# jwliao1209/DiffMusic

Hardware: AMD Instinct MI355X
Metric: denoising steps/sec (10 s clip, 200-step DPS) (higher is better)
Workload: dtype f16; 1 GPU; MusicLDM + DPS music_inpainting, 10 s @16 kHz, 200-step schedule, batch 8 per GPU (BASELINE.json configs[1]); global_batch=8, clips_per_gpu=8, lanes=1, parallelism=clip-sharded x1 (RCCL world size 1, no per-step collective), finite=True, nan_steps=0, settle_steps=10, cached_reference_transform=True, launched_by=single process

## Files before the change

diffmusic_amd/_lib.py:

```python
import ctypes as C
import os

_HERE = os.path.dirname(os.path.abspath(__file__))
LIB_PATH = os.environ.get("DMX_LIB_PATH") or os.path.join(_HERE, "lib", "libdiffmusic_hip.so")
MAX_STAGES = 8


class HifiGanConfig(C.Structure):
    _fields_ = [("model_in_dim", C.c_int), ("upsample_initial_channel", C.c_int), ("num_upsamples", C.c_int),
                ("upsample_rates", C.c_int * MAX_STAGES), ("upsample_kernel_sizes", C.c_int * MAX_STAGES),
                ("num_kernels", C.c_int), ("resblock_kernel_sizes", C.c_int * MAX_STAGES),
                ("num_dilations", C.c_int), ("resblock_dilation_sizes", C.c_int * (MAX_STAGES * MAX_STAGES)),
                ("leaky_relu_slope", C.c_float)]


class VaeConfig(C.Structure):
    _fields_ = [("latent_channels", C.c_int), ("out_channels", C.c_int), ("num_blocks", C.c_int),
                ("block_out_channels", C.c_int * MAX_STAGES), ("layers_per_block", C.c_int),
                ("norm_num_groups", C.c_int), ("eps", C.c_float)]


class UNetConfig(C.Structure):
    _fields_ = [("in_channels", C.c_int), ("out_channels", C.c_int), ("num_blocks", C.c_int),
                ("block_out_channels", C.c_int * MAX_STAGES), ("layers_per_block", C.c_int),
                ("attention_heads", C.c_int), ("norm_num_groups", C.c_int),
                ("down_attn", C.c_int * MAX_STAGES), ("up_attn", C.c_int * MAX_STAGES),
                ("class_embed_dim", C.c_int), ("num_attn_per_layer", C.c_int), ("attn_cross_dims", C.c_int * 4)]


class HtsatConfig(C.Structure):
    _fields_ = [("spec_size", C.c_int), ("num_mel_bins", C.c_int), ("patch_size", C.c_int), ("embed_dim", C.c_int), ("window_size", C.c_int),
                ("num_stages", C.c_int), ("depths", C.c_int * 4), ("num_heads", C.c_int * 4), ("ln_eps", C.c_float), ("bn_eps", C.c_float)]


class GemmDesc(C.Structure):
    _fields_ = [("A", C.c_void_p), ("W", C.c_void_p), ("C", C.c_void_p), ("C2", C.c_void_p),
                ("bias", C.c_void_p), ("rowbias", C.c_void_p), ("R", C.c_void_p), ("X", C.c_void_p),
                ("M", C.c_int), ("N", C.c_int), ("K", C.c_int), ("ldw", C.c_int),
                ("Hi", C.c_int), ("Wi", C.c_int), ("Ci", C.c_int), ("lda", C.c_int),
                ("Hq", C.c_int), ("Wq", C.c_int), ("sy", C.c_int), ("sx", C.c_int),
                ("ntaps", C.c_int),
                ("Ho", C.c_int), ("Wo", C.c_int), ("ldc", C.c_int), ("osy", C.c_int), ("ooy", C.c_int),
                ("osx", C.c_int), ("oox", C.c_int),
                ("ldr", C.c_int), ("ldx", C.c_int), ("ldc2", C.c_int),
                ("Z", C.c_int), ("Zi", C.c_int),
                ("sAo", C.c_longlong), ("sAi", C.c_longlong), ("sWo", C.c_longlong), ("sWi", C.c_longlong),
                ("sCo", C.c_longlong), ("sCi", C.c_longlong),
                ("alpha", C.c_float), ("act_slope", C.c_float), ("mask_slope", C.c_float),
                ("flags", C.c_int),
                ("tdy", C.c_byte * 16), ("tdx", C.c_byte * 16), ("resid_inv_slope", C.c_float), ("tile_cfg", C.c_int), ("ldrb", C.c_int), ("ksplit", C.c_int),
                ("XB", C.c_void_p), ("B2", C.c_void_p), ("ldxb", C.c_int), ("ldb2", C.c_int),
                ("colsum", C.c_void_p), ("ln_eps", C.c_float), ("rowstats_in", C.c_void_p), ("rowstats_out", C.c_void_p), ("nslots", C.c_int),
                ("gn_part", C.c_void_p), ("gnb_x", C.c_void_p), ("gnb_scale", C.c_void_p), ("gnb_shift", C.c_void_p),
                ("gnb_ldx", C.c_int), ("gnb_silu", C.c_int), ("gnb_stats", C.c_void_p), ("gnb_cpg", C.c_int)]


EPI_BIAS, EPI_ROWBIAS, EPI_RESID, EPI_ACCUM, EPI_MASK, EPI_LRELU2, EPI_TANH, EPI_F32OUT, EPI_NO_C, EPI_RESID_INV, EPI_MASKBITS, EPI_BITS2, EPI_SOFTBWD = \
    1, 2, 4, 8, 16, 32, 64, 128, 256, 512, 1024, 2048, 4096
EPI_GEGLU, EPI_LNFOLD, EPI_ROWSTATS, EPI_GNSTATS, EPI_GNBWD = 8192, 16384, 32768, 65536, 131072

_SIGS = {
    "dmx_abi_version": (C.c_int, []),
    "dmx_act_dtype": (C.c_int, []),
    "dmx_last_error": (C.c_char_p, []),
    "dmx_hifigan_create": (C.c_void_p, [C.POINTER(HifiGanConfig)]),
    "dmx_vae_decoder_create": (C.c_void_p, [C.POINTER(VaeConfig)]),
    "dmx_unet_create": (C.c_void_p, [C.POINTER(UNetConfig)]),
    "dmx_model_destroy": (None, [C.c_void_p]),
    "dmx_model_num_params": (C.c_int, [C.c_void_p]),
    "dmx_model_param_name": (C.c_char_p, [C.c_void_p, C.c_int]),
    "dmx_model_param_numel": (C.c_size_t, [C.c_void_p, C.c_int]),
    "dmx_model_param_ndim": (C.c_int, [C.c_void_p, C.c_int]),
    "dmx_model_param_dim": (C.c_int, [C.c_void_p, C.c_int, C.c_int]),
    "dmx_model_load_param": (C.c_int, [C.c_void_p, C.c_char_p, C.c_void_p, C.c_size_t]),
    "dmx_model_finalize": (C.c_int, [C.c_void_p, C.c_void_p]),
    "dmx_hifigan_out_len": (C.c_int, [C.c_void_p, C.c_int]),
    "dmx_hifigan_workspace_bytes": (C.c_size_t, [C.c_void_p, C.c_int, C.c_int]),
    "dmx_hifigan_fwd": (C.c_int, [C.c_void_p, C.c_void_p, C.c_void_p, C.c_int, C.c_int, C.c_void_p, C.c_size_t, C.c_void_p]),
    "dmx_hifigan_bwd": (C.c_int, [C.c_void_p, C.c_void_p, C.c_void_p, C.c_void_p]),
    "dmx_hifigan_fwd_dead": (C.c_int, [C.c_void_p, C.c_void_p, C.c_void_p, C.c_int, C.c_int, C.c_int, C.c_int, C.c_void_p, C.c_size_t,
                                       C.c_void_p]),
    "dmx_hifigan_dead_plan": (C.c_int, [C.c_void_p, C.POINTER(C.c_int), C.POINTER(C.c_int), C.POINTER(C.c_int), C.POINTER(C.c_int), C.c_int]),
    "dmx_conv_dead_rows": (C.c_int, [C.c_int] * 9 + [C.POINTER(C.c_int), C.POINTER(C.c_int)]),
    "dmx_vae_workspace_bytes": (C.c_size_t, [C.c_void_p, C.c_int, C.c_int, C.c_int]),
    "dmx_vae_decode_fwd": (C.c_int, [C.c_void_p, C.c_void_p, C.c_float, C.c_void_p, C.c_void_p, C.c_int, C.c_int, C.c_int,
                                     C.c_int, C.c_void_p, C.c_size_t, C.c_void_p]),
    "dmx_vae_decode_bwd": (C.c_int, [C.c_void_p, C.c_void_p, C.c_float, C.c_void_p, C.c_void_p]),
    "dmx_vae_encoder_create": (C.c_void_p, [C.POINTER(VaeConfig)]),
    "dmx_vae_encoder_workspace_bytes": (C.c_size_t, [C.c_void_p, C.c_int, C.c_int, C.c_int]),
    "dmx_vae_encode_fwd": (C.c_int, [C.c_void_p, C.c_void_p, C.c_float, C.c_void_p, C.c_int, C.c_int, C.c_int, C.c_void_p, C.c_size_t,
                                     C.c_void_p]),
    "dmx_latent_init": (C.c_int, [C.c_void_p] * 6 + [C.c_int] * 3 + [C.c_float] * 3 + [C.c_void_p]),
    "dmx_conv2d_raw": (C.c_int, [C.c_void_p] * 4 + [C.c_int] * 9 + [C.c_void_p]),
    "dmx_unet_workspace_bytes": (C.c_size_t, [C.c_void_p, C.c_int, C.c_int, C.c_int]),
    "dmx_unet_fwd": (C.c_int, [C.c_void_p, C.c_void_p, C.c_void_p, C.c_void_p, C.c_void_p, C.c_int, C.c_int, C.c_int,
                               C.c_void_p, C.c_size_t, C.c_void_p]),
    "dmx_unet_fwd_ctx": (C.c_int, [C.c_void_p] * 5 + [C.c_int, C.c_void_p, C.c_int, C.c_void_p, C.c_void_p, C.c_int, C.c_int, C.c_int,
                                   C.c_void_p, C.c_size_t, C.c_void_p]),
    "dmx_unet_workspace_bytes_ctx": (C.c_size_t, [C.c_void_p, C.c_int, C.c_int, C.c_int, C.c_int, C.c_int]),
    "dmx_htsat_create": (C.c_void_p, [C.POINTER(HtsatConfig)]),
    "dmx_htsat_feature_dims": (C.c_int, [C.c_void_p, C.POINTER(C.c_int), C.POINTER(C.c_int)]),
    "dmx_htsat_workspace_bytes": (C.c_size_t, [C.c_void_p, C.c_int, C.c_int]),
    "dmx_htsat_fwd": (C.c_int, [C.c_void_p, C.c_void_p, C.c_int, C.c_int, C.c_void_p, C.c_int, C.c_void_p, C.c_size_t, C.c_void_p]),
    "dmx_htsat_bwd": (C.c_int, [C.c_void_p, C.c_void_p, C.c_void_p, C.c_void_p, C.c_void_p]),
    "dmx_htsat_tape_raw": (C.c_size_t, [C.c_void_p, C.c_int, C.c_int, C.c_int, C.c_void_p, C.c_size_t, C.c_void_p]),
    "dmx_gram_fwd": (C.c_int, [C.c_void_p, C.c_void_p, C.c_int, C.c_int, C.c_int, C.c_void_p]),
    "dmx_gram_bwd": (C.c_int, [C.c_void_p, C.c_void_p, C.c_void_p, C.c_int, C.c_int, C.c_int, C.c_void_p]),
    "dmx_gemm_raw": (C.c_int, [C.c_void_p, C.c_size_t, C.c_void_p]),
    "dmx_prof_begin": (None, []),
    "dmx_prof_end": (C.c_int, [C.POINTER(C.c_double), C.POINTER(C.c_double)]),
    "dmx_flash_attn_raw": (C.c_int, [C.c_void_p, C.c_void_p, C.c_void_p, C.c_void_p, C.c_void_p] + [C.c_int] * 6 + [C.c_float, C.c_void_p]),
    "dmx_flash_attn_ld_raw": (C.c_int, [C.c_void_p] * 5 + [C.c_int] * 8 + [C.c_float, C.POINTER(C.c_int), C.c_void_p]),
    "dmx_softmax_raw": (C.c_int, [C.c_void_p] * 3 + [C.c_longlong, C.c_int, C.c_longlong, C.c_longlong, C.c_int, C.c_void_p]),
    "dmx_softmax_act_raw": (C.c_int, [C.c_void_p] * 3 + [C.c_longlong, C.c_int, C.c_longlong, C.c_int, C.c_void_p]),
    "dmx_transpose_raw": (C.c_int, [C.c_void_p, C.c_void_p, C.c_int, C.c_int, C.c_longlong, C.c_longlong, C.c_int, C.c_int] + [C.c_longlong] * 4
                          + [C.c_void_p]),
    "dmx_rowdot_raw": (C.c_int, [C.c_void_p] * 3 + [C.c_longlong, C.c_int, C.c_longlong, C.c_longlong, C.c_void_p]),
    "dmx_layernorm_raw": (C.c_int, [C.c_void_p] * 4 + [C.c_int, C.c_int, C.c_float, C.c_void_p]),
    "dmx_geglu_raw": (C.c_int, [C.c_void_p, C.c_void_p, C.c_longlong, C.c_int, C.c_void_p]),
    "dmx_gemm_splitk_workspace": (C.c_int, [C.c_void_p, C.c_size_t]),
    "dmx_conv_pair_raw": (C.c_int, [C.c_void_p, C.c_void_p, C.c_size_t, C.c_void_p]),
    "dmx_conv_pair_group_raw": (C.c_int, [C.c_int, C.c_void_p, C.c_void_p, C.c_size_t, C.c_void_p]),
    "dmx_conv_pair_dead_raw": (C.c_int, [C.c_void_p, C.c_void_p, C.c_size_t, C.POINTER(C.c_int), C.POINTER(C.c_int), C.POINTER(C.c_int), C.c_void_p]),
    "dmx_conv_pair_group_dead_raw": (C.c_int, [C.c_int, C.c_void_p, C.c_void_p, C.c_size_t, C.POINTER(C.c_int), C.c_void_p]),
    "dmx_groupnorm_scratch_floats": (C.c_size_t, [C.c_int, C.c_int, C.c_int]),
    "dmx_groupnorm_raw": (C.c_int, [C.c_void_p] * 8 + [C.c_int] * 4 + [C.c_float, C.c_int, C.c_void_p]),
    "dmx_groupnorm_part_floats": (C.c_size_t, [C.c_int, C.c_int, C.c_int]),
    "dmx_groupnorm_parts_raw": (C.c_int, [C.c_void_p] * 7 + [C.c_int] * 4 + [C.c_float, C.c_int, C.c_int, C.c_void_p, C.c_void_p, C.c_void_p]),
    "dmx_gemm_last_tile_rows_raw": (C.c_int, []),
    "dmx_groupnorm_bwd_raw": (C.c_int, [C.c_void_p] * 10 + [C.c_int] * 6 + [C.c_void_p, C.c_void_p, C.c_void_p]),
    "dmx_prof_dominant": (C.c_int, [C.POINTER(C.c_double)] * 3),
    "dmx_audio_create": (C.c_void_p, [C.c_int, C.c_int, C.c_int, C.c_int, C.c_void_p]),
    "dmx_audio_destroy": (None, [C.c_void_p]),
    "dmx_audio_num_frames": (C.c_int, [C.c_void_p, C.c_int]),
    "dmx_audio_num_bins": (C.c_int, [C.c_void_p]),
    "dmx_audio_state_bytes": (C.c_size_t, [C.c_void_p, C.c_int, C.c_int]),
    "dmx_audio_transform_fwd": (C.c_int, [C.c_void_p, C.c_void_p, C.c_longlong, C.c_void_p, C.c_void_p, C.c_int, C.c_int, C.c_int,
                                          C.c_int, C.c_float, C.c_float, C.c_void_p]),
    "dmx_audio_transform_bwd": (C.c_int, [C.c_void_p, C.c_void_p, C.c_void_p, C.c_longlong, C.c_void_p, C.c_int, C.c_int, C.c_int,
                                          C.c_int, C.c_float, C.c_float, C.c_int, C.c_void_p]),
    "dmx_audio_is_fused": (C.c_int, [C.c_void_p, C.c_int]),
    "dmx_audio_guidance_fwd": (C.c_int, [C.c_void_p, C.c_void_p, C.c_longlong, C.c_void_p, C.c_void_p, C.c_longlong, C.c_void_p, C.c_void_p,
                                         C.c_int, C.c_int, C.c_int, C.c_int, C.c_float, C.c_float, C.c_void_p]),
    "dmx_audio_guidance_bwd": (C.c_int, [C.c_void_p, C.c_void_p, C.c_longlong, C.c_void_p, C.c_void_p, C.c_longlong, C.c_float, C.c_void_p,
                                         C.c_void_p, C.c_longlong, C.c_int, C.c_void_p, C.c_int, C.c_int, C.c_int, C.c_int, C.c_float, C.c_float,
                                         C.c_void_p]),
    "dmx_audio_guidance_fwd_ex": (C.c_int, [C.c_void_p, C.c_void_p, C.c_longlong, C.c_void_p, C.c_void_p, C.c_longlong, C.c_void_p, C.c_void_p,
                                            C.c_int, C.c_int, C.c_int, C.c_int, C.c_float, C.c_float, C.c_void_p, C.c_longlong, C.c_void_p,
                                            C.c_float, C.c_void_p]),
    "dmx_audio_guidance_bwd_ex": (C.c_int, [C.c_void_p, C.c_void_p, C.c_longlong, C.c_void_p, C.c_void_p, C.c_longlong, C.c_float, C.c_void_p,
                                            C.c_void_p, C.c_longlong, C.c_int, C.c_void_p, C.c_int, C.c_int, C.c_int, C.c_int, C.c_float, C.c_float,
                                            C.c_void_p, C.c_longlong, C.c_void_p, C.c_float, C.c_void_p]),
    "dmx_audio_guidance_fwd_shaped": (C.c_int, [C.c_void_p, C.c_void_p, C.c_longlong, C.c_void_p, C.c_void_p, C.c_longlong, C.c_void_p, C.c_void_p,
                                                C.c_int, C.c_int, C.c_int, C.c_int, C.c_float, C.c_float, C.c_void_p, C.c_longlong, C.c_void_p,
                                                C.c_float, C.c_void_p, C.c_void_p]),
    "dmx_audio_guidance_bwd_shaped": (C.c_int, [C.c_void_p, C.c_void_p, C.c_longlong, C.c_void_p, C.c_void_p, C.c_longlong, C.c_float, C.c_void_p,
                                                C.c_void_p, C.c_longlong, C.c_int, C.c_void_p, C.c_int, C.c_int, C.c_int, C.c_int, C.c_float, C.c_float,
                                                C.c_void_p, C.c_longlong, C.c_void_p, C.c_float, C.c_void_p, C.c_void_p]),
    "dmx_clip_fwd": (C.c_int, [C.c_void_p, C.c_longlong, C.c_void_p, C.c_void_p, C.c_longlong, C.c_int, C.c_int, C.c_void_p]),
    "dmx_clip_bwd": (C.c_int, [C.c_void_p, C.c_longlong, C.c_void_p, C.c_longlong, C.c_void_p, C.c_void_p, C.c_longlong, C.c_int, C.c_int, C.c_int,
                               C.c_void_p]),
    "dmx_declip_project": (C.c_int, [C.c_void_p, C.c_longlong, C.c_void_p, C.c_longlong, C.c_void_p, C.c_void_p, C.c_longlong, C.c_int, C.c_int,
                                     C.c_void_p]),
    "dmx_drc_fwd": (C.c_int, [C.c_void_p, C.c_longlong, C.c_void_p, C.c_longlong, C.c_void_p, C.c_void_p, C.c_int, C.c_int] + [C.c_float] * 6 +
                    [C.c_void_p]),
    "dmx_drc_bwd": (C.c_int, [C.c_void_p, C.c_longlong, C.c_void_p, C.c_longlong, C.c_void_p, C.c_void_p, C.c_void_p, C.c_void_p, C.c_longlong,
                              C.c_int, C.c_int, C.c_int] + [C.c_float] * 6 + [C.c_void_p]),
    "dmx_drc_fwd_p": (C.c_int, [C.c_void_p, C.c_longlong, C.c_void_p, C.c_longlong, C.c_void_p, C.c_void_p, C.c_void_p, C.c_int, C.c_int, C.c_float,
                                C.c_void_p]),
    "dmx_drc_bwd_p": (C.c_int, [C.c_void_p, C.c_longlong, C.c_void_p, C.c_longlong] + [C.c_void_p] * 6 + [C.c_longlong, C.c_int, C.c_int, C.c_int,
                                                                                                        C.c_float, C.c_void_p]),
    "dmx_drc_pgrad": (C.c_int, [C.c_void_p] * 6 + [C.c_int, C.c_int, C.c_float, C.c_void_p]),
    "dmx_drc_update": (C.c_int, [C.c_void_p] * 5 + [C.c_int] * 3 + [C.c_void_p] + [C.c_double] * 3 + [C.c_float, C.c_void_p, C.c_void_p, C.c_void_p]),
    "dmx_warp_fwd": (C.c_int, [C.c_void_p, C.c_longlong, C.c_void_p, C.c_longlong, C.c_void_p, C.c_int, C.c_int, C.c_void_p]),
    "dmx_warp_bwd": (C.c_int, [C.c_void_p, C.c_void_p, C.c_longlong, C.c_void_p, C.c_int, C.c_int, C.c_int, C.c_void_p]),
    "dmx_warp_wgrad": (C.c_int, [C.c_void_p, C.c_void_p, C.c_longlong, C.c_void_p, C.c_longlong, C.c_void_p, C.c_int, C.c_int, C.c_void_p]),
    "dmx_warp_update": (C.c_int, [C.c_void_p] * 5 + [C.c_int] * 4 + [C.c_double] * 5 + [C.c_int, C.c_void_p]),
    "dmx_click_detect": (C.c_int, [C.c_void_p, C.c_longlong] + [C.c_void_p] * 5 + [C.c_int, C.c_int, C.c_float, C.c_float, C.c_void_p]),
    "dmx_click_mask": (C.c_int, [C.c_void_p, C.c_void_p, C.c_void_p, C.c_int, C.c_int, C.c_int, C.c_void_p]),
    "dmx_mask_rows": (C.c_int, [C.c_void_p, C.c_longlong, C.c_void_p, C.c_longlong, C.c_void_p, C.c_int, C.c_int, C.c_int, C.c_void_p]),
    "dmx_declick_blend": (C.c_int, [C.c_void_p, C.c_longlong, C.c_void_p, C.c_longlong, C.c_void_p, C.c_longlong, C.c_void_p, C.c_int, C.c_int,
                                    C.c_int, C.c_void_p]),
    "dmx_noise_add": (C.c_int, [C.c_void_p, C.c_void_p, C.c_void_p, C.c_longlong, C.c_float, C.c_void_p]),
    "dmx_audio_stft_mag": (C.c_int, [C.c_void_p, C.c_void_p, C.c_longlong, C.c_void_p, C.c_void_p, C.c_int, C.c_int, C.c_void_p]),
    "dmx_audio_stft_mag_bwd": (C.c_int, [C.c_void_p, C.c_void_p, C.c_void_p, C.c_longlong, C.c_void_p, C.c_int, C.c_int, C.c_int, C.c_void_p]),
    "dmx_audio_tf_frames": (C.c_int, [C.c_int]),
    "dmx_audio_tf_gain": (C.c_int, [C.c_void_p, C.c_void_p, C.c_longlong, C.c_void_p, C.c_longlong, C.c_void_p, C.c_longlong, C.c_int, C.c_int, C.c_int,
                                    C.c_void_p]),
    "dmx_audio_tf_curve": (C.c_int, [C.c_void_p, C.c_void_p, C.c_longlong, C.c_void_p, C.c_longlong, C.c_void_p, C.c_longlong, C.c_int, C.c_int, C.c_int,
                                     C.c_void_p]),
    "dmx_audio_tf_wgrad_segments": (C.c_int, [C.c_int]),
    "dmx_audio_tf_wgrad": (C.c_int, [C.c_void_p, C.c_void_p, C.c_longlong, C.c_void_p, C.c_longlong, C.c_void_p, C.c_int, C.c_int, C.c_void_p]),
    "dmx_audio_eq_update": (C.c_int, [C.c_void_p, C.c_int] + [C.c_void_p] * 3 + [C.c_int, C.c_int] + [C.c_double] * 4 + [C.c_int, C.c_void_p]),
    "dmx_audio_melscale": (C.c_int, [C.c_void_p, C.c_void_p, C.c_void_p, C.c_int, C.c_int, C.c_float, C.c_float, C.c_void_p]),
    "dmx_mask_apply": (C.c_int, [C.c_void_p, C.c_longlong, C.c_void_p, C.c_void_p, C.c_longlong, C.c_int, C.c_int, C.c_int, C.c_void_p]),
    "dmx_l2_loss": (C.c_int, [C.c_void_p, C.c_longlong, C.c_void_p, C.c_void_p, C.c_void_p, C.c_int, C.c_longlong, C.c_float, C.c_void_p]),
    "dmx_track_stitch_fwd": (C.c_int, [C.c_void_p, C.c_longlong, C.c_void_p, C.POINTER(C.c_int)] + [C.c_int] * 4 + [C.c_void_p]),
    "dmx_track_stitch_bwd": (C.c_int, [C.c_void_p, C.c_void_p, C.c_longlong, C.POINTER(C.c_int)] + [C.c_int] * 5 + [C.c_void_p]),
    "dmx_stem_mix_fwd": (C.c_int, [C.c_void_p, C.c_longlong, C.c_void_p, C.POINTER(C.c_float)] + [C.c_int] * 3 + [C.c_void_p]),
    "dmx_stem_mix_bwd": (C.c_int, [C.c_void_p, C.c_void_p, C.c_longlong, C.POINTER(C.c_float)] + [C.c_int] * 4 + [C.c_void_p]),
    "dmx_stem_project": (C.c_int, [C.c_void_p, C.c_longlong, C.c_void_p, C.c_void_p, C.POINTER(C.c_float), C.c_int, C.c_int, C.c_void_p]),
    "dmx_grad_normalize": (C.c_int, [C.c_void_p, C.c_void_p, C.c_int, C.c_longlong, C.c_float, C.c_void_p]),
    "dmx_fir_fwd": (C.c_int, [C.c_void_p, C.c_longlong, C.c_void_p, C.c_void_p, C.c_longlong] + [C.c_int] * 7 + [C.c_void_p]),
    "dmx_fir_bwd": (C.c_int, [C.c_void_p, C.c_longlong, C.c_void_p, C.c_void_p, C.c_void_p, C.c_longlong] + [C.c_int] * 7 + [C.c_void_p]),
    "dmx_fir_clip_fwd": (C.c_int, [C.c_void_p, C.c_longlong, C.c_void_p, C.c_void_p, C.c_longlong] + [C.c_int] * 4 + [C.c_void_p]),
    "dmx_fir_clip_bwd": (C.c_int, [C.c_void_p, C.c_longlong, C.c_void_p, C.c_void_p, C.c_void_p, C.c_longlong] + [C.c_int] * 4 + [C.c_void_p]),
    "dmx_fir_wgrad_workspace_floats": (C.c_size_t, [C.c_int, C.c_int, C.c_int]),
    "dmx_fir_wgrad": (C.c_int, [C.c_void_p, C.c_longlong, C.c_void_p, C.c_longlong, C.c_void_p, C.c_size_t] + [C.c_int] * 4 + [C.c_void_p]),
    "dmx_ir_update": (C.c_int, [C.c_void_p, C.c_int] + [C.c_void_p] * 4 + [C.c_int, C.c_int] + [C.c_double] * 4 + [C.c_int, C.c_void_p]),
    "dmx_sched_pred_x0": (C.c_int, [C.c_void_p, C.c_void_p, C.c_void_p, C.c_longlong, C.c_float, C.c_void_p]),
    "dmx_sched_pred_x0_ex": (C.c_int, [C.c_void_p, C.c_void_p, C.c_void_p, C.c_longlong, C.c_float, C.c_int, C.c_float, C.c_void_p]),
    "dmx_sched_step_ex": (C.c_int, [C.c_int] + [C.c_void_p] * 9 + [C.c_int, C.c_int] + [C.c_float] * 5 + [C.c_int, C.c_int, C.c_float, C.c_void_p]),
    "dmx_sched_cfg_combine": (C.c_int, [C.c_void_p, C.c_void_p, C.c_longlong, C.c_float, C.c_void_p]),
    "dmx_randn_philox": (C.c_int, [C.c_void_p, C.c_int, C.c_longlong, C.POINTER(C.c_ulonglong), C.c_ulonglong, C.c_void_p]),
    "dmx_sched_step": (C.c_int, [C.c_int] + [C.c_void_p] * 9 + [C.c_int, C.c_int] + [C.c_float] * 5 + [C.c_int, C.c_void_p]),
}

ADDED_IN_V4 = ("dmx_vae_encoder_create", "dmx_vae_encoder_workspace_bytes", "dmx_vae_encode_fwd", "dmx_latent_init",
               "dmx_track_stitch_fwd", "dmx_track_stitch_bwd", "dmx_audio_guidance_fwd_shaped", "dmx_audio_guidance_bwd_shaped",
               "dmx_clip_fwd", "dmx_clip_bwd", "dmx_declip_project", "dmx_hifigan_fwd_dead", "dmx_hifigan_dead_plan", "dmx_conv_dead_rows",
               "dmx_fir_clip_fwd", "dmx_fir_clip_bwd", "dmx_fir_wgrad", "dmx_fir_wgrad_workspace_floats", "dmx_ir_update",
               "dmx_stem_mix_fwd", "dmx_stem_mix_bwd", "dmx_stem_project", "dmx_audio_tf_gain", "dmx_audio_tf_frames",
               "dmx_audio_tf_curve", "dmx_audio_tf_wgrad_segments", "dmx_audio_tf_wgrad", "dmx_audio_eq_update", "dmx_drc_fwd", "dmx_drc_bwd",
               "dmx_warp_fwd", "dmx_warp_bwd", "dmx_warp_wgrad", "dmx_warp_update", "dmx_drc_fwd_p", "dmx_drc_bwd_p", "dmx_drc_pgrad",
               "dmx_drc_update", "dmx_click_detect", "dmx_click_mask", "dmx_mask_rows", "dmx_declick_blend")

_lib = None


def check_symbols(h, path=LIB_PATH):
    for name in ADDED_IN_V4:
        if not hasattr(h, name):
            raise RuntimeError(f"{path} reports ABI version {ABI_VERSION} but does not export `{name}` (a build from before the VAE "
                               "encoder / track-mode / declipping / blind-dereverberation / source-separation / time-frequency-masking / blind-equalisation / de-compression / wow-and-flutter / blind-wow-and-flutter / blind-de-compression / declicking entry points): rebuild it (python -m diffmusic_amd.build --force)")


def lib():
    global _lib
    if _lib is None:
        if not os.path.exists(LIB_PATH):
            raise RuntimeError(f"{LIB_PATH} is missing: build it with `python -m diffmusic_amd.build` "
                               "(the diffmusic_amd hot path has no CPU fallback)")
        h = C.CDLL(LIB_PATH)
        for name, (res, args) in _SIGS.items():
            if not hasattr(h, name):
                continue
            fn = getattr(h, name)
            fn.restype, fn.argtypes = res, args
        if h.dmx_abi_version() != ABI_VERSION:
            raise RuntimeError(f"libdiffmusic_hip.so ABI version {h.dmx_abi_version()} != {ABI_VERSION} expected by this package: rebuild it "
                               "(python -m diffmusic_amd.build --force)")
        check_symbols(h)
        _lib = h
    return _lib


ABI_VERSION = 4


def act_dtype():
    import torch
    return torch.float16 if lib().dmx_act_dtype() == 1 else torch.bfloat16


class DmxError(RuntimeError):
    pass


def check(rc, what=""):
    if rc != 0:
        msg = lib().dmx_last_error()
        raise DmxError(f"{what} failed with code {rc}: {msg.decode() if msg else ''}")
```

diffmusic_amd/csrc/capi.hip:

```cpp
#include "conv_pair.h"
#include "models.h"

#define M_IMPL(m) ((m) ? (m)->impl : nullptr)
#define ST(s) ((hipStream_t)(s))

extern "C" {

int dmx_abi_version(void) { return DMX_ABI_VERSION; }
int dmx_act_dtype(void) { return DMX_ACT_DTYPE; }

dmx_model* dmx_hifigan_create(const dmx_hifigan_config* cfg) {
  if (!cfg || cfg->num_upsamples > DMX_MAX_STAGES || cfg->num_kernels > DMX_MAX_STAGES || cfg->num_dilations > DMX_MAX_STAGES) {
    dmx_set_error("bad hifigan config");
    return nullptr;
  }
  return new dmx_model{dmx_make_hifigan(cfg)};
}
dmx_model* dmx_vae_decoder_create(const dmx_vae_config* cfg) {
  if (!cfg || cfg->num_blocks > DMX_MAX_STAGES) { dmx_set_error("bad vae config"); return nullptr; }
  Model* m = dmx_make_vae(cfg);
  return m ? new dmx_model{m} : nullptr;
}
dmx_model* dmx_unet_create(const dmx_unet_config* cfg) {
  if (!cfg || cfg->num_blocks > DMX_MAX_STAGES) { dmx_set_error("bad unet config"); return nullptr; }
  Model* m = dmx_make_unet(cfg);
  return m ? new dmx_model{m} : nullptr;
}
void dmx_model_destroy(dmx_model* m) {
  if (!m) return;
  delete m->impl;
  delete m;
}
int dmx_model_num_params(const dmx_model* m) { return (int)m->impl->ps.params.size(); }
const char* dmx_model_param_name(const dmx_model* m, int i) { return m->impl->ps.params[i].name.c_str(); }
size_t dmx_model_param_numel(const dmx_model* m, int i) { return m->impl->ps.params[i].numel; }
int dmx_model_param_ndim(const dmx_model* m, int i) { return (int)m->impl->ps.params[i].shape.size(); }
int dmx_model_param_dim(const dmx_model* m, int i, int d) { return m->impl->ps.params[i].shape[d]; }
int dmx_model_load_param(dmx_model* m, const char* name, const float* data_host, size_t numel) {
  if (m->impl->finalized) { dmx_set_error("model already finalized"); return DMX_ERR_STATE; }
  return m->impl->ps.load(name, data_host, numel);
}
int dmx_model_finalize(dmx_model* m, void* stream) {
  std::string missing;
  if (!m->impl->ps.all_loaded(&missing)) { dmx_set_error("parameter '%s' was never loaded", missing.c_str()); return DMX_ERR_PARAM; }
  const int rc = m->impl->finalize(ST(stream));
  if (rc == DMX_OK) m->impl->finalized = true;
  return rc;
}

static int check(dmx_model* m, int kind) {
  if (!m || !m->impl || m->impl->kind != kind) { dmx_set_error("wrong model handle"); return DMX_ERR_STATE; }
  if (!m->impl->finalized) { dmx_set_error("model not finalized"); return DMX_ERR_STATE; }
  return DMX_OK;
}

int dmx_hifigan_out_len(const dmx_model* m, int frames) { return dmx_hifigan_out_len_impl(m->impl, frames); }
size_t dmx_hifigan_workspace_bytes(dmx_model* m, int batch, int frames) { return dmx_hifigan_ws_impl(m->impl, batch, frames); }
int dmx_hifigan_fwd(dmx_model* m, const uint16_t* mel, float* wav, int batch, int frames, void* ws, size_t ws_bytes, void* stream) {
  int rc = check(m, DMX_MODEL_HIFIGAN);
  if (rc) return rc;
  if (!ws) { dmx_set_error("null workspace"); return DMX_ERR_WORKSPACE; }
  return dmx_hifigan_fwd_impl(m->impl, mel, wav, batch, frames, ws, ws_bytes, ST(stream));
}
int dmx_hifigan_fwd_dead(dmx_model* m, const uint16_t* mel, float* wav, int batch, int frames, int s0, int s1, void* ws, size_t ws_bytes,
                         void* stream) {
  int rc = check(m, DMX_MODEL_HIFIGAN);
  if (rc) return rc;
  if (!ws || !mel || !wav) { dmx_set_error("hifigan_fwd_dead: null buffer"); return DMX_ERR_STATE; }
  return dmx_hifigan_fwd_dead_impl(m->impl, mel, wav, batch, frames, s0, s1, ws, ws_bytes, ST(stream));
}
int dmx_hifigan_dead_plan(dmx_model* m, int* skipped, int* total, int* lo, int* hi, int n) {
  if (!m || !m->impl || m->impl->kind != DMX_MODEL_HIFIGAN) { dmx_set_error("wrong model handle"); return -1; }
  return dmx_hifigan_dead_plan_impl(m->impl, skipped, total, lo, hi, n);
}
int dmx_conv_dead_rows(int k, int dil, int pad, int stride, int transposed, int t_in, int t_out, int a, int b, int* lo, int* hi) {
  if (!lo || !hi) return DMX_ERR_STATE;
  return dmx_conv_dead_rows_impl(k, dil, pad, stride, transposed, t_in, t_out, a, b, lo, hi);
}
int dmx_hifigan_bwd(dmx_model* m, const float* dwav, uint16_t* dmel, void* stream) {
  int rc = check(m, DMX_MODEL_HIFIGAN);
  if (rc) return rc;
  return dmx_hifigan_bwd_impl(m->impl, dwav, dmel, ST(stream));
}

size_t dmx_vae_workspace_bytes(dmx_model* m, int batch, int h, int w) { return dmx_vae_ws_impl(m->impl, batch, h, w); }
int dmx_vae_decode_fwd(dmx_model* m, const float* z, float z_scale, uint16_t* mel, float* mel_f32, int batch, int h, int w,
                       int keep_state, void* ws, size_t ws_bytes, void* stream) {
  int rc = check(m, DMX_MODEL_VAE);
  if (rc) return rc;
  if (!ws) { dmx_set_error("null workspace"); return DMX_ERR_WORKSPACE; }
  return dmx_vae_fwd_impl(m->impl, z, z_scale, mel, mel_f32, batch, h, w, keep_state, ws, ws_bytes, ST(stream));
}
int dmx_vae_decode_bwd(dmx_model* m, const uint16_t* dmel, float z_scale, float* dz, void* stream) {
  int rc = check(m, DMX_MODEL_VAE);
  if (rc) return rc;
  return dmx_vae_bwd_impl(m->impl, dmel, z_scale, dz, ST(stream));
}

dmx_model* dmx_vae_encoder_create(const dmx_vae_config* cfg) {
  if (!cfg || cfg->num_blocks > DMX_MAX_STAGES) { dmx_set_error("bad vae config"); return nullptr; }
  Model* m = dmx_make_vae_encoder(cfg);
  return m ? new dmx_model{m} : nullptr;
}
size_t dmx_vae_encoder_workspace_bytes(dmx_model* m, int batch, int frames, int bins) {
  if (!m || !m->impl || m->impl->kind != DMX_MODEL_VAE_ENC) return 0;
  return dmx_vae_enc_ws_impl(m->impl, batch, frames, bins);
}
int dmx_vae_encode_fwd(dmx_model* m, const float* mel, float log_floor, float* moments, int batch, int frames, int bins, void* ws,
                       size_t ws_bytes, void* stream) {
  int rc = check(m, DMX_MODEL_VAE_ENC);
  if (rc) return rc;
  if (!ws) { dmx_set_error("null workspace"); return DMX_ERR_WORKSPACE; }
  return dmx_vae_enc_fwd_impl(m->impl, mel, log_floor, moments, batch, frames, bins, ws, ws_bytes, ST(stream));
}
int dmx_latent_init(const float* moments, float* mean, float* logvar, float* x, const float* eps, const float* noise, int batch,
                    int latent_channels, int hw, float sqrt_abar, float scaling_factor, float sqrt_1m_abar, void* stream) {
  return dmx_latent_init_impl(moments, mean, logvar, x, eps, noise, batch, latent_channels, hw, sqrt_abar, scaling_factor, sqrt_1m_abar, ST(stream));
}
int dmx_conv2d_raw(const float* w_host, const float* b_host, const void* x, void* y, int B, int Hi, int Wi, int Ci, int Co, int k, int stride,
                   int pad_lo, int pad_hi, void* stream) {
  return dmx_conv2d_raw_impl(w_host, b_host, (const act_t*)x, (act_t*)y, B, Hi, Wi, Ci, Co, k, stride, pad_lo, pad_hi, ST(stream));
}

dmx_model* dmx_htsat_create(const dmx_htsat_config* cfg) {
  Model* impl = dmx_make_htsat(cfg);
  if (!impl) return nullptr;
  return new dmx_model{impl};
}
int dmx_htsat_feature_dims(dmx_model* m, int* tokens, int* channels) {
  if (!m || !m->impl || m->impl->kind != DMX_MODEL_HTSAT) { dmx_set_error("wrong model handle"); return DMX_ERR_STATE; }
  dmx_htsat_dims_impl(m->impl, tokens, channels);
  return DMX_OK;
}
size_t dmx_htsat_workspace_bytes(dmx_model* m, int batch, int frames) {
  if (!m || !m->impl || m->impl->kind != DMX_MODEL_HTSAT) return 0;
  return dmx_htsat_ws_impl(m->impl, batch, frames);
}
int dmx_htsat_fwd(dmx_model* m, const float* mel, int batch, int frames, float* feat, int keep_state, void* ws, size_t ws_bytes, void* stream) {
  int rc = check(m, DMX_MODEL_HTSAT);
  if (rc) return rc;
  if (!ws) { dmx_set_error("null workspace"); return DMX_ERR_WORKSPACE; }
  return dmx_htsat_fwd_impl(m->impl, mel, batch, frames, feat, keep_state, ws, ws_bytes, ST(stream));
}
int dmx_htsat_bwd(dmx_model* m, const float* dfeat, const float* scale, float* dmel, void* stream) {
  int rc = check(m, DMX_MODEL_HTSAT);
  if (rc) return rc;
  return dmx_htsat_bwd_impl(m->impl, dfeat, scale, dmel, ST(stream));
}
size_t dmx_htsat_tape_raw(dmx_model* m, int stage, int block, int which, void* dst, size_t dst_elems, void* stream) {
  if (!m || !m->impl || m->impl->kind != DMX_MODEL_HTSAT) return 0;
  const act_t* p = nullptr;
  const size_t n = dmx_htsat_tape_impl(m->impl, stage, block, which, &p);
  if (n && dst && dst_elems >= n) (void)hipMemcpyAsync(dst, p, n * sizeof(act_t), hipMemcpyDeviceToDevice, ST(stream));
  return n;
}
int dmx_gram_fwd(const float* F, float* G, int batch, int tokens, int channels, void* stream) {
  const int rc = dmx_gram_fwd_impl(F, G, batch, tokens, channels, ST(stream));
  if (rc == DMX_ERR_SHAPE) dmx_set_error("gram: 1 <= tokens <= 96");
  return rc;
}
int dmx_gram_bwd(const float* F, const float* dG, float* dF, int batch, int tokens, int channels, void* stream) {
  return dmx_gram_bwd_impl(F, dG, dF, batch, tokens, channels, ST(stream));
}

size_t dmx_unet_workspace_bytes(dmx_model* m, int batch, int h, int w) { return dmx_unet_ws_impl(m->impl, batch, h, w, 0, 0); }
size_t dmx_unet_workspace_bytes_ctx(dmx_model* m, int batch, int h, int w, int n0, int n1) { return dmx_unet_ws_impl(m->impl, batch, h, w, n0, n1); }
int dmx_unet_fwd(dmx_model* m, const float* x, const float* t, const float* class_labels, float* eps, int batch, int h, int w,
                 void* ws, size_t ws_bytes, void* stream) {
  int rc = check(m, DMX_MODEL_UNET);
  if (rc) return rc;
  if (!ws) { dmx_set_error("null workspace"); return DMX_ERR_WORKSPACE; }
  return dmx_unet_fwd_impl(m->impl, x, t, class_labels, eps, batch, h, w, ws, ws_bytes, ST(stream), nullptr, 0, nullptr, 0, nullptr);
}
int dmx_unet_fwd_ctx(dmx_model* m, const float* x, const float* t, const float* class_labels, const float* ctx0, int n0,
                     const float* ctx1, int n1, const float* bias1, float* eps, int batch, int h, int w, void* ws, size_t ws_bytes,
                     void* stream) {
  int rc = check(m, DMX_MODEL_UNET);
  if (rc) return rc;
  if (!ws) { dmx_set_error("null workspace"); return DMX_ERR_WORKSPACE; }
  return dmx_unet_fwd_impl(m->impl, x, t, class_labels, eps, batch, h, w, ws, ws_bytes, ST(stream), ctx0, n0, ctx1, n1, bias1);
}

static thread_local int g_raw_gn_rows = 0;
int dmx_gemm_raw(const void* desc, size_t desc_bytes, void* stream) {
  if (desc_bytes != sizeof(GemmDesc)) { dmx_set_error("GemmDesc size mismatch: %zu vs %zu", desc_bytes, sizeof(GemmDesc)); return DMX_ERR_SHAPE; }
  return dmx_gemm_launch(*reinterpret_cast<const GemmDesc*>(desc), ST(stream), &g_raw_gn_rows);
}
int dmx_gemm_last_tile_rows_raw(void) { return g_raw_gn_rows; }

int dmx_conv_pair_raw(const void* desc_a, const void* desc_b, size_t desc_bytes, void* stream) {
  if (desc_bytes != sizeof(GemmDesc)) { dmx_set_error("GemmDesc size mismatch: %zu vs %zu", desc_bytes, sizeof(GemmDesc)); return DMX_ERR_SHAPE; }
  const GemmDesc* a = reinterpret_cast<const GemmDesc*>(desc_a);
  const GemmDesc& b = *reinterpret_cast<const GemmDesc*>(desc_b);
  if (!dmx_conv_pair_eligible(a, b)) { dmx_set_error("shape not handled by the fused convolution-pair kernel"); return DMX_ERR_SHAPE; }
  return dmx_conv_pair_launch(a, b, ST(stream));
}

int dmx_conv_pair_group_raw(int n, const void* descs_a, const void* descs_b, size_t desc_bytes, void* stream) {
  if (desc_bytes != sizeof(GemmDesc)) { dmx_set_error("GemmDesc size mismatch: %zu vs %zu", desc_bytes, sizeof(GemmDesc)); return DMX_ERR_SHAPE; }
  if (n < 1 || n > 3) { dmx_set_error("conv pair group: 1..3 problems"); return DMX_ERR_SHAPE; }
  const GemmDesc* a = reinterpret_cast<const GemmDesc*>(descs_a);
  const GemmDesc* b = reinterpret_cast<const GemmDesc*>(descs_b);
  const GemmDesc* pa[3]; const GemmDesc* pb[3];
  for (int j = 0; j < n; ++j) { pa[j] = a + j; pb[j] = b + j; }
  const int rc = dmx_conv_pair_group_launch(n, pa, pb, ST(stream));
  if (rc == DMX_ERR_SHAPE) dmx_set_error("shape not handled by the fused convolution-pair kernel");
  return rc;
}

static PairDead pair_dead_of(const int* d) { PairDead pd; pd.skip0 = d[0]; pd.skip1 = d[1]; pd.zero0 = d[2]; pd.zero1 = d[3]; return pd; }

int dmx_conv_pair_dead_raw(const void* desc_a, const void* desc_b, size_t desc_bytes, const int* dead, int* skipped, int* total, void* stream) {
  if (skipped) *skipped = 0;
  if (total) *total = 0;
  if (desc_bytes != sizeof(GemmDesc)) { dmx_set_error("GemmDesc size mismatch: %zu vs %zu", desc_bytes, sizeof(GemmDesc)); return DMX_ERR_SHAPE; }
  const GemmDesc* a = reinterpret_cast<const GemmDesc*>(desc_a);
  const GemmDesc& b = *reinterpret_cast<const GemmDesc*>(desc_b);
  if (!dmx_conv_pair_eligible(a, b)) { dmx_set_error("shape not handled by the fused convolution-pair kernel"); return DMX_ERR_SHAPE; }
  PairDead pd;
  if (dead) pd = pair_dead_of(dead);
  int sk = 0, tot = 0;
  dmx_conv_pair_slabs(a, b, dead ? &pd : nullptr, &sk, &tot);
  if (skipped) *skipped = sk;
  if (total) *total = tot;
  const int rc = dmx_conv_pair_launch(a, b, ST(stream), dead ? &pd : nullptr);
  if (rc == DMX_ERR_SHAPE) dmx_set_error("dead rows not handled by the fused convolution-pair kernel (zero rows need the residual to be stage a's input)");
  return rc;
}

int dmx_conv_pair_group_dead_raw(int n, const void* descs_a, const void* descs_b, size_t desc_bytes, const int* dead, void* stream) {
  if (desc_bytes != sizeof(GemmDesc)) { dmx_set_error("GemmDesc size mismatch: %zu vs %zu", desc_bytes, sizeof(GemmDesc)); return DMX_ERR_SHAPE; }
  if (n < 1 || n > 3) { dmx_set_error("conv pair group: 1..3 problems"); return DMX_ERR_SHAPE; }
  const GemmDesc* a = reinterpret_cast<const GemmDesc*>(descs_a);
  const GemmDesc* b = reinterpret_cast<const GemmDesc*>(descs_b);
  const GemmDesc* pa[3]; const GemmDesc* pb[3];
  PairDead pd[3];
  for (int j = 0; j < n; ++j) { pa[j] = a + j; pb[j] = b + j; if (dead) pd[j] = pair_dead_of(dead + 4 * j); }
  const int rc = dmx_conv_pair_group_launch(n, pa, pb, ST(stream), dead ? pd : nullptr);
  if (rc == DMX_ERR_SHAPE) dmx_set_error("shape not handled by the fused convolution-pair kernel");
  return rc;
}

int dmx_flash_attn_raw(const void* q, const void* k, const void* v, void* o, const float* colbias, int B, int Nq, int Nk, int ldv, int C,
                       int heads, float scale, void* stream) {
  const int rc = dmx_flash_attn_fwd((const act_t*)q, (const act_t*)k, (const act_t*)v, (act_t*)o, colbias, B, Nq, Nk, C, heads, scale,
                                    ST(stream), 0, 0, ldv);
  if (rc == DMX_ERR_SHAPE) dmx_set_error("flash attention: unsupported head_dim / strides");
  return rc;
}

int dmx_flash_attn_ld_raw(const void* q, const void* k, const void* v, void* o, const float* colbias, int B, int Nq, int Nk, int ldq, int ldk,
                          int ldv, int C, int heads, float scale, int* qt_out, void* stream) {
  if (qt_out) *qt_out = 0;
  if (B < 1 || heads < 1 || C < heads || C % heads) { dmx_set_error("flash attention: C %d is not heads %d x head_dim", C, heads); return DMX_ERR_SHAPE; }
  const int rc = dmx_flash_attn_fwd((const act_t*)q, (const act_t*)k, (const act_t*)v, (act_t*)o, colbias, B, Nq, Nk, C, heads, scale,
                                    ST(stream), ldq, ldk, ldv, qt_out);
  if (rc == DMX_ERR_SHAPE)
    dmx_set_error("flash attention: head_dim %d (multiples of 8 up to 96), Nq %d, Nk %d (>= 1) or row strides %d / %d / %d (multiples of 8) unsupported",
                  C / heads, Nq, Nk, ldq, ldk, ldv);
  return rc;
}

int dmx_softmax_raw(const float* S, void* P, const float* colbias, long long rows, int N, long long lds, long long ldp, int rows_per_bias,
                    void* stream) {
  const int rc = dmx_softmax_fwd(S, (act_t*)P, colbias, rows, N, lds, ldp, rows_per_bias, ST(stream));
  if (rc == DMX_ERR_SHAPE) dmx_set_error("softmax: N %d (a multiple of 4, <= 4096), lds %lld, ldp %lld (multiples of 4) unsupported", N, lds, ldp);
  return rc;
}
int dmx_softmax_act_raw(const void* S, void* P, const float* colbias, long long rows, int N, long long ldp, int rows_per_bias, void* stream) {
  const int rc = dmx_softmax_act((const act_t*)S, (act_t*)P, colbias, rows, N, ldp, rows_per_bias, ST(stream));
  if (rc == DMX_ERR_SHAPE) dmx_set_error("softmax: N %d (a multiple of 4, <= 4096), ldp %lld (a multiple of 4) unsupported", N, ldp);
  return rc;
}
int dmx_transpose_raw(const void* in, void* out, int R, int C, long long ldi, long long ldo, int Z, int Zi, long long sIo, long long sIi,
                      long long sOo, long long sOi, void* stream) {
  return dmx_transpose((const act_t*)in, (act_t*)out, R, C, ldi, ldo, Z, Zi, sIo, sIi, sOo, sOi, ST(stream));
}
int dmx_rowdot_raw(const void* a, const void* b, float* out, long long rows, int C, long long lda, long long ldb, void* stream) {
  const int rc = dmx_rowdot((const act_t*)a, (const act_t*)b, out, rows, C, lda, ldb, ST(stream));
  if (rc == DMX_ERR_SHAPE) dmx_set_error("rowdot: C %d, lda %lld, ldb %lld must be multiples of 8", C, lda, ldb);
  return rc;
}
int dmx_layernorm_raw(const void* x, void* y, const float* gamma, const float* beta, int rows, int C, float eps, void* stream) {
  const int rc = dmx_layernorm_fwd((const act_t*)x, (act_t*)y, gamma, beta, rows, C, eps, ST(stream));
  if (rc == DMX_ERR_SHAPE) dmx_set_error("layernorm: C %d must be a multiple of 8", C);
  return rc;
}
int dmx_geglu_raw(const void* x, void* y, long long rows, int I, void* stream) {
  const int rc = dmx_geglu((const act_t*)x, (act_t*)y, rows, I, ST(stream));
  if (rc == DMX_ERR_SHAPE) dmx_set_error("geglu: I %d must be a multiple of 8", I);
  return rc;
}

int dmx_gemm_splitk_workspace(void* ws, size_t bytes) {
  dmx_gemm_set_splitk_workspace(reinterpret_cast<float*>(ws), ws ? bytes : 0);
  return DMX_OK;
}

size_t dmx_groupnorm_scratch_floats(int B, int C, int G) { return dmx_gn_scratch_floats(B, C, G); }
int dmx_groupnorm_raw(const void* x, void* y, const float* gamma, const float* beta, float* stats, float* scale, float* shift,
                      float* partial, int B, int P, int C, int G, float eps, int silu, void* stream) {
  const int rc = dmx_groupnorm_fwd((const act_t*)x, (act_t*)y, gamma, beta, stats, scale, shift, partial, B, P, C, G, eps, silu, ST(stream));
  if (rc == DMX_ERR_SHAPE) dmx_set_error("groupnorm: unsupported channel / group counts");
  return rc;
}

size_t dmx_groupnorm_part_floats(int B, int P, int N) { return dmx_gn_part_floats(B, P, N); }
int dmx_groupnorm_parts_raw(const void* x, void* y, const float* gamma, const float* beta, float* stats, float* scale, float* shift,
                            int B, int P, int C, int G, float eps, int silu, int nreg, float* const* part, const int* geom, void* stream) {
  if (nreg < 1 || nreg > 8) { dmx_set_error("groupnorm_parts: 1..8 regions"); return DMX_ERR_SHAPE; }
  if (G <= 0 || C % G || ((C / G) & 3)) { dmx_set_error("groupnorm_parts: channels per group must be a multiple of 4 (C %d, G %d)", C, G); return DMX_ERR_SHAPE; }
  GnParts gp;
  for (int i = 0; i < nreg; ++i) {
    GnRegion r;
    r.part = part[i]; r.tm = geom[i * 6]; r.P = geom[i * 6 + 1]; r.nq = geom[i * 6 + 2]; r.qoff = geom[i * 6 + 3]; r.cq = geom[i * 6 + 4];
    if (!r.part || r.tm < 32 || r.P < r.tm || r.nq <= 0 || r.cq <= 0 || r.cq > r.nq || r.qoff < 0 || r.qoff + r.cq > C / 4) {
      dmx_set_error("groupnorm_parts: region %d: tm %d, P %d, nq %d, qoff %d, cq %d do not describe a producer launch of this tensor", i, r.tm, r.P, r.nq, r.qoff, r.cq);
      return DMX_ERR_SHAPE;
    }
    gp.r[gp.n++] = r;
  }
  const int rc = dmx_groupnorm_fwd((const act_t*)x, (act_t*)y, gamma, beta, stats, scale, shift, nullptr, B, P, C, G, eps, silu, ST(stream), &gp);
  if (rc == DMX_ERR_SHAPE) dmx_set_error("groupnorm: unsupported channel / group counts");
  return rc;
}
int dmx_groupnorm_bwd_raw(const void* x, const void* dy, const void* add, void* dx, const float* stats, const float* scale, const float* shift,
                          float* k0, float* k1, float* partial, int B, int P, int C, int G, int silu, int nreg, float* const* part,
                          const int* geom, void* stream) {
  if (nreg < 0 || nreg > 8) { dmx_set_error("groupnorm_bwd: 0..8 regions"); return DMX_ERR_SHAPE; }
  if (nreg > 0 && !partial && (G <= 0 || C % G || ((C / G) & 3))) { dmx_set_error("groupnorm_bwd: regions need channels per group % 4 == 0, or scratch for the classic pass"); return DMX_ERR_SHAPE; }
  GnParts gp;
  for (int i = 0; i < nreg; ++i) {
    GnRegion r;
    r.part = part[i]; r.tm = geom[i * 6]; r.P = geom[i * 6 + 1]; r.nq = geom[i * 6 + 2]; r.qoff = geom[i * 6 + 3]; r.cq = geom[i * 6 + 4];
    if (!r.part || r.tm < 32 || r.P < r.tm || r.nq <= 0 || r.cq <= 0 || r.cq > r.nq || r.qoff < 0 || r.qoff + r.cq > C / 4) {
      dmx_set_error("groupnorm_bwd: region %d does not describe a producer launch of this tensor", i);
      return DMX_ERR_SHAPE;
    }
    gp.r[gp.n++] = r;
  }
  return dmx_groupnorm_bwd((const act_t*)x, (const act_t*)dy, (const act_t*)add, (act_t*)dx, stats, scale, shift, k0, k1, partial, B, P, C, G,
                           silu, ST(stream), nreg ? &gp : nullptr);
}

}
```

diffmusic_amd/csrc/conv_pair.h:

```cpp
#pragma once
#include <cstdlib>
#include <cstring>
#include "dmx_common.h"

struct PairDead { int skip0 = 0, skip1 = 0, zero0 = 0, zero1 = 0; };

bool dmx_conv_pair_eligible(const GemmDesc* a, const GemmDesc& b);
int dmx_conv_pair_launch(const GemmDesc* a, const GemmDesc& b, hipStream_t st, const PairDead* dead = nullptr);
int dmx_conv_pair_group_launch(int n, const GemmDesc* const* a, const GemmDesc* const* b, hipStream_t st, const PairDead* dead = nullptr);
void dmx_conv_pair_slabs(const GemmDesc* a, const GemmDesc& b, const PairDead* dead, int* skipped, int* total);

int dmx_prof_open(hipStream_t st);
void dmx_prof_close(int rec, hipStream_t st, double flops, double bytes, int M, int N, int K, int taps, int flags, int cfg);
```

diffmusic_amd/csrc/conv_pair.hip:

```cpp
#include "gemm_epilogue.h"
#include "conv_pair.h"

namespace {

constexpr int PAIR_HALO = 50;
constexpr int PAIR_ROWS = 256;
constexpr unsigned PAIR_OOB = 0x80000000u;

struct PairParams {
  GemmDesc a, b;
  int T, nb, BMo;
  int loA, hiA, loB, hiB;
  int off0A, dA, off0B, dB;
  int single;
  int r_from_slab;
  int a_tape_bits_only;
  int skip_q0, skip_n;
  int z0, z1;
};

#ifdef DMX_PAIR_STAMPS
__device__ unsigned long long g_pair_stamps[4096 * 8];
#define DMX_STAMP(i) do { stamp_v[i] = wall_clock64(); } while (0)
#else
#define DMX_STAMP(i) do { } while (0)
#endif

template <int C>
struct PairCfg {
  static constexpr int PITCH = 2 * C + 32;
  static constexpr int CPR = C / 8;
  static constexpr int WN = C > 64 ? C / 64 : 1;
  static constexpr int NW = 4 * WN;
  static constexpr int NT = NW * 64;
  static constexpr int FN = C / 16 / WN;
  static constexpr int SLAB_ROWS = PAIR_ROWS + PAIR_HALO;
  static constexpr int SLAB_BYTES = SLAB_ROWS * PITCH;
  static constexpr int TILE = C * 128;
  static constexpr int NS = C == 128 ? 4 : 3;
  static constexpr int PER = TILE / 1024 / NW;
  static constexpr int SLAB_IT = (SLAB_ROWS * CPR + NT - 1) / NT;
  static constexpr int BITS_IT = PAIR_ROWS * CPR / NT;
  static constexpr int BITS_BYTES = PAIR_ROWS * CPR;
  static constexpr int BIAS_BYTES = 2 * C * 4;
  static constexpr int LDS_BYTES = SLAB_BYTES + NS * TILE + BITS_BYTES + BIAS_BYTES;
  static constexpr int MIN_WAVES = C == 32 ? 3 : 2;
  static_assert(PER >= 1 && PAIR_ROWS * CPR % NT == 0, "tile / thread-count mismatch");
};

template <int FN>
struct PairFrags { frag8_t x[2][4]; frag8_t w[2][FN]; };

#define DMX_PAIR_DSR(dst, addr, off) asm volatile("ds_read_b128 %0, %1 offset:%2" : "=v"(dst) : "v"(addr), "n"(off))

#define DMX_LDS_ADDR(p) ((unsigned)(size_t)(__attribute__((address_space(3))) const char*)(p))
typedef unsigned u32x2_t __attribute__((ext_vector_type(2)));
typedef unsigned u32x4_t __attribute__((ext_vector_type(4)));
__device__ __forceinline__ void pair_lds_w64(const void* p, uint2 v) {
  const u32x2_t w = {v.x, v.y};
  asm volatile("ds_write_b64 %0, %1" ::"v"(DMX_LDS_ADDR(p)), "v"(w) : "memory");
}
#define DMX_PAIR_DSR64(dst, p) asm volatile("ds_read_b64 %0, %1" : "=v"(dst) : "v"(DMX_LDS_ADDR(p)))
#define DMX_PAIR_DSRU8(dst, p) asm volatile("ds_read_u8 %0, %1" : "=v"(dst) : "v"(DMX_LDS_ADDR(p)))
__device__ __forceinline__ void pair_lds_wait() { asm volatile("s_waitcnt lgkmcnt(0)" ::: "memory"); }
template <typename T>
__device__ __forceinline__ void pair_tie8(T (&r)[8]) {
  asm volatile("s_waitcnt lgkmcnt(0)" : "+v"(r[0]), "+v"(r[1]), "+v"(r[2]), "+v"(r[3]), "+v"(r[4]), "+v"(r[5]), "+v"(r[6]), "+v"(r[7]) : : "memory");
}
template <typename T>
__device__ __forceinline__ void pair_tie16(T (&r)[16]) {
  asm volatile("s_waitcnt lgkmcnt(0)"
               : "+v"(r[0]), "+v"(r[1]), "+v"(r[2]), "+v"(r[3]), "+v"(r[4]), "+v"(r[5]), "+v"(r[6]), "+v"(r[7]), "+v"(r[8]), "+v"(r[9]), "+v"(r[10]),
                 "+v"(r[11]), "+v"(r[12]), "+v"(r[13]), "+v"(r[14]), "+v"(r[15])
               :
               : "memory");
}
template <typename T, int N>
__device__ __forceinline__ void pair_tie(T (&r)[N]) {
  static_assert(N == 8 || N == 16, "4 row fragments x 2 or 4 column fragments");
  if constexpr (N == 8) pair_tie8(r); else pair_tie16(r);
}

__device__ __forceinline__ void pair_settle(PairFrags<4>& f) {
  asm volatile("s_waitcnt lgkmcnt(0)"
               : "+v"(f.x[0][0]), "+v"(f.x[0][1]), "+v"(f.x[0][2]), "+v"(f.x[0][3]), "+v"(f.x[1][0]), "+v"(f.x[1][1]), "+v"(f.x[1][2]),
                 "+v"(f.x[1][3]), "+v"(f.w[0][0]), "+v"(f.w[0][1]), "+v"(f.w[0][2]), "+v"(f.w[0][3]), "+v"(f.w[1][0]), "+v"(f.w[1][1]),
                 "+v"(f.w[1][2]), "+v"(f.w[1][3])
               :
               : "memory");
}
__device__ __forceinline__ void pair_settle(PairFrags<2>& f) {
  asm volatile("s_waitcnt lgkmcnt(0)"
               : "+v"(f.x[0][0]), "+v"(f.x[0][1]), "+v"(f.x[0][2]), "+v"(f.x[0][3]), "+v"(f.x[1][0]), "+v"(f.x[1][1]), "+v"(f.x[1][2]),
                 "+v"(f.x[1][3]), "+v"(f.w[0][0]), "+v"(f.w[0][1]), "+v"(f.w[1][0]), "+v"(f.w[1][1])
               :
               : "memory");
}

template <int C>
__device__ __forceinline__ void pair_body(const PairParams& P, char* smem, int bid, const int nwg) {
  using K = PairCfg<C>;
  constexpr int PITCH = K::PITCH, CPR = K::CPR, FN = K::FN, NS = K::NS, PER = K::PER, TILE = K::TILE, NT = K::NT, NW = K::NW, WN = K::WN;
  char* ring = smem;
  char* slab = smem + NS * TILE;
  unsigned char* s_bits = reinterpret_cast<unsigned char*>(slab + K::SLAB_BYTES);
  float* s_bias = reinterpret_cast<float*>(slab + K::SLAB_BYTES + K::BITS_BYTES);

  const int tid = threadIdx.x, lane = tid & 63, lr = lane & 15, lq = lane >> 4;
  const int wave = __builtin_amdgcn_readfirstlane(tid >> 6);
  const int rg = wave / WN, cg = wave - rg * WN;
#ifdef DMX_PAIR_STAMPS
  const int stamp_id = bid;
  unsigned long long stamp_v[8] = {0, 0, 0, 0, 0, 0, 0, 0};
#endif
  DMX_STAMP(0);
  {
    const int q = nwg >> 3, r = nwg & 7, xcd = bid & 7, loc = bid >> 3;
    bid = (xcd < r ? xcd * (q + 1) : r * (q + 1) + (xcd - r) * q) + loc;
  }
  const int T = P.T;
  const int b = bid / P.nb;
  int tq = bid - b * P.nb;
  if (tq >= P.skip_q0) tq += P.skip_n;
  const int t0 = tq * P.BMo;
  const bool single = P.single != 0;
  const int kA = single ? 0 : P.a.ntaps, kB = P.b.ntaps;
  const int stepsA = (kA * C + 63) / 64, stepsB = (kB * C + 63) / 64, total = stepsA + stepsB;

  const __amdgpu_buffer_rsrc_t rsA = __builtin_amdgcn_make_buffer_rsrc(const_cast<act_t*>(single ? P.b.W : P.a.W), 0, PAIR_OOB, 0x00020000);
  const __amdgpu_buffer_rsrc_t rsB = __builtin_amdgcn_make_buffer_rsrc(const_cast<act_t*>(P.b.W), 0, PAIR_OOB, 0x00020000);
  const int lrow = lane >> 3, cc = (lane & 7) ^ lrow;
  auto issue_dma = [&](int g) {
    const bool inA = g < stepsA;
    const int sidx = inA ? g : g - stepsA;
    const int Kel = inA ? P.a.K : P.b.K;
    const unsigned ldw2 = (unsigned)(inA ? P.a.ldw : P.b.ldw) * 2u;
    const int kel = sidx * 64 + cc * 8;
    const bool ok = g < total && kel < Kel;
    char* dst = ring + (g % NS) * TILE;
#pragma unroll
    for (int i = 0; i < PER; ++i) {
      const int j = i * NW + wave;
      const unsigned voff = ok ? (unsigned)(j * 8 + lrow) * ldw2 + (unsigned)kel * 2u : PAIR_OOB;
      if (inA) __builtin_amdgcn_raw_ptr_buffer_load_lds(rsA, (__attribute__((address_space(3))) void*)(dst + j * 1024), 16, voff, 0, 0, 0);
      else __builtin_amdgcn_raw_ptr_buffer_load_lds(rsB, (__attribute__((address_space(3))) void*)(dst + j * 1024), 16, voff, 0, 0, 0);
    }
  };
  issue_dma(0);
  issue_dma(1);
  issue_dma(2);

  {
    const act_t* src = single ? P.b.A : P.a.A;
    const int nrows = PAIR_ROWS + (single ? P.loB + P.hiB : P.loA + P.hiA);
    const int tfirst = t0 - P.loB - (single ? 0 : P.loA);
    uint4 sv[K::SLAB_IT];
#pragma unroll
    for (int it = 0; it < K::SLAB_IT; ++it) {
      const int c = tid + it * NT, row = c / CPR, piece = c % CPR, t = tfirst + row;
      sv[it] = make_uint4(0, 0, 0, 0);
      if (row < nrows && t >= 0 && t < T && !(t >= P.z0 && t < P.z1)) sv[it] = *reinterpret_cast<const uint4*>(src + ((long long)b * T + t) * C + piece * 8);
    }
    const bool masked = !single && (P.a.flags & EPI_MASK);
    const bool maskbits = !single && (P.a.flags & EPI_MASKBITS);
    constexpr int BPT = K::BITS_BYTES / NT;
    static_assert(BPT == 4 || BPT == 8, "bit-mask copy granularity");
    static_assert(CPR % BPT == 0, "a thread's mask bytes must stay inside one row");
    uint32_t mb[2] = {0u, 0u};
    if (maskbits) {
      const int c = tid * BPT, row = c / CPR, piece = c % CPR, t = t0 - P.loB + row;
      if (t >= 0 && t < T) {
        const unsigned char* src = P.a.XB + ((long long)b * T + t) * P.a.ldxb + piece;
        mb[0] = *reinterpret_cast<const uint32_t*>(src);
        if (BPT == 8) mb[1] = *reinterpret_cast<const uint32_t*>(src + 4);
      }
    }
#pragma unroll
    for (int it = 0; it < K::SLAB_IT; ++it) {
      const int c = tid + it * NT, row = c / CPR, piece = c % CPR;
      if (row < K::SLAB_ROWS) *reinterpret_cast<uint4*>(slab + row * PITCH + piece * 16) = sv[it];
    }
    if (masked) {
#pragma unroll 1
      for (int it = 0; it < K::BITS_IT; ++it) {
        const int c = tid + it * NT, row = c / CPR, piece = c % CPR, t = t0 - P.loB + row;
        uint4 m = make_uint4(0, 0, 0, 0);
        if (t >= 0 && t < T) m = *reinterpret_cast<const uint4*>(P.a.X + ((long long)b * T + t) * C + piece * 8);
        s_bits[c] = (unsigned char)dmx_pos8(m);
      }
    }
    if (maskbits) {
      uint32_t* d = reinterpret_cast<uint32_t*>(s_bits + tid * BPT);
      d[0] = mb[0];
      if (BPT == 8) d[1] = mb[1];
    }
  }
  if (tid < 2 * C) {
    const GemmDesc& d = tid < C ? P.a : P.b;
    const int ch = tid < C ? tid : tid - C;
    s_bias[tid] = (!(single && tid < C) && d.bias && (d.flags & (EPI_BIAS | EPI_BIASINIT))) ? d.bias[ch] : 0.f;
  }
  asm volatile("s_waitcnt vmcnt(0)" ::: "memory");
  __syncthreads();
  DMX_STAMP(1);

  f32x4 acc[4][FN];
  auto zero_acc = [&]() {
#pragma unroll
    for (int i = 0; i < 4; ++i)
#pragma unroll
      for (int n = 0; n < FN; ++n) acc[i][n] = f32x4{0.f, 0.f, 0.f, 0.f};
  };
  auto init_acc = [&](const GemmDesc& d) {
    if (C < 128 && (d.flags & EPI_BIASINIT)) {
      f32x4 bb[FN];
#pragma unroll
      for (int n = 0; n < FN; ++n)
        asm volatile("ds_read_b128 %0, %1" : "=v"(bb[n]) : "v"(DMX_LDS_ADDR(s_bias + (&d == &P.b ? C : 0) + cg * 64 + n * 16 + lq * 4)));
      if constexpr (FN == 2) asm volatile("s_waitcnt lgkmcnt(0)" : "+v"(bb[0]), "+v"(bb[1]) : : "memory");
      else asm volatile("s_waitcnt lgkmcnt(0)" : "+v"(bb[0]), "+v"(bb[1]), "+v"(bb[2]), "+v"(bb[3]) : : "memory");
#pragma unroll
      for (int n = 0; n < FN; ++n)
#pragma unroll
        for (int i = 0; i < 4; ++i) acc[i][n] = bb[n];
    } else {
      zero_acc();
    }
  };
  using Frags = PairFrags<FN>;
  const unsigned xlane = (unsigned)(size_t)(__attribute__((address_space(3))) const char*)(slab + (rg * 64 + lr) * PITCH + lq * 16);
  const unsigned wlane0 = (unsigned)(size_t)(__attribute__((address_space(3))) const char*)(ring + (cg * 64 + lr) * 128 + (((0 * 4 + lq) ^ (lr & 7)) << 4));
  const unsigned wlane1 = (unsigned)(size_t)(__attribute__((address_space(3))) const char*)(ring + (cg * 64 + lr) * 128 + (((1 * 4 + lq) ^ (lr & 7)) << 4));
  auto load_frags = [&](Frags& f, bool isB, int sidx, int g) {
    const int off0 = isB ? P.off0B : P.off0A, dd = isB ? P.dB : P.dA, kk = isB ? kB : kA;
    unsigned xa0, xa1;
    if constexpr (C >= 64) {
      constexpr int SPT = C / 64;
      const int tp = sidx / SPT, kh = sidx - tp * SPT;
      xa0 = xlane + (unsigned)((off0 + tp * dd) * PITCH + kh * 128);
      xa1 = xa0 + 64u;
    } else {
      const int tp0 = 2 * sidx, tp1 = (2 * sidx + 1 < kk) ? 2 * sidx + 1 : kk - 1;
      xa0 = xlane + (unsigned)((off0 + tp0 * dd) * PITCH);
      xa1 = xlane + (unsigned)((off0 + tp1 * dd) * PITCH);
    }
    const unsigned wo = (unsigned)((g % NS) * TILE);
    const unsigned wa0 = wlane0 + wo, wa1 = wlane1 + wo;
    static_for<0, 4>([&f, xa0, xa1](auto I) {
      constexpr int i = decltype(I)::value;
      DMX_PAIR_DSR(f.x[0][i], xa0, i * 16 * PITCH);
      DMX_PAIR_DSR(f.x[1][i], xa1, i * 16 * PITCH);
    });
    static_for<0, FN>([&f, wa0, wa1](auto N) {
      constexpr int n = decltype(N)::value;
      DMX_PAIR_DSR(f.w[0][n], wa0, n * 2048);
      DMX_PAIR_DSR(f.w[1][n], wa1, n * 2048);
    });
  };
  auto mfma_half = [&](const Frags& f, int ks) {
#pragma unroll
    for (int i = 0; i < 4; ++i)
#pragma unroll
      for (int n = 0; n < FN; ++n) acc[i][n] = DMX_MFMA16(f.w[ks][n], f.x[ks][i], acc[i][n]);
  };
  auto step = [&](Frags& cur, Frags& nxt, bool isB, int sidx, int n, int g) {
    const bool more = sidx + 1 < n;
    if (more) load_frags(nxt, isB, sidx + 1, g + 1);
    mfma_half(cur, 0);
    __builtin_amdgcn_sched_barrier(0);
    issue_dma(g + 3);
    __builtin_amdgcn_sched_barrier(0);
    mfma_half(cur, 1);
    if (more) pair_settle(nxt);
    asm volatile("s_waitcnt vmcnt(%0)" ::"n"(PER) : "memory");
    __builtin_amdgcn_s_barrier();
  };
  auto run_stage = [&](bool isB, int n, int g0) {
    Frags fa, fb;
    load_frags(fa, isB, 0, g0);
    pair_settle(fa);
    __builtin_amdgcn_s_barrier();
    if constexpr (C == 128) {
      int sidx = 0;
      for (; sidx + 1 < n; sidx += 2) {
        const int g = g0 + sidx;
        load_frags(fb, isB, sidx + 1, g + 1);
        mfma_half(fa, 0);
        __builtin_amdgcn_sched_barrier(0);
        issue_dma(g + 3);
        __builtin_amdgcn_sched_barrier(0);
        mfma_half(fa, 1);
        __builtin_amdgcn_sched_barrier(0);
        issue_dma(g + 4);
        __builtin_amdgcn_sched_barrier(0);
        pair_settle(fb);
        const bool more = sidx + 2 < n;
        if (more) load_frags(fa, isB, sidx + 2, g + 2);
        mfma_half(fb, 0);
        mfma_half(fb, 1);
        if (more) pair_settle(fa);
        asm volatile("s_waitcnt vmcnt(0)" ::: "memory");
        __builtin_amdgcn_s_barrier();
      }
      if (sidx < n) {
        mfma_half(fa, 0);
        __builtin_amdgcn_sched_barrier(0);
        issue_dma(g0 + sidx + 3);
        __builtin_amdgcn_sched_barrier(0);
        mfma_half(fa, 1);
        asm volatile("s_waitcnt vmcnt(0)" ::: "memory");
        __builtin_amdgcn_s_barrier();
      }
    } else {
      for (int sidx = 0; sidx < n; sidx += 2) {
        step(fa, fb, isB, sidx, n, g0 + sidx);
        if (sidx + 1 < n) step(fb, fa, isB, sidx + 1, n, g0 + sidx + 1);
      }
    }
  };

  uint2 rpre[4 * FN];
  unsigned tape_bits[2] = {0u, 0u};
  bool tape_bits_valid = false;
#pragma unroll
  for (int i = 0; i < 4 * FN; ++i) rpre[i] = make_uint2(0, 0);
  if (!single) {
    init_acc(P.a);
    run_stage(false, stepsA, 0);
    DMX_STAMP(2);
    const int fa = P.a.flags;
    float4 abias[FN];
    {
      f32x4 ab[FN];
#pragma unroll
      for (int n = 0; n < FN; ++n) asm volatile("ds_read_b128 %0, %1" : "=v"(ab[n]) : "v"(DMX_LDS_ADDR(s_bias + cg * 64 + n * 16 + lq * 4)));
      if constexpr (FN == 2) asm volatile("s_waitcnt lgkmcnt(0)" : "+v"(ab[0]), "+v"(ab[1]) : : "memory");
      else asm volatile("s_waitcnt lgkmcnt(0)" : "+v"(ab[0]), "+v"(ab[1]), "+v"(ab[2]), "+v"(ab[3]) : : "memory");
#pragma unroll
      for (int n = 0; n < FN; ++n) abias[n] = (fa & EPI_BIAS) ? make_float4(ab[n][0], ab[n][1], ab[n][2], ab[n][3]) : make_float4(0.f, 0.f, 0.f, 0.f);
    }
    if (P.r_from_slab) {
      u32x2_t rp[4 * FN];
#pragma unroll
      for (int i = 0; i < 4; ++i)
#pragma unroll
        for (int n = 0; n < FN; ++n)
          DMX_PAIR_DSR64(rp[i * FN + n], slab + (rg * 64 + i * 16 + lr + P.loA + P.loB) * PITCH + (cg * 64 + n * 16 + lq * 4) * 2);
      pair_tie(rp);
#pragma unroll
      for (int k = 0; k < 4 * FN; ++k) rpre[k] = make_uint2(rp[k][0], rp[k][1]);
      __builtin_amdgcn_s_barrier();
    }
    DMX_STAMP(6);
    const float aslope = P.a.act_slope, mslope = P.a.mask_slope;
#pragma unroll
    for (int i = 0; i < 4; ++i) {
      const int row = rg * 64 + i * 16 + lr;
      const int t = t0 - P.loB + row;
      const bool inside = t >= 0 && t < T;
      unsigned mbits[FN];
#pragma unroll
      for (int n = 0; n < FN; ++n) mbits[n] = 0u;
      if (fa & (EPI_MASK | EPI_MASKBITS)) {
#pragma unroll
        for (int n = 0; n < FN; ++n) DMX_PAIR_DSRU8(mbits[n], s_bits + row * CPR + ((cg * 64 + n * 16 + lq * 4) >> 3));
        if constexpr (FN == 2) asm volatile("s_waitcnt lgkmcnt(0)" : "+v"(mbits[0]), "+v"(mbits[1]) : : "memory");
        else asm volatile("s_waitcnt lgkmcnt(0)" : "+v"(mbits[0]), "+v"(mbits[1]), "+v"(mbits[2]), "+v"(mbits[3]) : : "memory");
      }
#pragma unroll
      for (int n = 0; n < FN; ++n) {
        const int ch = cg * 64 + n * 16 + lq * 4;
        float v[4] = {acc[i][n][0], acc[i][n][1], acc[i][n][2], acc[i][n][3]};
        if (fa & (EPI_MASK | EPI_MASKBITS)) {
          const unsigned bits = mbits[n] >> (ch & 4);
#pragma unroll
          for (int e = 0; e < 4; ++e) v[e] *= ((bits >> e) & 1u) ? 1.f : mslope;
        }
        {
          const float4 bb = abias[n];
          v[0] += bb.x; v[1] += bb.y; v[2] += bb.z; v[3] += bb.w;
        }
        if (fa & EPI_LRELU2) {
#pragma unroll
          for (int e = 0; e < 4; ++e) v[e] = v[e] > 0.f ? v[e] : v[e] * aslope;
        }
        if (!inside) { v[0] = v[1] = v[2] = v[3] = 0.f; }
        pair_lds_w64(slab + row * PITCH + ch * 2, make_uint2(pack2a(v[0], v[1]), pack2a(v[2], v[3])));
      }
    }
    pair_lds_wait();
    __builtin_amdgcn_s_barrier();
    DMX_STAMP(7);
    if (fa & EPI_LRELU2) {
      const bool bits = (fa & EPI_BITS2) != 0, full = !P.a_tape_bits_only;
      u32x4_t tq[K::BITS_IT];
#pragma unroll
      for (int it = 0; it < K::BITS_IT; ++it) {
        const int c = tid + it * NT, row = c / CPR, piece = c % CPR;
        asm volatile("ds_read_b128 %0, %1" : "=v"(tq[it]) : "v"(DMX_LDS_ADDR(slab + row * PITCH + piece * 16)));
      }
      static_assert(K::BITS_IT == 4 || K::BITS_IT == 8, "tape read-back granularity");
      if constexpr (K::BITS_IT == 4)
        asm volatile("s_waitcnt lgkmcnt(0)" : "+v"(tq[0]), "+v"(tq[1]), "+v"(tq[2]), "+v"(tq[3]) : : "memory");
      else
        asm volatile("s_waitcnt lgkmcnt(0)" : "+v"(tq[0]), "+v"(tq[1]), "+v"(tq[2]), "+v"(tq[3]), "+v"(tq[4]), "+v"(tq[5]), "+v"(tq[6]), "+v"(tq[7]) : : "memory");
      uint4 tv[K::BITS_IT];
#pragma unroll
      for (int it = 0; it < K::BITS_IT; ++it) tv[it] = make_uint4(tq[it][0], tq[it][1], tq[it][2], tq[it][3]);
#pragma unroll
      for (int it = 0; it < K::BITS_IT; ++it) {
        const int c = tid + it * NT, row = c / CPR, piece = c % CPR, t = t0 - P.loB + row;
        if (row >= P.loB && row < P.loB + P.BMo && t < T) {
          if (full) *reinterpret_cast<uint4*>(P.a.C2 + ((long long)b * T + t) * C + piece * 8) = tv[it];
        }
        if constexpr (C < 128) {
          if (bits) tape_bits[it >> 2] |= (dmx_pos8(tv[it]) & 0xffu) << (8 * (it & 3));
        } else {
          if (bits && row >= P.loB && row < P.loB + P.BMo && t < T) P.a.B2[((long long)b * T + t) * P.a.ldb2 + piece] = (unsigned char)dmx_pos8(tv[it]);
        }
      }
      tape_bits_valid = bits && C < 128;
    }
  }

  DMX_STAMP(3);
  init_acc(P.b);
  run_stage(true, stepsB, stepsA);
  __syncthreads();
  DMX_STAMP(4);
  {
    constexpr int EPI_WAVE_BYTES = 64 * (FN * 32 + 16) + 64 * 12;
    static_assert(EPI_WAVE_BYTES * NW <= K::SLAB_BYTES, "epilogue staging does not fit the slab");
    const int mbase = b * T + t0;
    const int tend = t0 + P.BMo < T ? t0 + P.BMo : T;
    gemm_epilogue_lds_impl<4, FN, 1>(P.b, acc, mbase + rg * 64, cg * 64, lane, 0, T, slab + wave * EPI_WAVE_BYTES, b * T + tend, rpre,
                                        !single && P.r_from_slab != 0);
  }
  if (tape_bits_valid) {
#pragma unroll
    for (int it = 0; it < K::BITS_IT; ++it) {
      const int c = tid + it * NT, row = c / CPR, piece = c % CPR, t = t0 - P.loB + row;
      if (row >= P.loB && row < P.loB + P.BMo && t < T)
        P.a.B2[((long long)b * T + t) * P.a.ldb2 + piece] = (unsigned char)((tape_bits[it >> 2] >> (8 * (it & 3))) & 0xffu);
    }
  }
  DMX_STAMP(5);
#ifdef DMX_PAIR_STAMPS
  if (threadIdx.x == 0 && stamp_id < 4096)
    for (int i = 0; i < 8; ++i) g_pair_stamps[stamp_id * 8 + i] = stamp_v[i];
#endif
}

template <int C>
__global__ __launch_bounds__(PairCfg<C>::NT, PairCfg<C>::MIN_WAVES) void conv_pair_kernel(const PairParams P) {
  extern __shared__ __attribute__((aligned(1024))) char smem[];
  pair_body<C>(P, smem, blockIdx.x, gridDim.x);
}

constexpr int DMX_PAIR_GROUP = 3;
struct PairGroup { PairParams p[DMX_PAIR_GROUP]; int n[DMX_PAIR_GROUP]; };
template <int C>
__global__ __launch_bounds__(PairCfg<C>::NT, PairCfg<C>::MIN_WAVES) void conv_pair_group_kernel(const PairGroup G) {
  extern __shared__ __attribute__((aligned(1024))) char smem[];
  const int j = blockIdx.y, n = G.n[j];
  if ((int)blockIdx.x >= n) return;
  pair_body<C>(G.p[j], smem, blockIdx.x, n);
}

struct Halo { int lo, hi; bool ok; int d; };
Halo halo_of(const GemmDesc& d) {
  Halo h{0, 0, true, d.ntaps > 1 ? d.tdx[1] - d.tdx[0] : 0};
  for (int j = 0; j < d.ntaps; ++j) {
    if (d.tdx[j] != d.tdx[0] + j * h.d) h.ok = false;
    if (d.tdy[j] != 0) h.ok = false;
    if (-d.tdx[j] > h.lo) h.lo = -d.tdx[j];
    if (d.tdx[j] > h.hi) h.hi = d.tdx[j];
  }
  if (h.lo + h.hi > PAIR_HALO) h.ok = false;
  return h;
}

bool stage_ok(const GemmDesc& d, int C, int T, int allowed_flags) {
  if (d.N != C || d.Ci != C || d.lda != C || d.K != d.ntaps * C || d.ldw < d.K) return false;
  if (d.ntaps < 1 || d.ntaps > 16 || d.Z != 1 || d.Hq != 1 || d.Hi != 1 || d.Ho != 1) return false;
  if (d.Wq != T || d.Wi != T || d.Wo != T || d.sx != 1 || d.osx != 1 || d.oox != 0 || d.ooy != 0) return false;
  if (d.flags & ~allowed_flags) return false;
  if (d.M % T != 0) return false;
  return true;
}

bool g_pair_enabled = getenv("DMX_NO_PAIR") == nullptr;

}

bool dmx_conv_pair_eligible(const GemmDesc* a, const GemmDesc& b) {
  if (!g_pair_enabled) return false;
  const int C = b.N, T = b.Wq;
  static const bool c128 = getenv("DMX_NO_PAIR128") == nullptr;
  if (C != 32 && C != 64 && !(C == 128 && c128)) return false;
  if (T < 1) return false;
  const int bflags = EPI_BIAS | EPI_RESID | EPI_RESID_INV | EPI_ACCUM | EPI_MASK | EPI_LRELU2 | EPI_NO_C | EPI_MASKBITS | EPI_BITS2;
  if (!stage_ok(b, C, T, bflags) || !halo_of(b).ok) return false;
  if ((b.flags & EPI_LRELU2) && !(b.act_slope >= 0.f && b.act_slope <= 1.f)) return false;
  if ((b.flags & EPI_RESID_INV) && !(b.resid_inv_slope >= 1.f)) return false;
  if (b.ldc != C || ((b.flags & EPI_RESID) && b.ldr != C) || ((b.flags & EPI_MASK) && b.ldx != C) || ((b.flags & EPI_LRELU2) && b.ldc2 != C))
    return false;
  if ((b.flags & EPI_MASKBITS) && (!b.XB || b.ldxb * 8 < C || (b.ldxb & 3))) return false;
  if ((b.flags & EPI_BITS2) && (!b.B2 || b.ldb2 * 8 < C)) return false;
  if (a) {
    if (!stage_ok(*a, C, T, EPI_BIAS | EPI_LRELU2 | EPI_NO_C | EPI_MASK | EPI_MASKBITS | EPI_BITS2) || !halo_of(*a).ok) return false;
    if (a->M != b.M || a->alpha != 1.f) return false;
    if ((a->flags & EPI_LRELU2) && !(a->flags & EPI_BITS2) && (a->ldc2 != C || !a->C2)) return false;
    if ((a->flags & EPI_LRELU2) && a->C2 && a->ldc2 != C) return false;
    if ((a->flags & EPI_BITS2) && (!(a->flags & EPI_LRELU2) || !a->B2 || a->ldb2 * 8 < C)) return false;
    if ((a->flags & EPI_MASK) && (a->ldx != C || !a->X)) return false;
    if ((a->flags & EPI_MASKBITS) && (!a->XB || a->ldxb * 8 < C || (a->ldxb & 3) || (a->flags & EPI_MASK))) return false;
    const Halo hb = halo_of(b);
    if (PAIR_ROWS - hb.lo - hb.hi < 128) return false;
  }
  return true;
}

namespace {
void pair_skip_slabs(const PairDead* dead, int T, int BMo, int& q0, int& q1) {
  q0 = q1 = 0;
  if (!dead || dead->skip1 <= dead->skip0) return;
  const int nb = cdiv(T, BMo);
  const int lo = cdiv(dead->skip0 > 0 ? dead->skip0 : 0, BMo), hi = dead->skip1 >= T ? nb : dead->skip1 / BMo;
  if (hi > lo && hi - lo < nb) { q0 = lo; q1 = hi; }
}

long long pair_params(const GemmDesc* a, const GemmDesc& b, PairParams& P, double& fl, double& by, const PairDead* dead = nullptr) {
  memset(&P, 0, sizeof(P));
  P.b = b;
  P.single = a ? 0 : 1;
  if (a) P.a = *a;
  const Halo hb = halo_of(b);
  P.loB = hb.lo; P.hiB = hb.hi;
  P.off0B = b.tdx[0] + hb.lo; P.dB = hb.d;
  if (a) { const Halo ha = halo_of(*a); P.loA = ha.lo; P.hiA = ha.hi; P.off0A = a->tdx[0] + ha.lo; P.dA = ha.d; }
  P.T = b.Wq;
  P.BMo = a ? PAIR_ROWS - hb.lo - hb.hi : PAIR_ROWS;
  P.nb = cdiv(P.T, P.BMo);
  const int nb_all = P.nb;
  {
    int q0, q1;
    pair_skip_slabs(dead, P.T, P.BMo, q0, q1);
    P.skip_q0 = q0; P.skip_n = q1 - q0;
    P.nb -= P.skip_n;
    if (dead && dead->zero1 > dead->zero0) { P.z0 = dead->zero0; P.z1 = dead->zero1; }
  }
  static const bool bias_init = getenv("DMX_NO_BIAS_INIT") == nullptr;
  if (bias_init && b.N < 128) {
    if ((P.b.flags & EPI_BIAS) && P.b.bias && !(P.b.flags & (EPI_MASK | EPI_MASKBITS))) P.b.flags = (P.b.flags & ~EPI_BIAS) | EPI_BIASINIT;
    if (a && (P.a.flags & EPI_BIAS) && P.a.bias && !(P.a.flags & (EPI_MASK | EPI_MASKBITS))) P.a.flags = (P.a.flags & ~EPI_BIAS) | EPI_BIASINIT;
  }
  P.r_from_slab = (a && (b.flags & EPI_RESID) && b.R == a->A && b.ldr == b.N) ? 1 : 0;
  P.a_tape_bits_only = (a && (a->flags & EPI_BITS2) && !a->C2) ? 1 : 0;
  const int nclips = b.M / P.T;
  const int C = b.N;
  fl = 2.0 * b.M * (double)b.N * b.K;
  by = 2.0 * b.M * (double)C * 2.0;
  const double bits_by = b.M * (double)C / 8.0;
  if (a) {
    fl += 2.0 * a->M * (double)a->N * a->K;
    if ((a->flags & EPI_LRELU2) && !P.a_tape_bits_only) by += 2.0 * b.M * (double)C;
    if (a->flags & EPI_BITS2) by += bits_by;
    if (a->flags & EPI_MASK) by += 2.0 * b.M * (double)C;
    if (a->flags & EPI_MASKBITS) by += bits_by;
  }
  if ((b.flags & EPI_RESID) && !P.r_from_slab) by += 2.0 * b.M * (double)C;
  if (b.flags & EPI_MASK) by += 2.0 * b.M * (double)C;
  if (b.flags & EPI_MASKBITS) by += bits_by;
  if (b.flags & EPI_BITS2) by += bits_by;
  if (b.flags & EPI_ACCUM) by += 2.0 * b.M * (double)C;
  if ((b.flags & EPI_LRELU2) && !(b.flags & EPI_NO_C)) by += 2.0 * b.M * (double)C;
  fl *= (double)P.nb / nb_all; by *= (double)P.nb / nb_all;
  return (long long)nclips * P.nb;
}
bool pair_zero_ok(const PairParams& P) { return P.z1 <= P.z0 || !(P.b.flags & EPI_RESID) || P.r_from_slab; }
}

void dmx_conv_pair_slabs(const GemmDesc* a, const GemmDesc& b, const PairDead* dead, int* skipped, int* total) {
  const Halo hb = halo_of(b);
  const int T = b.Wq, BMo = a ? PAIR_ROWS - hb.lo - hb.hi : PAIR_ROWS;
  int q0, q1;
  pair_skip_slabs(dead, T, BMo, q0, q1);
  *skipped = q1 - q0;
  *total = cdiv(T, BMo);
}

static int pair_extra_lds() { static const int v = [] { const char* e = getenv("DMX_PAIR_EXTRA_LDS"); return e ? atoi(e) : 0; }(); return v; }
int dmx_conv_pair_launch(const GemmDesc* a, const GemmDesc& b, hipStream_t st, const PairDead* dead) {
  if (!dmx_conv_pair_eligible(a, b)) return DMX_ERR_SHAPE;
  PairParams P;
  double fl, by;
  const long long grid = pair_params(a, b, P, fl, by, dead);
  if (grid > 0x7fffffffLL) return DMX_ERR_SHAPE;
  if (!pair_zero_ok(P)) return DMX_ERR_SHAPE;
  const int C = b.N;
  const int rec = dmx_prof_open(st);
  auto launch = [&](auto tag) {
    constexpr int CC = decltype(tag)::value;
    static bool attr = false;
    if (!attr) { (void)hipFuncSetAttribute((const void*)conv_pair_kernel<CC>, hipFuncAttributeMaxDynamicSharedMemorySize, PairCfg<CC>::LDS_BYTES + (CC < 128 ? pair_extra_lds() : 0)); attr = true; }
    hipLaunchKernelGGL(conv_pair_kernel<CC>, dim3((unsigned)grid), dim3(PairCfg<CC>::NT), PairCfg<CC>::LDS_BYTES + (CC < 128 ? pair_extra_lds() : 0), st, P);
  };
  if (C == 32) launch(std::integral_constant<int, 32>{});
  else if (C == 64) launch(std::integral_constant<int, 64>{});
  else launch(std::integral_constant<int, 128>{});
  dmx_prof_close(rec, st, fl, by, b.M, b.N, (a ? a->K : 0) + b.K, b.ntaps, b.flags, a ? 21 : 20);
  return hipGetLastError() == hipSuccess ? DMX_OK : DMX_ERR_LAUNCH;
}

int dmx_conv_pair_group_launch(int n, const GemmDesc* const* a, const GemmDesc* const* b, hipStream_t st, const PairDead* dead) {
  if (n < 1 || n > DMX_PAIR_GROUP) return DMX_ERR_SHAPE;
  static const bool off = getenv("DMX_NO_PAIR_GROUP") != nullptr;
  bool same = !off && n > 1;
  for (int j = 0; j < n; ++j) {
    if (!a[j] || !b[j] || !dmx_conv_pair_eligible(a[j], *b[j])) return DMX_ERR_SHAPE;
    if (b[j]->N != b[0]->N) same = false;
    for (int i = 0; i < j; ++i)
      if (b[j]->C == b[i]->C || (b[j]->C2 && b[j]->C2 == b[i]->C2)) same = false;
  }
  if (!same) {
    for (int j = 0; j < n; ++j) { const int rc = dmx_conv_pair_launch(a[j], *b[j], st, dead ? dead + j : nullptr); if (rc != DMX_OK) return rc; }
    return DMX_OK;
  }
  int order[DMX_PAIR_GROUP] = {0, 1, 2};
  auto work = [&](int j) { return a[j]->K + b[j]->K; };
  for (int i = 0; i < n; ++i)
    for (int k = i + 1; k < n; ++k)
      if (work(order[k]) > work(order[i])) { const int t = order[i]; order[i] = order[k]; order[k] = t; }
  PairGroup G;
  memset(&G, 0, sizeof(G));
  double fl = 0.0, by = 0.0;
  long long gmax = 0;
  int Ksum = 0;
  for (int i = 0; i < n; ++i) {
    const int j = order[i];
    double f1, b1;
    const long long g = pair_params(a[j], *b[j], G.p[i], f1, b1, dead ? dead + j : nullptr);
    if (g > 0x7ffffff0LL || !pair_zero_ok(G.p[i])) return DMX_ERR_SHAPE;
    G.n[i] = (int)g;
    if (g > gmax) gmax = g;
    fl += f1; by += b1; Ksum += a[j]->K + b[j]->K;
  }
  const unsigned gx = (unsigned)((gmax + 7) & ~7ll);
  const int C = b[0]->N;
  const int rec = dmx_prof_open(st);
  auto launch = [&](auto tag) {
    constexpr int CC = decltype(tag)::value;
    static bool attr = false;
    if (!attr) { (void)hipFuncSetAttribute((const void*)conv_pair_group_kernel<CC>, hipFuncAttributeMaxDynamicSharedMemorySize, PairCfg<CC>::LDS_BYTES); attr = true; }
    hipLaunchKernelGGL(conv_pair_group_kernel<CC>, dim3(gx, (unsigned)n), dim3(PairCfg<CC>::NT), PairCfg<CC>::LDS_BYTES, st, G);
  };
  if (C == 32) launch(std::integral_constant<int, 32>{});
  else if (C == 64) launch(std::integral_constant<int, 64>{});
  else launch(std::integral_constant<int, 128>{});
  dmx_prof_close(rec, st, fl, by, b[0]->M, C, Ksum, b[0]->ntaps, b[0]->flags, 22);
  return hipGetLastError() == hipSuccess ? DMX_OK : DMX_ERR_LAUNCH;
}

#ifdef DMX_PAIR_STAMPS
extern "C" int dmx_pair_stamps_read(unsigned long long* host) {
  return hipMemcpyFromSymbol(host, HIP_SYMBOL(g_pair_stamps), sizeof(unsigned long long) * 4096 * 8) == hipSuccess ? 0 : -1;
}
#endif
```

diffmusic_amd/csrc/gemm_epilogue.h:

```cpp
#pragma once
#include "dmx_common.h"
#include <type_traits>

namespace {

template <int I, int N, typename F>
__device__ __forceinline__ void static_for(F&& f) {
  if constexpr (I < N) {
    f(std::integral_constant<int, I>{});
    static_for<I + 1, N>(f);
  }
}


template <int FM, int FN>
__device__ __forceinline__ void gemm_epilogue(const GemmDesc& p, f32x4 (&acc)[FM][FN], int m0, int n0, int lr, int lq,
                                              long long coff, int HqWq) {
  const int flags = p.flags;
#pragma unroll
  for (int i = 0; i < FM; ++i) {
    const int m = m0 + i * 16 + lr;
    if (m >= p.M) continue;
    const int b = m / HqWq, rem = m - b * HqWq;
    const int qy = rem / p.Wq, qx = rem - qy * p.Wq;
    const long long orow = ((long long)b * p.Ho + (qy * p.osy + p.ooy)) * p.Wo + (qx * p.osx + p.oox);
#pragma unroll
    for (int j = 0; j < FN; ++j) {
      const int n = n0 + j * 16 + lq * 4;
      if (n >= p.N) continue;
      float v[4] = {acc[i][j][0], acc[i][j][1], acc[i][j][2], acc[i][j][3]};
      if (flags & EPI_MASK) {
        const uint2 xr = *reinterpret_cast<const uint2*>(p.X + coff + orow * p.ldx + n);
        const float s = p.mask_slope;
        v[0] *= (alo(xr.x) > 0.f) ? 1.f : s;
        v[1] *= (ahi(xr.x) > 0.f) ? 1.f : s;
        v[2] *= (alo(xr.y) > 0.f) ? 1.f : s;
        v[3] *= (ahi(xr.y) > 0.f) ? 1.f : s;
      }
      if (flags & EPI_BIAS) {
        const float4 bb = *reinterpret_cast<const float4*>(p.bias + n);
        v[0] += bb.x; v[1] += bb.y; v[2] += bb.z; v[3] += bb.w;
      }
      if (flags & EPI_ROWBIAS) {
        const float4 bb = *reinterpret_cast<const float4*>(p.rowbias + (long long)b * (p.ldrb ? p.ldrb : p.N) + n);
        v[0] += bb.x; v[1] += bb.y; v[2] += bb.z; v[3] += bb.w;
      }
      if (flags & EPI_RESID) {
        const uint2 rr = *reinterpret_cast<const uint2*>(p.R + coff + orow * p.ldr + n);
        float r0 = alo(rr.x), r1 = ahi(rr.x), r2 = alo(rr.y), r3 = ahi(rr.y);
        if (flags & EPI_RESID_INV) {
          const float is = p.resid_inv_slope;
          r0 = r0 > 0.f ? r0 : r0 * is; r1 = r1 > 0.f ? r1 : r1 * is; r2 = r2 > 0.f ? r2 : r2 * is; r3 = r3 > 0.f ? r3 : r3 * is;
        }
        v[0] += r0; v[1] += r1; v[2] += r2; v[3] += r3;
      }
      const float al = p.alpha;
      v[0] *= al; v[1] *= al; v[2] *= al; v[3] *= al;
      if (flags & EPI_F32OUT) {
        float* cp = reinterpret_cast<float*>(p.C) + coff + orow * p.ldc + n;
        if (flags & EPI_ACCUM) {
          const float4 o = *reinterpret_cast<const float4*>(cp);
          v[0] += o.x; v[1] += o.y; v[2] += o.z; v[3] += o.w;
        }
        if (flags & EPI_TANH) { v[0] = tanhf(v[0]); v[1] = tanhf(v[1]); v[2] = tanhf(v[2]); v[3] = tanhf(v[3]); }
        *reinterpret_cast<float4*>(cp) = make_float4(v[0], v[1], v[2], v[3]);
      } else {
        act_t* cp = reinterpret_cast<act_t*>(p.C) + coff + orow * p.ldc + n;
        if (flags & EPI_ACCUM) {
          const uint2 o = *reinterpret_cast<const uint2*>(cp);
          v[0] += alo(o.x); v[1] += ahi(o.x); v[2] += alo(o.y); v[3] += ahi(o.y);
        }
        if (flags & EPI_TANH) { v[0] = tanhf(v[0]); v[1] = tanhf(v[1]); v[2] = tanhf(v[2]); v[3] = tanhf(v[3]); }
        if (!(flags & EPI_NO_C)) *reinterpret_cast<uint2*>(cp) = make_uint2(pack2a(v[0], v[1]), pack2a(v[2], v[3]));
      }
      if (flags & EPI_LRELU2) {
        const float s = p.act_slope;
        const float a0 = v[0] > 0.f ? v[0] : v[0] * s, a1 = v[1] > 0.f ? v[1] : v[1] * s;
        const float a2 = v[2] > 0.f ? v[2] : v[2] * s, a3 = v[3] > 0.f ? v[3] : v[3] * s;
        *reinterpret_cast<uint2*>(p.C2 + coff + orow * p.ldc2 + n) = make_uint2(pack2a(a0, a1), pack2a(a2, a3));
      }
    }
  }
}

__device__ __forceinline__ unsigned dmx_pos8(const uint4& v) {
  auto pos = [](uint32_t u) -> uint32_t { return (((u & 0x7fff7fffu) + 0x7fff7fffu) & ~u) & 0x80008000u; };
  const uint32_t w = (pos(v.x) >> 15) | (pos(v.y) >> 13) | (pos(v.z) >> 11) | (pos(v.w) >> 9);
  return (w & 0x55u) | ((w >> 15) & 0xaau);
}

#ifndef DMX_GNB_HB
#define DMX_GNB_HB 4
#endif
#ifndef DMX_EPI_IB
#define DMX_EPI_IB 4
#endif
template <int FM>
struct EpiChunk { static constexpr int IB = (FM % DMX_EPI_IB == 0) ? DMX_EPI_IB : (FM % 4 == 0) ? 4 : (FM % 3 == 0) ? 3 : (FM % 2 == 0) ? 2 : 1; static constexpr int CH = IB * 16; };

template <int FM, int FN, int EM>
__device__ __forceinline__ void gemm_epilogue_lds_impl(const GemmDesc& p, f32x4 (&acc)[FM][FN], int m0, int n0, int lane,
                                                       long long coff, int HqWq, char* wl, int mlimit,
                                                       const uint2 (&rpre)[FM * FN], const bool use_rpre) {
  constexpr bool BITS = EM == 1;
  constexpr bool SOFT = EM == 2;
  constexpr bool GEGLU = EM == 3;
  constexpr bool ROWS = EM == 4;
  static_assert(!ROWS || FN == 2 || FN == 4, "row statistics come in slots of 32 columns");
  constexpr bool GNS = EM == 5;
  constexpr bool GNB = EM == 6;
  static_assert(!GEGLU || FN % 2 == 0, "GEGLU pairs accumulator fragments");
  constexpr int CH = EpiChunk<FM>::CH;
  constexpr int IB = EpiChunk<FM>::IB;
  constexpr int TNB = FN * 32;
  constexpr int PITCH = TNB + 16;
  constexpr int CPR = TNB / 16;
  constexpr int RPI = 64 / CPR;
  constexpr int NIT = CH / RPI;
  static_assert(CH % RPI == 0, "chunk rows must be a multiple of the rows per wave-instruction");
  const int lr = lane & 15, lq = lane >> 4;
  const int rr = lane / CPR, cch = lane - rr * CPR;
  int* tab = reinterpret_cast<int*>(wl + CH * PITCH);
  const int flags = p.flags;
  const int ncol = n0 + cch * 8;
  const bool col_ok = ncol < p.N;
  const int mend = p.M < mlimit ? p.M : mlimit;
  const bool ident = p.osy == 1 && p.osx == 1 && p.ooy == 0 && p.oox == 0 && p.Ho == p.Hq && p.Wo == p.Wq;
#define DMX_LDS_SYNC() asm volatile("s_waitcnt lgkmcnt(0)" ::: "memory")
  float4 bcol[FN];
#pragma unroll
  for (int j = 0; j < FN; ++j) {
    const int n = n0 + j * 16 + lq * 4;
    bcol[j] = ((flags & EPI_BIAS) && n < p.N) ? *reinterpret_cast<const float4*>(p.bias + n) : make_float4(0.f, 0.f, 0.f, 0.f);
  }
  float gs[4] = {0.f, 0.f, 0.f, 0.f};
  constexpr int GN_SLOT = 64;
  static_assert(!(GNS || GNB) || (CH == GN_SLOT && FN == 4), "GroupNorm statistics: 64-row chunks of 64-column wave tiles only (one summation order)");
  const int gn_b0 = (GNS || GNB) ? m0 / HqWq : 0;
  static_for<0, FM / IB>([&](auto H) {
    constexpr int h = decltype(H)::value;
    int orows[NIT];
    if (ident) {
#pragma unroll
      for (int it = 0; it < NIT; ++it) {
        const int m = m0 + h * CH + it * RPI + rr;
        orows[it] = m < mend ? m : -1;
      }
    } else {
      if (lane < CH) {
        const int m = m0 + h * CH + lane;
        int orow = -1;
        if (m < mend) {
          const int b = m / HqWq, rem = m - b * HqWq;
          const int qy = rem / p.Wq, qx = rem - qy * p.Wq;
          orow = (b * p.Ho + (qy * p.osy + p.ooy)) * p.Wo + (qx * p.osx + p.oox);
        }
        tab[lane] = orow;
      }
      DMX_LDS_SYNC();
#pragma unroll
      for (int it = 0; it < NIT; ++it) orows[it] = tab[it * RPI + rr];
      DMX_LDS_SYNC();
    }
    auto stage_in = [&](const act_t* G, int ld, auto&& f) {
      {
        uint4 v[NIT];
#pragma unroll
        for (int it = 0; it < NIT; ++it) {
          const bool ok = orows[it] >= 0 && col_ok;
          const long long off = ok ? (long long)orows[it] * ld + ncol : 0ll;
          v[it] = *reinterpret_cast<const uint4*>(G + coff + off);
          if (!ok) v[it] = make_uint4(0, 0, 0, 0);
        }
#pragma unroll
        for (int it = 0; it < NIT; ++it) *reinterpret_cast<uint4*>(wl + (it * RPI + rr) * PITCH + cch * 16) = v[it];
      }
      DMX_LDS_SYNC();
#pragma unroll
      for (int ii = 0; ii < IB; ++ii)
#pragma unroll
        for (int j = 0; j < FN; ++j) {
          const uint2 q = *reinterpret_cast<const uint2*>(wl + (ii * 16 + lr) * PITCH + (j * 16 + lq * 4) * 2);
          f(acc[h * IB + ii][j], alo(q.x), ahi(q.x), alo(q.y), ahi(q.y));
        }
      DMX_LDS_SYNC();
    };
    auto stage_out = [&](act_t* G, int ld, auto&& f) {
      constexpr int JS = GEGLU ? 2 : 1;
      static_for<0, IB>([&](auto II) {
        static_for<0, FN / JS>([&](auto JJ) {
          constexpr int ii = decltype(II)::value, j = decltype(JJ)::value * JS;
          float o[4];
          f(acc[h * IB + ii][j], o);
          *reinterpret_cast<uint2*>(wl + (ii * 16 + lr) * PITCH + ((j / JS) * 16 + lq * 4) * 2) = make_uint2(pack2a(o[0], o[1]), pack2a(o[2], o[3]));
        });
      });
      DMX_LDS_SYNC();
      constexpr int HN = NIT > 4 ? NIT / 2 : NIT;
#pragma unroll
      for (int g0 = 0; g0 < NIT; g0 += HN) {
      uint4 v[HN];
#pragma unroll
      for (int it = 0; it < HN; ++it) v[it] = *reinterpret_cast<const uint4*>(wl + ((g0 + it) * RPI + rr) * PITCH + cch * 16);
      const int ocol = GEGLU ? (n0 >> 1) + cch * 8 : ncol;
      const bool ocol_ok = GEGLU ? (cch < CPR / 2 && ocol < (p.N >> 1)) : col_ok;
#pragma unroll
      for (int it = 0; it < HN; ++it) {
        if (orows[g0 + it] >= 0 && ocol_ok) *reinterpret_cast<uint4*>(G + coff + (long long)orows[g0 + it] * ld + ocol) = v[it];
      }
      }
    };
    auto emit_gn = [&]() {
#ifndef DMX_BF16
      typedef _Float16 dmx_h2 __attribute__((ext_vector_type(2)));
      const dmx_h2 one = {(_Float16)1.0f, (_Float16)1.0f};
#endif
#pragma unroll
      for (int it = 0; it < NIT; ++it) {
        const uint4 v = *reinterpret_cast<const uint4*>(wl + (it * RPI + rr) * PITCH + cch * 16);
        if (orows[it] >= 0 && col_ok) {
#ifndef DMX_BF16
          const dmx_h2 a0 = __builtin_bit_cast(dmx_h2, v.x), a1 = __builtin_bit_cast(dmx_h2, v.y);
          const dmx_h2 a2 = __builtin_bit_cast(dmx_h2, v.z), a3 = __builtin_bit_cast(dmx_h2, v.w);
          const float s0 = __builtin_amdgcn_fdot2(a0, one, __builtin_amdgcn_fdot2(a1, one, 0.f, false), false);
          const float q0 = __builtin_amdgcn_fdot2(a0, a0, __builtin_amdgcn_fdot2(a1, a1, 0.f, false), false);
          const float s1 = __builtin_amdgcn_fdot2(a2, one, __builtin_amdgcn_fdot2(a3, one, 0.f, false), false);
          const float q1 = __builtin_amdgcn_fdot2(a2, a2, __builtin_amdgcn_fdot2(a3, a3, 0.f, false), false);
#else
          const float f0 = alo(v.x), f1 = ahi(v.x), f2 = alo(v.y), f3 = ahi(v.y), f4 = alo(v.z), f5 = ahi(v.z), f6 = alo(v.w), f7 = ahi(v.w);
          const float s0 = (f0 + f1) + (f2 + f3), s1 = (f4 + f5) + (f6 + f7);
          const float q0 = __builtin_fmaf(f0, f0, __builtin_fmaf(f1, f1, __builtin_fmaf(f2, f2, f3 * f3)));
          const float q1 = __builtin_fmaf(f4, f4, __builtin_fmaf(f5, f5, __builtin_fmaf(f6, f6, f7 * f7)));
#endif
          gs[0] += s0; gs[1] += q0; gs[2] += s1; gs[3] += q1;
        }
      }
    };
    auto emit_gnb = [&]() {
      {
        const int bb = gn_b0;
        float sc[8], sf[8];
        {
          const float* scp = p.gnb_scale + (long long)bb * p.N + ncol;
          const float* sfp = p.gnb_shift + (long long)bb * p.N + ncol;
          const float4 a0 = col_ok ? *reinterpret_cast<const float4*>(scp) : make_float4(0.f, 0.f, 0.f, 0.f);
          const float4 a1 = col_ok ? *reinterpret_cast<const float4*>(scp + 4) : make_float4(0.f, 0.f, 0.f, 0.f);
          const float4 c0 = col_ok ? *reinterpret_cast<const float4*>(sfp) : make_float4(0.f, 0.f, 0.f, 0.f);
          const float4 c1 = col_ok ? *reinterpret_cast<const float4*>(sfp + 4) : make_float4(0.f, 0.f, 0.f, 0.f);
          sc[0] = a0.x; sc[1] = a0.y; sc[2] = a0.z; sc[3] = a0.w; sc[4] = a1.x; sc[5] = a1.y; sc[6] = a1.z; sc[7] = a1.w;
          sf[0] = c0.x; sf[1] = c0.y; sf[2] = c0.z; sf[3] = c0.w; sf[4] = c1.x; sf[5] = c1.y; sf[6] = c1.z; sf[7] = c1.w;
        }
        const int ngrp = p.N / p.gnb_cpg;
        const float mu[2] = {col_ok ? p.gnb_stats[((long long)bb * ngrp + ncol / p.gnb_cpg) * 2] : 0.f,
                             col_ok ? p.gnb_stats[((long long)bb * ngrp + (ncol + 4) / p.gnb_cpg) * 2] : 0.f};
        constexpr int HB = DMX_GNB_HB > 4 && NIT % DMX_GNB_HB == 0 ? DMX_GNB_HB : (NIT % 4 == 0 ? 4 : (NIT % 3 == 0 ? 3 : (NIT % 2 == 0 ? 2 : 1)));
#pragma unroll
        for (int g0 = 0; g0 < NIT; g0 += HB) {
          uint4 xv[HB];
          bool ok[HB];
#pragma unroll
          for (int it = 0; it < HB; ++it) {
            ok[it] = orows[g0 + it] >= 0 && col_ok;
            xv[it] = *reinterpret_cast<const uint4*>(p.gnb_x + (ok[it] ? (long long)orows[g0 + it] * p.gnb_ldx + ncol : 0ll));
          }
#pragma unroll
          for (int it = 0; it < HB; ++it) {
            const uint4 dv = *reinterpret_cast<const uint4*>(wl + ((g0 + it) * RPI + rr) * PITCH + cch * 16);
            if (ok[it]) {
              const float xf[8] = {alo(xv[it].x), ahi(xv[it].x), alo(xv[it].y), ahi(xv[it].y), alo(xv[it].z), ahi(xv[it].z), alo(xv[it].w), ahi(xv[it].w)};
              const float df[8] = {alo(dv.x), ahi(dv.x), alo(dv.y), ahi(dv.y), alo(dv.z), ahi(dv.z), alo(dv.w), ahi(dv.w)};
              float a1[2] = {0.f, 0.f}, a2[2] = {0.f, 0.f};
#pragma unroll
              for (int e = 0; e < 8; ++e) {
                float dz = df[e];
                if (p.gnb_silu) {
                  const float z = __builtin_fmaf(xf[e], sc[e], sf[e]);
                  const float sg = __builtin_amdgcn_rcpf(1.f + __expf(-z));
                  dz *= sg * (1.f + z * (1.f - sg));
                }
                const float dxh = dz * sc[e];
                a1[e >> 2] += dxh;
                a2[e >> 2] = __builtin_fmaf(dxh, xf[e] - mu[e >> 2], a2[e >> 2]);
              }
              gs[0] += a1[0]; gs[1] += a2[0]; gs[2] += a1[1]; gs[3] += a2[1];
            }
          }
        }
      }
    };
    auto emit_bits = [&]() {
#pragma unroll
      for (int it = 0; it < NIT; ++it) {
        const uint4 v = *reinterpret_cast<const uint4*>(wl + (it * RPI + rr) * PITCH + cch * 16);
        if (orows[it] >= 0 && col_ok) p.B2[(long long)orows[it] * p.ldb2 + (ncol >> 3)] = (unsigned char)dmx_pos8(v);
      }
    };
    if (BITS && (flags & EPI_MASKBITS)) {
      static_assert(FN == 2 || FN == 4, "sign-bit masks: wave tiles of 32 or 64 columns");
      const float sl = p.mask_slope;
      const bool span_ok = n0 + FN * 16 <= p.N;
      const int sh0 = 8 * (lq >> 1) + 4 * (lq & 1);
      uint32_t q0s[IB], q1s[IB];
      int orow_s[IB];
#pragma unroll
      for (int ii = 0; ii < IB; ++ii) {
        const int r = ii * 16 + lr;
        if (ident) { const int m = m0 + h * CH + r; orow_s[ii] = m < mend ? m : -1; }
        else orow_s[ii] = tab[r];
      }
      if (span_ok) {
#pragma unroll
        for (int ii = 0; ii < IB; ++ii) {
          const unsigned char* src = p.XB + (long long)(orow_s[ii] >= 0 ? orow_s[ii] : 0) * p.ldxb + (n0 >> 3);
          if constexpr (FN == 4) { const uint2 q = *reinterpret_cast<const uint2*>(src); q0s[ii] = q.x; q1s[ii] = q.y; }
          else { q0s[ii] = *reinterpret_cast<const uint32_t*>(src); q1s[ii] = 0xffffffffu; }
        }
#pragma unroll
        for (int ii = 0; ii < IB; ++ii) if (orow_s[ii] < 0) { q0s[ii] = 0xffffffffu; q1s[ii] = 0xffffffffu; }
      } else {
#pragma unroll
        for (int ii = 0; ii < IB; ++ii) {
          uint32_t q0 = 0xffffffffu, q1 = 0xffffffffu;
          if (orow_s[ii] >= 0) {
            const unsigned char* src = p.XB + (long long)orow_s[ii] * p.ldxb + (n0 >> 3);
            q0 = q1 = 0u;
#pragma unroll 1
            for (int k = 0; k < FN * 2; ++k) {
              const uint32_t by = n0 + k * 8 < p.N ? (uint32_t)src[k] : 0xffu;
              if (k < 4) q0 |= by << (8 * k); else q1 |= by << (8 * (k - 4));
            }
          }
          q0s[ii] = q0; q1s[ii] = q1;
        }
      }
#pragma unroll
      for (int ii = 0; ii < IB; ++ii) {
        const uint32_t q0 = q0s[ii], q1 = q1s[ii];
#pragma unroll
        for (int j = 0; j < FN; ++j) {
          const unsigned nib = ((j < 2 ? q0 : q1) >> (sh0 + 16 * (j & 1)));
          f32x4& a = acc[h * IB + ii][j];
          a[0] *= (nib & 1u) ? 1.f : sl; a[1] *= (nib & 2u) ? 1.f : sl; a[2] *= (nib & 4u) ? 1.f : sl; a[3] *= (nib & 8u) ? 1.f : sl;
        }
      }
    } else if (SOFT && (flags & EPI_SOFTBWD)) {
      const float* rv = p.rowbias + (p.sCo ? coff / p.sCo : 0ll) * (long long)p.M;
#pragma unroll
      for (int ii = 0; ii < IB; ++ii) {
        const int m = m0 + h * CH + ii * 16 + lr;
        const float dl = m < mend ? rv[m] : 0.f;
#pragma unroll
        for (int j = 0; j < FN; ++j) { f32x4& a = acc[h * IB + ii][j]; a[0] -= dl; a[1] -= dl; a[2] -= dl; a[3] -= dl; }
      }
      stage_in(p.X, p.ldx, [&](f32x4& a, float x0, float x1, float x2, float x3) { a[0] *= x0; a[1] *= x1; a[2] *= x2; a[3] *= x3; });
    } else if (flags & EPI_MASK) {
      const float sl = p.mask_slope;
      stage_in(p.X, p.ldx, [&](f32x4& a, float x0, float x1, float x2, float x3) {
        a[0] *= x0 > 0.f ? 1.f : sl; a[1] *= x1 > 0.f ? 1.f : sl; a[2] *= x2 > 0.f ? 1.f : sl; a[3] *= x3 > 0.f ? 1.f : sl;
      });
    }
    if (flags & (EPI_BIAS | EPI_ROWBIAS)) {
#pragma unroll
      for (int ii = 0; ii < IB; ++ii) {
        int bimg = 0;
        if (flags & EPI_ROWBIAS) {
          const int m = m0 + h * CH + ii * 16 + lr;
          bimg = (m < p.M ? m : 0) / HqWq;
        }
#pragma unroll
        for (int j = 0; j < FN; ++j) {
          const int n = n0 + j * 16 + lq * 4;
          if (n >= p.N) continue;
          f32x4& a = acc[h * IB + ii][j];
          if (flags & EPI_BIAS) {
            const float4 bb = bcol[j];
            a[0] += bb.x; a[1] += bb.y; a[2] += bb.z; a[3] += bb.w;
          }
          if (flags & EPI_ROWBIAS) {
            const float4 bb = *reinterpret_cast<const float4*>(p.rowbias + (long long)bimg * (p.ldrb ? p.ldrb : p.N) + n);
            a[0] += bb.x; a[1] += bb.y; a[2] += bb.z; a[3] += bb.w;
          }
        }
      }
    }
    if constexpr (GEGLU) {
#pragma unroll
      for (int ii = 0; ii < IB; ++ii)
#pragma unroll
        for (int j = 0; j < FN; j += 2) {
          f32x4& a = acc[h * IB + ii][j];
          const f32x4& g = acc[h * IB + ii][j + 1];
#pragma unroll
          for (int e = 0; e < 4; ++e) a[e] *= 0.5f * g[e] * erfcf(g[e] * -0.70710678118654752f);
        }
    }
    if ((flags & EPI_RESID) && use_rpre) {
      const float is = (flags & EPI_RESID_INV) ? p.resid_inv_slope : 1.f;
#pragma unroll
      for (int ii = 0; ii < IB; ++ii)
#pragma unroll
        for (int j = 0; j < FN; ++j) {
          const uint2 q = rpre[(h * IB + ii) * FN + j];
          const float x0 = alo(q.x), x1 = ahi(q.x), x2 = alo(q.y), x3 = ahi(q.y);
          f32x4& a = acc[h * IB + ii][j];
          a[0] += fminf(x0, x0 * is); a[1] += fminf(x1, x1 * is); a[2] += fminf(x2, x2 * is); a[3] += fminf(x3, x3 * is);
        }
    } else if (flags & EPI_RESID) {
      const float is = (flags & EPI_RESID_INV) ? p.resid_inv_slope : 1.f;
      stage_in(p.R, p.ldr, [&](f32x4& a, float x0, float x1, float x2, float x3) {
        a[0] += fminf(x0, x0 * is); a[1] += fminf(x1, x1 * is); a[2] += fminf(x2, x2 * is); a[3] += fminf(x3, x3 * is);
      });
    }
    if (p.alpha != 1.f) {
      const float al = p.alpha;
#pragma unroll
      for (int ii = 0; ii < IB; ++ii)
#pragma unroll
        for (int j = 0; j < FN; ++j) { f32x4& a = acc[h * IB + ii][j]; a[0] *= al; a[1] *= al; a[2] *= al; a[3] *= al; }
    }
    if (flags & EPI_ACCUM)
      stage_in(reinterpret_cast<const act_t*>(p.C), p.ldc, [&](f32x4& a, float x0, float x1, float x2, float x3) { a[0] += x0; a[1] += x1; a[2] += x2; a[3] += x3; });
    if (flags & EPI_TANH) {
#pragma unroll
      for (int ii = 0; ii < IB; ++ii)
#pragma unroll
        for (int j = 0; j < FN; ++j) { f32x4& a = acc[h * IB + ii][j]; a[0] = tanhf(a[0]); a[1] = tanhf(a[1]); a[2] = tanhf(a[2]); a[3] = tanhf(a[3]); }
    }
    if constexpr (ROWS) {
      if (flags & EPI_ROWSTATS) {
        float2* rso = reinterpret_cast<float2*>(p.rowstats_out);
        const int ns = p.nslots;
#pragma unroll
        for (int ii = 0; ii < IB; ++ii) {
          const int m = m0 + h * CH + ii * 16 + lr;
#pragma unroll
          for (int sl = 0; sl < FN / 2; ++sl) {
            float sv = 0.f, qv = 0.f;
#pragma unroll
            for (int jj = 0; jj < 2; ++jj) {
              const int j = sl * 2 + jj;
              const f32x4& a = acc[h * IB + ii][j];
              if (n0 + j * 16 + lq * 4 < p.N) {
                sv += (a[0] + a[1]) + (a[2] + a[3]);
                qv += (a[0] * a[0] + a[1] * a[1]) + (a[2] * a[2] + a[3] * a[3]);
              }
            }
            sv += __shfl_xor(sv, 16, 64); sv += __shfl_xor(sv, 32, 64);
            qv += __shfl_xor(qv, 16, 64); qv += __shfl_xor(qv, 32, 64);
            const int slot = (n0 >> 5) + sl;
            if (lq == 0 && m < mend && slot < ns) rso[(long long)m * ns + slot] = make_float2(sv, qv);
          }
        }
      }
    }
    const bool bits2 = (flags & EPI_BITS2) != 0;
    if (!(flags & EPI_NO_C)) {
      stage_out(reinterpret_cast<act_t*>(p.C), p.ldc, [&](const f32x4& a, float (&o)[4]) { o[0] = a[0]; o[1] = a[1]; o[2] = a[2]; o[3] = a[3]; });
      if constexpr (BITS) { if (bits2 && !(flags & EPI_LRELU2)) emit_bits(); }
      if constexpr (GNS) { if (flags & EPI_GNSTATS) emit_gn(); }
      if constexpr (GNB) { if ((flags & EPI_GNBWD) && m0 + h * CH < mend) emit_gnb(); }
      if constexpr (GNS || GNB) {
        if ((flags & (EPI_GNSTATS | EPI_GNBWD)) && m0 + h * CH < mend) {
#pragma unroll
          for (int o = CPR; o < 64; o <<= 1) {
#pragma unroll
            for (int k = 0; k < 4; ++k) gs[k] += __shfl_xor(gs[k], o, 64);
          }
          if (rr == 0 && col_ok) {
            const int nq = p.N >> 2, slots = (HqWq + GN_SLOT - 1) / GN_SLOT + 1;
            float* dst = p.gn_part + (((long long)gn_b0 * slots + (m0 + h * CH - gn_b0 * HqWq) / GN_SLOT) * nq + (ncol >> 2)) * 2;
            *reinterpret_cast<float4*>(dst) = make_float4(gs[0], gs[1], gs[2], gs[3]);
          }
        }
        gs[0] = gs[1] = gs[2] = gs[3] = 0.f;
      }
      DMX_LDS_SYNC();
    }
    if (flags & EPI_LRELU2) {
      const float sl = p.act_slope;
      stage_out(p.C2, p.ldc2, [&](const f32x4& a, float (&o)[4]) {
        o[0] = fmaxf(a[0], a[0] * sl); o[1] = fmaxf(a[1], a[1] * sl); o[2] = fmaxf(a[2], a[2] * sl); o[3] = fmaxf(a[3], a[3] * sl);
      });
      if constexpr (BITS) { if (bits2) emit_bits(); }
      DMX_LDS_SYNC();
    }
  });
#undef DMX_LDS_SYNC
}

template <int FM, int FN, int EM>
__device__ __forceinline__ void gemm_epilogue_lds(const GemmDesc& p, f32x4 (&acc)[FM][FN], int m0, int n0, int lane,
                                                  long long coff, int HqWq, char* wl, int mlimit = 0x7fffffff) {
  const uint2 none[FM * FN] = {};
  gemm_epilogue_lds_impl<FM, FN, EM>(p, acc, m0, n0, lane, coff, HqWq, wl, mlimit, none, false);
}

}
```

diffmusic_amd/csrc/hifigan.hip:

```cpp
#include "models.h"
#include "conv_pair.h"
#include <cstdlib>

struct SplitKScope {
  explicit SplitKScope(float* ws, size_t bytes, bool on) : on_(on && ws) { if (on_) dmx_gemm_set_splitk_workspace(ws, bytes); }
  ~SplitKScope() { if (on_) dmx_gemm_set_splitk_workspace(nullptr, 0); }
  bool on_;
};

struct Span { int a = 0, b = 0; bool empty() const { return b <= a; } };
static inline Span span_meet(Span x, Span y) { Span r{x.a > y.a ? x.a : y.a, x.b < y.b ? x.b : y.b}; if (r.empty()) r = Span{}; return r; }
static inline long long floor_div(long long a, long long b) { return a >= 0 ? a / b : -((-a + b - 1) / b); }
static inline long long ceil_div(long long a, long long b) { return -floor_div(-a, b); }

int dmx_conv_dead_rows_impl(int k, int dil, int pad, int stride, int transposed, int t_in, int t_out, int a, int b, int* lo, int* hi) {
  *lo = *hi = 0;
  if (k < 1 || dil < 1 || stride < 1 || pad < 0 || t_in < 1 || t_out < 1) return DMX_ERR_SHAPE;
  if (!transposed && stride != 1) return DMX_ERR_SHAPE;
  if (a < 0) a = 0;
  if (b > t_out) b = t_out;
  if (b <= a) return DMX_OK;
  const long long INF = 1ll << 40;
  const long long ea = a == 0 ? -INF : a, eb = b == t_out ? INF : b;
  long long l, h;
  if (!transposed) {
    l = ea - pad + (long long)(k - 1) * dil;
    h = eb - pad;
  } else {
    l = ceil_div(ea + pad, stride);
    h = ceil_div(eb - (k - 1) + pad, stride);
  }
  if (l < 0) l = 0;
  if (h > t_in) h = t_in;
  if (h > l) { *lo = (int)l; *hi = (int)h; }
  return DMX_OK;
}
static Span dead_in(const ConvLayer& L, Span d, int t_in, int t_out) {
  Span r;
  (void)dmx_conv_dead_rows_impl(L.kw, L.dil, L.pad_w, L.stride, L.transposed ? 1 : 0, t_in, t_out, d.a, d.b, &r.a, &r.b);
  return r;
}

struct DeadPlan {
  int B = 0, T = 0, s0 = 0, s1 = 0;
  bool on = false;
  Span wav;
  std::vector<Span> out, xs;
  std::vector<Span> xo, h, x;
  std::vector<int> skipped, total;
};

struct HifiGan : Model {
  dmx_hifigan_config cfg;
  DeadPlan plan;
  bool use_dead = false;
  static constexpr size_t kSplitKBytes = 32u << 20;
  float* splitk_ws = nullptr;
  ConvLayer conv_pre, conv_post;
  std::vector<ConvLayer> ups;
  std::vector<ConvLayer> c1, c2;
  int nk = 0, nd = 0, ns = 0;
  int B = 0, T = 0;
  std::vector<int> Ts;
  act_t* act_pre = nullptr;
  std::vector<act_t*> xs_a;
  std::vector<act_t*> ha, xa;
  std::vector<act_t*> act_out;
  std::vector<unsigned char*> hb, xb;
  std::vector<char> fused;
  float* wav8 = nullptr;
  bool have_tape = false;
  hipStream_t bstream[DMX_MAX_STAGES] = {};
  std::vector<hipEvent_t> events;
  size_t ev_next = 0;
  bool want_multi = true;
  hipEvent_t next_event() { hipEvent_t e = events[ev_next]; ev_next = (ev_next + 1) % events.size(); return e; }
  bool multi() const { return want_multi && !dry && !dmx_prof_is_active() && nk > 1; }
  bool multi_wanted() const { return want_multi && nk > 1; }

  int idx(int s, int k, int d) const { return (s * nk + k) * nd + d; }

  explicit HifiGan(const dmx_hifigan_config& c) : cfg(c) {
    kind = DMX_MODEL_HIFIGAN;
    ns = c.num_upsamples; nk = c.num_kernels; nd = c.num_dilations;
    const int C0 = c.upsample_initial_channel;
    conv_pre = make_conv1d(ps, "conv_pre", c.model_in_dim, C0, 7, 1, 3, true);
    for (int i = 0; i < ns; ++i) {
      const int s = c.upsample_rates[i], k = c.upsample_kernel_sizes[i];
      ups.push_back(make_convT1d(ps, "upsampler." + std::to_string(i), C0 >> i, C0 >> (i + 1), k, s, (k - s) / 2, true));
    }
    int ch = C0;
    for (int i = 0; i < ns; ++i) {
      ch = C0 >> (i + 1);
      for (int j = 0; j < nk; ++j) {
        const int k = c.resblock_kernel_sizes[j];
        const std::string pre = "resblocks." + std::to_string(i * nk + j);
        for (int d = 0; d < nd; ++d) {
          const int dil = c.resblock_dilation_sizes[j * nd + d];
          c1.push_back(make_conv1d(ps, pre + ".convs1." + std::to_string(d), ch, ch, k, dil, (k * dil - dil) / 2, true));
          c2.push_back(make_conv1d(ps, pre + ".convs2." + std::to_string(d), ch, ch, k, 1, (k - 1) / 2, true));
        }
      }
    }
    conv_post = make_conv1d(ps, "conv_post", ch, 1, 7, 1, 3, true);
    want_multi = getenv("DMX_MULTI_STREAM") != nullptr && getenv("DMX_SINGLE_STREAM") == nullptr;
    for (int k = 1; k < nk; ++k) (void)hipStreamCreateWithFlags(&bstream[k], hipStreamNonBlocking);
    events.resize(256);
    for (auto& e : events) (void)hipEventCreateWithFlags(&e, hipEventDisableTiming);
    splitk_ws = (float*)ps.dalloc(kSplitKBytes);
  }
  ~HifiGan() override {
    dmx_gemm_release_splitk_workspace(splitk_ws);
    for (int k = 1; k < nk; ++k) if (bstream[k]) (void)hipStreamDestroy(bstream[k]);
    for (auto& e : events) (void)hipEventDestroy(e);
  }

  int finalize(hipStream_t st) override {
    int rc = pack_layer(ps, conv_pre, st);
    for (auto& l : ups) if (rc == DMX_OK) rc = pack_layer(ps, l, st);
    for (auto& l : c1) if (rc == DMX_OK) rc = pack_layer(ps, l, st);
    for (auto& l : c2) if (rc == DMX_OK) rc = pack_layer(ps, l, st);
    if (rc == DMX_OK) rc = pack_layer(ps, conv_post, st);
    return rc;
  }

  bool step_is_fused(int id, int To) const {
    GemmDesc da, db;
    act_t* dummy = reinterpret_cast<act_t*>(size_t(256));
    unsigned char* dummyb = reinterpret_cast<unsigned char*>(size_t(256));
    Epi ea; ea.flags = EPI_LRELU2 | EPI_NO_C | EPI_BITS2; ea.act_slope = cfg.leaky_relu_slope; ea.B2 = dummyb;
    if (conv_fwd_1d_desc(c1[id], dummy, nullptr, B, To, ea, da) != DMX_OK) return false;
    Epi eb; eb.flags = EPI_RESID | EPI_RESID_INV | EPI_LRELU2 | EPI_NO_C | EPI_ACCUM; eb.R = dummy; eb.C2 = dummy;
    eb.resid_inv_slope = 1.f / cfg.leaky_relu_slope; eb.act_slope = cfg.leaky_relu_slope;
    if (conv_fwd_1d_desc(c2[id], nullptr, dummy, B, To, eb, db) != DMX_OK) return false;
    return dmx_conv_pair_eligible(&da, db);
  }

  void step_slabs(int id, int To, bool bwd, const PairDead& pd, int& skipped, int& total) const {
    GemmDesc da, db;
    act_t* dummy = reinterpret_cast<act_t*>(size_t(256));
    unsigned char* dummyb = reinterpret_cast<unsigned char*>(size_t(256));
    skipped = total = 0;
    if (!bwd) {
      Epi ea; ea.flags = EPI_LRELU2 | EPI_NO_C | EPI_BITS2; ea.act_slope = cfg.leaky_relu_slope; ea.B2 = dummyb;
      Epi eb; eb.flags = EPI_RESID | EPI_RESID_INV; eb.R = dummy; eb.resid_inv_slope = 1.f / cfg.leaky_relu_slope;
      if (conv_fwd_1d_desc(c1[id], dummy, nullptr, B, To, ea, da) != DMX_OK || conv_fwd_1d_desc(c2[id], nullptr, dummy, B, To, eb, db) != DMX_OK) return;
    } else {
      Epi ea; ea.flags = EPI_MASKBITS; ea.mask_slope = cfg.leaky_relu_slope; ea.XB = dummyb;
      Epi eb; eb.flags = EPI_RESID | EPI_MASKBITS; eb.mask_slope = cfg.leaky_relu_slope; eb.R = dummy; eb.XB = dummyb;
      if (conv_bwd_1d_desc(c2[id], dummy, dummy, B, To, ea, da) != DMX_OK || conv_bwd_1d_desc(c1[id], dummy, dummy, B, To, eb, db) != DMX_OK) return;
    }
    dmx_conv_pair_slabs(&da, db, &pd, &skipped, &total);
  }
  bool stage_all_fused(int s, int To) const {
    bool all = nk <= 3;
    for (int k = 0; k < nk; ++k) for (int d = 0; d < nd; ++d) all = all && step_is_fused(idx(s, k, d), To);
    return all;
  }
  PairDead dead_fwd(int id) const {
    const Span w = span_meet(plan.xo[id], plan.h[id]);
    PairDead pd; pd.skip0 = w.a; pd.skip1 = w.b;
    return pd;
  }
  PairDead dead_bwd(int s, int id, int d) const {
    const Span w = d == 0 ? plan.xs[s] : plan.x[id];
    PairDead pd; pd.skip0 = w.a; pd.skip1 = w.b; pd.zero0 = plan.xo[id].a; pd.zero1 = plan.xo[id].b;
    return pd;
  }

  void make_plan(int T_, int s0, int s1) {
    if (plan.B == B && plan.T == T_ && plan.s0 == s0 && plan.s1 == s1 && (int)plan.out.size() == ns) return;
    plan = DeadPlan();
    plan.B = B; plan.T = T_; plan.s0 = s0; plan.s1 = s1;
    plan.out.assign(ns, Span{}); plan.xs.assign(ns, Span{});
    plan.xo.assign(ns * nk * nd, Span{}); plan.h.assign(ns * nk * nd, Span{}); plan.x.assign(ns * nk * nd, Span{});
    plan.skipped.assign(ns, 0); plan.total.assign(ns, 0);
    std::vector<int> len(ns);
    int t = T_;
    for (int i = 0; i < ns; ++i) { t = conv_out_len(ups[i], t); len[i] = t; }
    const int Tout = ns ? len[ns - 1] : T_;
    plan.wav = span_meet(Span{s0, s1}, Span{0, Tout});
    if (plan.wav.empty() || ns == 0) return;
    Span cur = dead_in(conv_post, plan.wav, Tout, Tout);
    for (int s = ns - 1; s >= 0; --s) {
      const int To = len[s], Tin = s ? len[s - 1] : T_;
      plan.out[s] = cur;
      Span xs{0, To};
      for (int k = 0; k < nk; ++k) {
        Span o = cur;
        for (int d = nd - 1; d >= 0; --d) {
          const int id = idx(s, k, d);
          plan.xo[id] = o;
          plan.h[id] = dead_in(c2[id], o, To, To);
          plan.x[id] = span_meet(dead_in(c1[id], plan.h[id], To, To), o);
          o = plan.x[id];
        }
        xs = span_meet(xs, o);
      }
      plan.xs[s] = xs;
      cur = dead_in(ups[s], xs, Tin, To);
    }
    if (multi_wanted()) return;
    int any = 0;
    for (int s = 0; s < ns; ++s) {
      if (!stage_all_fused(s, len[s])) continue;
      for (int k = 0; k < nk; ++k)
        for (int d = 0; d < nd; ++d) {
          const int id = idx(s, k, d);
          int sk, tot;
          step_slabs(id, len[s], false, dead_fwd(id), sk, tot);
          plan.skipped[s] += sk; plan.total[s] += tot;
          step_slabs(id, len[s], true, dead_bwd(s, id, d), sk, tot);
          plan.skipped[s] += sk; plan.total[s] += tot;
        }
      any += plan.skipped[s];
    }
    plan.on = any > 0;
    if (!plan.on) plan.skipped.assign(ns, 0);
  }

  int out_len(int T_) const {
    int t = T_;
    for (int i = 0; i < ns; ++i) t = conv_out_len(ups[i], t);
    return t;
  }

  int forward(const act_t* mel, float* wav, int B_, int T_, void* ws, size_t ws_bytes, hipStream_t st, int s0 = 0, int s1 = 0) {
    if (cfg.model_in_dim & 7) return DMX_ERR_SHAPE;
    dry = (ws == nullptr);
    B = B_;
    if (!dry) {
      use_dead = false;
      if (s1 > s0) { make_plan(T_, s0, s1); use_dead = plan.on; }
    }
    const bool dead = use_dead && !dry;
    SplitKScope sk_scope(splitk_ws, kSplitKBytes, !dry && !multi_wanted());
    arena.reset(ws, dry ? (size_t)-1 : ws_bytes);
    T = T_;
    Ts.assign(ns, 0);
    xs_a.assign(ns, nullptr); act_out.assign(ns, nullptr);
    ha.assign(ns * nk * nd, nullptr); xa.assign(ns * nk * nd, nullptr);
    hb.assign(ns * nk * nd, nullptr); xb.assign(ns * nk * nd, nullptr);
    fused.assign(ns * nk * nd, 0);
    const float slope = cfg.leaky_relu_slope;
    auto bits = [&](size_t rows, int C) { return (unsigned char*)arena.raw(rows * (size_t)(C >> 3)); };
    act_pre = arena.bf((size_t)B * T * conv_pre.Cop);
    {
      Epi e; e.flags = EPI_LRELU2 | EPI_NO_C; e.act_slope = slope; e.C2 = act_pre;
      RUN(conv_fwd_1d(conv_pre, mel, act_pre, B, T, e, st));
    }
    const act_t* cur_act = act_pre;
    int Tin = T;
    for (int s = 0; s < ns; ++s) {
      const ConvLayer& up = ups[s];
      const int To = conv_out_len(up, Tin), C = up.Cop;
      const size_t n = (size_t)B * To * C;
      Ts[s] = To;
      xs_a[s] = arena.bf(n);
      act_out[s] = arena.bf(n);
      unsigned char* xs_b = nullptr;
      for (int k = 0; k < nk; ++k)
        for (int d = 0; d < nd; ++d) {
          const int id = idx(s, k, d);
          fused[id] = step_is_fused(id, To) ? 1 : 0;
          xa[id] = d == 0 ? xs_a[s] : arena.bf(n);
          if (fused[id]) {
            hb[id] = bits((size_t)B * To, C);
            if (d == 0) { if (!xs_b) xs_b = bits((size_t)B * To, C); xb[id] = xs_b; }
            else xb[id] = bits((size_t)B * To, C);
          } else {
            ha[id] = arena.bf(n);
          }
        }
      const size_t mk = arena.mark();
      act_t* sum = arena.bf(n);
      {
        Epi e; e.flags = EPI_LRELU2 | EPI_NO_C; e.act_slope = slope; e.C2 = xs_a[s];
        if (xs_b) { e.flags |= EPI_BITS2; e.B2 = xs_b; }
        RUN(conv_fwd_1d(up, cur_act, xs_a[s], B, Tin, e, st));
      }
      const float next_slope = (s == ns - 1) ? 0.01f : slope;
      const bool mt = multi();
      bool all_fused = nk <= 3;
      for (int k = 0; k < nk; ++k) for (int d = 0; d < nd; ++d) all_fused = all_fused && fused[idx(s, k, d)] != 0;
      if (all_fused && !mt) {
        for (int d = 0; d < nd; ++d) {
          GemmDesc da[DMX_MAX_STAGES], db[DMX_MAX_STAGES];
          const GemmDesc* pa[DMX_MAX_STAGES]; const GemmDesc* pb[DMX_MAX_STAGES];
          PairDead pd[DMX_MAX_STAGES];
          for (int k = 0; k < nk; ++k) {
            const int id = idx(s, k, d);
            if (dead) pd[k] = dead_fwd(id);
            {
              Epi e; e.flags = EPI_LRELU2 | EPI_NO_C | EPI_BITS2; e.act_slope = slope; e.B2 = hb[id];
              RUN(conv_fwd_1d_desc(c1[id], xa[id], ha[id], B, To, e, da[k]));
            }
            if (d < nd - 1) {
              const int idn = idx(s, k, d + 1);
              act_t* xn = xa[idn];
              Epi e; e.flags = EPI_RESID | EPI_RESID_INV | EPI_LRELU2 | EPI_NO_C | EPI_BITS2; e.R = xa[id]; e.resid_inv_slope = 1.f / slope;
              e.act_slope = slope; e.C2 = xn; e.B2 = xb[idn];
              RUN(conv_fwd_1d_desc(c2[id], ha[id], xn, B, To, e, db[k]));
            } else {
              Epi e; e.flags = EPI_RESID | EPI_RESID_INV; e.R = xa[id]; e.resid_inv_slope = 1.f / slope; e.alpha = 1.f / nk;
              if (k > 0) e.flags |= EPI_ACCUM;
              if (k == nk - 1) { e.flags |= EPI_LRELU2 | EPI_NO_C; e.act_slope = next_slope; e.C2 = act_out[s]; }
              RUN(conv_fwd_1d_desc(c2[id], ha[id], sum, B, To, e, db[k]));
            }
            pa[k] = &da[k]; pb[k] = &db[k];
          }
          if (dry) continue;
          for (int k = 0; k < nk; ++k)
            if (!dmx_conv_pair_eligible(&da[k], db[k])) {
              dmx_set_error("hifigan: resblock step %d was planned as fused but the pair kernel refuses it", idx(s, k, d));
              return DMX_ERR_STATE;
            }
          if (d < nd - 1) RUN(dmx_conv_pair_group_launch(nk, pa, pb, st, dead ? pd : nullptr));
          else for (int k = 0; k < nk; ++k) RUN(conv_pair_run(da[k], db[k], st, dead ? &pd[k] : nullptr));
        }
        arena.release(mk);
        cur_act = act_out[s];
        Tin = To;
        continue;
      }
      hipEvent_t fin_prev = nullptr;
      if (mt) {
        hipEvent_t e0 = next_event();
        (void)hipEventRecord(e0, st);
        for (int k = 1; k < nk; ++k) (void)hipStreamWaitEvent(bstream[k], e0, 0);
      }
      for (int k = 0; k < nk; ++k) {
        hipStream_t sk = (mt && k > 0) ? bstream[k] : st;
        for (int d = 0; d < nd; ++d) {
          const int id = idx(s, k, d);
          const bool fz = fused[id] != 0;
          GemmDesc da, db;
          {
            Epi e; e.flags = EPI_LRELU2 | EPI_NO_C; e.act_slope = slope;
            if (fz) { e.flags |= EPI_BITS2; e.B2 = hb[id]; } else e.C2 = ha[id];
            RUN(conv_fwd_1d_desc(c1[id], xa[id], ha[id], B, To, e, da));
          }
          if (d < nd - 1) {
            const int idn = idx(s, k, d + 1);
            act_t* xn = xa[idn];
            Epi e; e.flags = EPI_RESID | EPI_RESID_INV | EPI_LRELU2 | EPI_NO_C; e.R = xa[id]; e.resid_inv_slope = 1.f / slope;
            e.act_slope = slope; e.C2 = xn;
            if (fused[idn]) { e.flags |= EPI_BITS2; e.B2 = xb[idn]; }
            RUN(conv_fwd_1d_desc(c2[id], ha[id], xn, B, To, e, db));
          } else {
            Epi e; e.flags = EPI_RESID | EPI_RESID_INV; e.R = xa[id]; e.resid_inv_slope = 1.f / slope; e.alpha = 1.f / nk;
            if (k > 0) e.flags |= EPI_ACCUM;
            if (k == nk - 1) { e.flags |= EPI_LRELU2 | EPI_NO_C; e.act_slope = next_slope; e.C2 = act_out[s]; }
            RUN(conv_fwd_1d_desc(c2[id], ha[id], sum, B, To, e, db));
          }
          if (!dry && fz && !dmx_conv_pair_eligible(&da, db)) {
            dmx_set_error("hifigan: resblock step %d was planned as fused but the pair kernel refuses it", id);
            return DMX_ERR_STATE;
          }
          if (d == nd - 1 && mt && fin_prev) (void)hipStreamWaitEvent(sk, fin_prev, 0);
          RUN(conv_pair_run(da, db, sk));
          if (d == nd - 1 && mt) { fin_prev = next_event(); (void)hipEventRecord(fin_prev, sk); }
        }
      }
      if (mt && fin_prev) (void)hipStreamWaitEvent(st, fin_prev, 0);
      arena.release(mk);
      cur_act = act_out[s];
      Tin = To;
    }
    const int Tout = Tin;
    wav8 = arena.f32((size_t)B * Tout * 8);
    CHECK_WS("hifigan");
    {
      Epi e; e.flags = EPI_F32OUT | EPI_TANH;
      RUN(conv_fwd_1d(conv_post, cur_act, wav8, B, Tout, e, st));
    }
    if (dead) RUN(dmx_gather_col_f32_dead(wav8, wav, (long long)B * Tout, 8, 0, Tout, plan.wav.a, plan.wav.b, st));
    else RUN(dmx_gather_col_f32(wav8, wav, (long long)B * Tout, 8, 0, st));
    have_tape = true;
    return DMX_OK;
  }

  int backward(const float* dwav, act_t* dmel, hipStream_t st) {
    if (!have_tape && !dry) { dmx_set_error("hifigan backward without forward"); return DMX_ERR_STATE; }
    SplitKScope sk_scope(splitk_ws, kSplitKBytes, !dry && !multi_wanted());
    const float slope = cfg.leaky_relu_slope;
    const int Tout = Ts[ns - 1];
    const size_t mk0 = arena.mark();
    act_t* gz = arena.bf((size_t)B * Tout * 8);
    const int Clast = ups[ns - 1].Cop;
    act_t* g = arena.bf((size_t)B * Tout * Clast);
    CHECK_WS("hifigan");
    const bool dead = use_dead && !dry;
    if (dead) RUN(dmx_tanh_bwd_pad8_dead(dwav, wav8, gz, (long long)B * Tout, Tout, plan.wav.a, plan.wav.b, st));
    else RUN(dmx_tanh_bwd_pad8(dwav, wav8, gz, (long long)B * Tout, st));
    {
      Epi e; e.flags = EPI_MASK; e.X = act_out[ns - 1]; e.mask_slope = 0.01f; e.alpha = 1.f / nk;
      RUN(conv_bwd_1d(conv_post, gz, g, B, Tout, e, st));
    }
    for (int s = ns - 1; s >= 0; --s) {
      const int To = Ts[s], Tin = s == 0 ? T : Ts[s - 1], C = ups[s].Cop;
      const size_t n = (size_t)B * To * C;
      act_t* gxs = arena.bf(n);
      act_t* ghk[DMX_MAX_STAGES];
      act_t* gAB[DMX_MAX_STAGES][2];
      for (int k = 0; k < nk; ++k) { ghk[k] = arena.bf(n); gAB[k][0] = arena.bf(n); gAB[k][1] = arena.bf(n); }
      const int Cin = ups[s].Cip;
      act_t* gprev = arena.bf((size_t)B * Tin * Cin);
      CHECK_WS("hifigan");
      const bool mt = multi();
      hipEvent_t fin_prev = nullptr;
      bool all_fused = nk <= 3;
      for (int k = 0; k < nk; ++k) for (int d = 0; d < nd; ++d) all_fused = all_fused && fused[idx(s, k, d)] != 0;
      if (all_fused && !mt) {
        const act_t* gcs[DMX_MAX_STAGES];
        for (int k = 0; k < nk; ++k) gcs[k] = g;
        if (dead && !plan.xs[s].empty() &&
            hipMemset2DAsync(gxs + (size_t)plan.xs[s].a * C, (size_t)To * C * sizeof(act_t), 0, (size_t)(plan.xs[s].b - plan.xs[s].a) * C * sizeof(act_t),
                             (size_t)B, st) != hipSuccess) {
          dmx_set_error("hifigan: clearing the dead rows of a stage gradient failed");
          return DMX_ERR_LAUNCH;
        }
        for (int d = nd - 1; d >= 0; --d) {
          GemmDesc da[DMX_MAX_STAGES], db[DMX_MAX_STAGES];
          const GemmDesc* pa[DMX_MAX_STAGES]; const GemmDesc* pb[DMX_MAX_STAGES];
          act_t* dsts[DMX_MAX_STAGES];
          PairDead pd[DMX_MAX_STAGES];
          for (int k = 0; k < nk; ++k) {
            const int id = idx(s, k, d);
            if (dead) pd[k] = dead_bwd(s, id, d);
            {
              Epi e; e.mask_slope = slope; e.flags = EPI_MASKBITS; e.XB = hb[id];
              RUN(conv_bwd_1d_desc(c2[id], gcs[k], ghk[k], B, To, e, da[k]));
            }
            Epi e; e.flags = EPI_RESID | EPI_MASKBITS; e.mask_slope = slope; e.R = gcs[k]; e.XB = xb[id];
            if (d == 0) { dsts[k] = gxs; if (k > 0) e.flags |= EPI_ACCUM; }
            else dsts[k] = (gcs[k] == gAB[k][0]) ? gAB[k][1] : gAB[k][0];
            RUN(conv_bwd_1d_desc(c1[id], ghk[k], dsts[k], B, To, e, db[k]));
            pa[k] = &da[k]; pb[k] = &db[k];
          }
          if (!dry) {
            if (d > 0) RUN(dmx_conv_pair_group_launch(nk, pa, pb, st, dead ? pd : nullptr));
            else for (int k = 0; k < nk; ++k) RUN(conv_pair_run(da[k], db[k], st, dead ? &pd[k] : nullptr));
          }
          for (int k = 0; k < nk; ++k) gcs[k] = dsts[k];
        }
      } else {
      if (mt) {
        hipEvent_t e0 = next_event();
        (void)hipEventRecord(e0, st);
        for (int k = 1; k < nk; ++k) (void)hipStreamWaitEvent(bstream[k], e0, 0);
      }
      for (int k = 0; k < nk; ++k) {
        hipStream_t sk = (mt && k > 0) ? bstream[k] : st;
        const act_t* gc = g;
        for (int d = nd - 1; d >= 0; --d) {
          const int id = idx(s, k, d);
          GemmDesc da, db;
          {
            Epi e; e.mask_slope = slope;
            if (fused[id]) { e.flags = EPI_MASKBITS; e.XB = hb[id]; } else { e.flags = EPI_MASK; e.X = ha[id]; }
            RUN(conv_bwd_1d_desc(c2[id], gc, ghk[k], B, To, e, da));
          }
          Epi e; e.flags = EPI_RESID; e.mask_slope = slope; e.R = gc;
          if (fused[id]) { e.flags |= EPI_MASKBITS; e.XB = xb[id]; } else { e.flags |= EPI_MASK; e.X = xa[id]; }
          act_t* dst;
          if (d == 0) {
            dst = gxs;
            if (k > 0) e.flags |= EPI_ACCUM;
            if (mt && fin_prev) (void)hipStreamWaitEvent(sk, fin_prev, 0);
          } else {
            dst = (gc == gAB[k][0]) ? gAB[k][1] : gAB[k][0];
          }
          RUN(conv_bwd_1d_desc(c1[id], ghk[k], dst, B, To, e, db));
          RUN(conv_pair_run(da, db, sk));
          if (d == 0 && mt) { fin_prev = next_event(); (void)hipEventRecord(fin_prev, sk); }
          gc = dst;
        }
      }
      }
      if (mt && fin_prev) (void)hipStreamWaitEvent(st, fin_prev, 0);
      {
        Epi e; e.flags = EPI_MASK; e.mask_slope = slope;
        if (s > 0) { e.X = act_out[s - 1]; e.alpha = 1.f / nk; } else { e.X = act_pre; }
        RUN(conv_bwd_1d(ups[s], gxs, gprev, B, Tin, e, st));
      }
      g = gprev;
    }
    {
      Epi e;
      RUN(conv_bwd_1d(conv_pre, g, dmel, B, T, e, st));
    }
    arena.release(mk0);
    return DMX_OK;
  }
};

Model* dmx_make_hifigan(const dmx_hifigan_config* c) { return new HifiGan(*c); }
int dmx_hifigan_out_len_impl(Model* m, int T) { return static_cast<HifiGan*>(m)->out_len(T); }
int dmx_hifigan_fwd_impl(Model* m, const act_t* mel, float* wav, int B, int T, void* ws, size_t wsb, hipStream_t st) {
  return static_cast<HifiGan*>(m)->forward(mel, wav, B, T, ws, wsb, st);
}
int dmx_hifigan_fwd_dead_impl(Model* m, const act_t* mel, float* wav, int B, int T, int s0, int s1, void* ws, size_t wsb, hipStream_t st) {
  return static_cast<HifiGan*>(m)->forward(mel, wav, B, T, ws, wsb, st, s0, s1);
}
int dmx_hifigan_dead_plan_impl(Model* m, int* skipped, int* total, int* lo, int* hi, int n) {
  HifiGan* h = static_cast<HifiGan*>(m);
  for (int s = 0; s < n && s < h->ns; ++s) {
    const bool have = h->use_dead && s < (int)h->plan.out.size();
    if (skipped) skipped[s] = have ? h->plan.skipped[s] : 0;
    if (total) total[s] = have ? h->plan.total[s] : 0;
    if (lo) lo[s] = have ? h->plan.out[s].a : 0;
    if (hi) hi[s] = have ? h->plan.out[s].b : 0;
  }
  return h->ns;
}
int dmx_hifigan_bwd_impl(Model* m, const float* dwav, act_t* dmel, hipStream_t st) {
  return static_cast<HifiGan*>(m)->backward(dwav, dmel, st);
}
size_t dmx_hifigan_ws_impl(Model* m, int B, int T) {
  HifiGan* h = static_cast<HifiGan*>(m);
  h->arena.peak = 0;
  h->forward(nullptr, nullptr, B, T, nullptr, 0, nullptr);
  h->backward(nullptr, nullptr, nullptr);
  h->have_tape = false;
  h->dry = false;
  return h->arena.peak + 256;
}
```

diffmusic_amd/csrc/models.h:

```cpp
#pragma once
#include "layers.h"
#include "../../include/diffmusic_hip.h"

enum { DMX_MODEL_HIFIGAN = 1, DMX_MODEL_VAE = 2, DMX_MODEL_UNET = 3, DMX_MODEL_HTSAT = 4, DMX_MODEL_VAE_ENC = 5 };

struct Model {
  int kind = 0;
  ParamStore ps;
  Arena arena;
  bool finalized = false;
  bool dry = false;
  virtual ~Model() { ps.free_all(); }
  virtual int finalize(hipStream_t st) = 0;
};
struct dmx_model { Model* impl; };

#define RUN(expr) do { if (!dry) { int rc_ = (expr); if (rc_ != DMX_OK) return rc_; } } while (0)
#define CHECK_WS(name) do { if (arena.overflow) { dmx_set_error(name " workspace too small: need %zu bytes", arena.peak); return DMX_ERR_WORKSPACE; } } while (0)

Model* dmx_make_hifigan(const dmx_hifigan_config* c);
int dmx_hifigan_out_len_impl(Model* m, int T);
int dmx_hifigan_fwd_impl(Model* m, const act_t* mel, float* wav, int B, int T, void* ws, size_t wsb, hipStream_t st);
int dmx_hifigan_bwd_impl(Model* m, const float* dwav, act_t* dmel, hipStream_t st);
int dmx_hifigan_fwd_dead_impl(Model* m, const act_t* mel, float* wav, int B, int T, int s0, int s1, void* ws, size_t wsb, hipStream_t st);
int dmx_hifigan_dead_plan_impl(Model* m, int* skipped, int* total, int* lo, int* hi, int n);
int dmx_conv_dead_rows_impl(int k, int dil, int pad, int stride, int transposed, int t_in, int t_out, int a, int b, int* lo, int* hi);
size_t dmx_hifigan_ws_impl(Model* m, int B, int T);

Model* dmx_make_vae(const dmx_vae_config* c);
size_t dmx_vae_ws_impl(Model* m, int B, int h, int w);
int dmx_vae_fwd_impl(Model* m, const float* z, float zs, act_t* mel, float* mel32, int B, int h, int w, int keep, void* ws, size_t wsb,
                     hipStream_t st);
int dmx_vae_bwd_impl(Model* m, const act_t* dmel, float zs, float* dz, hipStream_t st);
Model* dmx_make_vae_encoder(const dmx_vae_config* c);
size_t dmx_vae_enc_ws_impl(Model* m, int B, int T, int F);
int dmx_vae_enc_fwd_impl(Model* m, const float* mel, float log_floor, float* moments, int B, int T, int F, void* ws, size_t wsb, hipStream_t st);
int dmx_latent_init_impl(const float* moments, float* mean, float* logvar, float* x, const float* eps, const float* noise, int B, int L, int P,
                         float sqrt_abar, float scaling_factor, float sqrt_1m_abar, hipStream_t st);
int dmx_conv2d_raw_impl(const float* w_host, const float* b_host, const act_t* x, act_t* y, int B, int Hi, int Wi, int Ci, int Co, int k,
                        int stride, int pad_lo, int pad_hi, hipStream_t st);
Model* dmx_make_unet(const dmx_unet_config* c);
size_t dmx_unet_ws_impl(Model* m, int B, int h, int w, int n0, int n1);
int dmx_unet_fwd_impl(Model* m, const float* x, const float* t, const float* cls, float* eps, int B, int h, int w, void* ws, size_t wsb,
                      hipStream_t st, const float* c0, int n0, const float* c1, int n1, const float* bias1);

Model* dmx_make_htsat(const dmx_htsat_config* c);
size_t dmx_htsat_ws_impl(Model* m, int B, int frames);
int dmx_htsat_fwd_impl(Model* m, const float* mel, int B, int frames, float* feat, int keep, void* ws, size_t wsb, hipStream_t st);
int dmx_htsat_bwd_impl(Model* m, const float* dfeat, const float* scale, float* dmel, hipStream_t st);
void dmx_htsat_dims_impl(Model* m, int* tokens, int* channels);
size_t dmx_htsat_tape_impl(Model* m, int stage, int block, int which, const act_t** p);
int dmx_gram_fwd_impl(const float* F, float* G, int B, int T, int C, hipStream_t st);
int dmx_gram_bwd_impl(const float* F, const float* dG, float* dF, int B, int T, int C, hipStream_t st);
```

diffmusic_amd/engine.py:

```python
import ctypes as C
import os
import torch
from . import _lib as L
from . import ops
from ._ctypes_ops import _stream
from .weights import synth_state_dict

HIFIGAN_DEFAULT = dict(model_in_dim=64, upsample_initial_channel=1024, upsample_rates=[5, 4, 2, 2, 2],
                       upsample_kernel_sizes=[16, 16, 8, 4, 4], resblock_kernel_sizes=[3, 7, 11],
                       resblock_dilation_sizes=[[1, 3, 5]] * 3, leaky_relu_slope=0.1, sampling_rate=16000)
VAE_DEFAULT = dict(latent_channels=8, out_channels=1, block_out_channels=[128, 256, 512], layers_per_block=2,
                   norm_num_groups=32, scaling_factor=0.9227914214134216, eps=1e-6)
UNET_MUSICLDM_DEFAULT = dict(in_channels=8, out_channels=8, block_out_channels=[128, 256, 384, 640],
                             layers_per_block=2, attention_heads=8, norm_num_groups=32,
                             down_attn=[0, 1, 1, 1], up_attn=[1, 1, 1, 0], class_embed_dim=512, attn_cross_dims=[0])
UNET_AUDIOLDM2_DEFAULT = dict(UNET_MUSICLDM_DEFAULT, class_embed_dim=0, attn_cross_dims=[0, 768, 1024])


def _fill(arr, vals):
    for i, v in enumerate(vals):
        arr[i] = int(v)


class _Engine:
    kind = "generic"

    def __init__(self, handle, config, device):
        if not handle:
            L.check(-1, "model create")
        self._h = C.c_void_p(handle)
        self.cfg = dict(config)
        self.device = torch.device(device)
        self._ws = {}
        self._finalized = False

    def __del__(self):
        try:
            if getattr(self, "_h", None):
                L.lib().dmx_model_destroy(self._h)
                self._h = None
        except Exception:
            pass

    def param_specs(self):
        lib = L.lib()
        out = []
        for i in range(lib.dmx_model_num_params(self._h)):
            nd = lib.dmx_model_param_ndim(self._h, i)
            out.append((lib.dmx_model_param_name(self._h, i).decode(),
                        tuple(lib.dmx_model_param_dim(self._h, i, d) for d in range(nd))))
        return out

    def _stride_of(self, name):
        return 1

    def synth_state_dict(self, seed=0):
        return synth_state_dict(self.param_specs(), seed, self.kind, self._stride_of)

    allow_unexpected = ()

    def load_state_dict(self, sd, strict=False):
        lib = L.lib()
        from .weights import check_manifest
        specs = self.param_specs()
        check_manifest(specs, sd if strict else {n: sd[n] for n, _ in specs if n in sd}, f"{self.kind} ({type(self).__name__})",
                       self.allow_unexpected)
        for name, shape in specs:
            t = sd[name].detach().to(torch.float32).contiguous().cpu()
            L.check(lib.dmx_model_load_param(self._h, name.encode(), C.c_void_p(t.data_ptr()), t.numel()), name)
        with torch.cuda.device(self.device):
            L.check(lib.dmx_model_finalize(self._h, _stream()), "finalize")
            torch.cuda.synchronize()
        self._finalized = True
        return self

    def _workspace(self, key, nbytes):
        ws = self._ws.get("buf")
        if ws is None or ws.numel() < nbytes:
            self._ws.clear()
            ws = torch.empty(int(nbytes), dtype=torch.uint8, device=self.device)
            self._ws["buf"] = ws
        return ws


class HifiGanEngine(_Engine):
    kind = "hifigan"
    allow_unexpected = ("mean", "scale")

    def __init__(self, config=None, device="cuda"):
        cfg = dict(HIFIGAN_DEFAULT)
        cfg.update(config or {})
        c = L.HifiGanConfig()
        c.model_in_dim, c.upsample_initial_channel = cfg["model_in_dim"], cfg["upsample_initial_channel"]
        c.num_upsamples = len(cfg["upsample_rates"])
        _fill(c.upsample_rates, cfg["upsample_rates"])
        _fill(c.upsample_kernel_sizes, cfg["upsample_kernel_sizes"])
        c.num_kernels = len(cfg["resblock_kernel_sizes"])
        _fill(c.resblock_kernel_sizes, cfg["resblock_kernel_sizes"])
        c.num_dilations = len(cfg["resblock_dilation_sizes"][0])
        _fill(c.resblock_dilation_sizes, [d for row in cfg["resblock_dilation_sizes"] for d in row])
        c.leaky_relu_slope = cfg["leaky_relu_slope"]
        super().__init__(L.lib().dmx_hifigan_create(C.byref(c)), cfg, device)
        self.dead_span_enabled = os.environ.get("DMX_NO_DEAD_SPAN", "0") in ("", "0")

    def _stride_of(self, name):
        return self.cfg["upsample_rates"][int(name.split(".")[1])]

    @property
    def config(self):
        from types import SimpleNamespace
        return SimpleNamespace(**self.cfg)

    def out_len(self, frames):
        return L.lib().dmx_hifigan_out_len(self._h, frames)

    def __call__(self, mel):
        return self.forward(mel.to(device=self.device, dtype=L.act_dtype()).contiguous())

    def forward(self, mel, dead=None):
        assert mel.dtype == L.act_dtype() and mel.is_cuda and mel.is_contiguous()
        B, T, _ = mel.shape
        lib = L.lib()
        ws = self._workspace(("h", B, T), lib.dmx_hifigan_workspace_bytes(self._h, B, T))
        self._shape = (B, T)
        live = dead is not None and self.dead_span_enabled and int(dead[1]) > int(dead[0])
        s0, s1 = (int(dead[0]), int(dead[1])) if live else (0, 0)
        return ops.hip.hifigan_fwd(self._h.value, mel, ws, s0, s1)

    def dead_plan(self):
        n = len(self.cfg["upsample_rates"])
        flat = list(ops.hip.hifigan_dead_plan(self._h.value, n))
        return [dict(skipped=flat[4 * s], total=flat[4 * s + 1], span=(flat[4 * s + 2], flat[4 * s + 3])) for s in range(n)]

    def backward(self, dwav):
        _, T = self._shape
        assert dwav.dtype == torch.float32 and dwav.is_contiguous()
        return ops.hip.hifigan_bwd(self._h.value, dwav, T, self.cfg["model_in_dim"])


class VaeDecoderEngine(_Engine):
    kind = "vae"
    allow_unexpected = ("encoder.", "quant_conv.")

    def __init__(self, config=None, device="cuda"):
        cfg = dict(VAE_DEFAULT)
        cfg.update(config or {})
        c = L.VaeConfig()
        c.latent_channels, c.out_channels = cfg["latent_channels"], cfg["out_channels"]
        c.num_blocks = len(cfg["block_out_channels"])
        _fill(c.block_out_channels, cfg["block_out_channels"])
        c.layers_per_block, c.norm_num_groups, c.eps = cfg["layers_per_block"], cfg["norm_num_groups"], cfg["eps"]
        super().__init__(L.lib().dmx_vae_decoder_create(C.byref(c)), cfg, device)
        self.scale_factor = 2 ** (c.num_blocks - 1)
        self.scaling_factor = cfg["scaling_factor"]

    @property
    def config(self):
        from types import SimpleNamespace
        return SimpleNamespace(**self.cfg)

    def decode(self, z):
        from types import SimpleNamespace
        _, m32 = self.decode_hip(z.to(device=self.device, dtype=torch.float32).contiguous(), 1.0, keep_state=False, want_f32=True)
        return SimpleNamespace(sample=m32.unsqueeze(1))

    def decode_hip(self, z, z_scale=1.0, keep_state=True, want_f32=False):
        assert z.dtype == torch.float32 and z.is_cuda and z.is_contiguous()
        B, _, h, w = z.shape
        lib = L.lib()
        ws = self._workspace(("v", B, h, w), lib.dmx_vae_workspace_bytes(self._h, B, h, w))
        self._shape = (B, h, w)
        mel, mel32 = ops.hip.vae_dec_fwd(self._h.value, z, float(z_scale), bool(keep_state), bool(want_f32), self.scale_factor, ws)
        return (mel, mel32) if want_f32 else mel

    def backward(self, dmel, z_scale=1.0):
        assert dmel.dtype == L.act_dtype() and dmel.is_contiguous()
        return ops.hip.vae_dec_bwd(self._h.value, dmel, float(z_scale), self.cfg["latent_channels"], self.scale_factor)


class LatentDistribution:

    def __init__(self, moments, h, w):
        self.moments, self._hw = moments, (int(h), int(w))
        self.mean, self.logvar, _ = ops.hip.latent_init(moments, h, w, None, None, 1.0, 1.0, 0.0, False)

    def mode(self, scale=1.0):
        if scale == 1.0:
            return self.mean
        return ops.hip.latent_init(self.moments, *self._hw, None, None, 1.0, float(scale), 0.0, True)[2]

    def sample(self, generator=None, scale=1.0):
        from .torch_utils import randn_tensor
        eps = randn_tensor(self.mean.shape, generator=generator, device=self.mean.device, dtype=torch.float32).contiguous()
        return ops.hip.latent_init(self.moments, *self._hw, eps, None, 1.0, float(scale), 0.0, True)[2]


class VaeEncoderEngine(_Engine):
    kind = "vae_enc"
    allow_unexpected = ("decoder.", "post_quant_conv.")

    def __init__(self, config=None, device="cuda"):
        cfg = dict(VAE_DEFAULT)
        cfg.update(config or {})
        c = L.VaeConfig()
        c.latent_channels, c.out_channels = cfg["latent_channels"], cfg["out_channels"]
        c.num_blocks = len(cfg["block_out_channels"])
        _fill(c.block_out_channels, cfg["block_out_channels"])
        c.layers_per_block, c.norm_num_groups, c.eps = cfg["layers_per_block"], cfg["norm_num_groups"], cfg["eps"]
        super().__init__(L.lib().dmx_vae_encoder_create(C.byref(c)), cfg, device)
        self.scale_factor = 2 ** (c.num_blocks - 1)
        self.scaling_factor = cfg["scaling_factor"]

    @property
    def config(self):
        from types import SimpleNamespace
        return SimpleNamespace(**self.cfg)

    def encode_hip(self, mel, log_floor=0.0):
        assert mel.dtype == torch.float32 and mel.is_cuda and mel.is_contiguous() and mel.dim() == 3
        B, T, F = mel.shape
        nbytes = L.lib().dmx_vae_encoder_workspace_bytes(self._h, B, T, F)
        if nbytes == 0:
            L.check(-1, "vae encoder workspace")
        ws = self._workspace(("e", B, T, F), nbytes)
        return ops.hip.vae_enc_fwd(self._h.value, mel, float(log_floor), self.cfg["latent_channels"], self.scale_factor, ws)

    def encode(self, mel, log_floor=0.0):
        from types import SimpleNamespace
        if mel.dim() == 4:
            mel = mel.squeeze(1)
        mel = mel.to(device=self.device, dtype=torch.float32).contiguous()
        s = self.scale_factor
        return SimpleNamespace(latent_dist=LatentDistribution(self.encode_hip(mel, log_floor), mel.shape[1] // s, mel.shape[2] // s))


class UNetEngine(_Engine):
    kind = "unet"

    def __init__(self, config=None, device="cuda"):
        cfg = dict(UNET_MUSICLDM_DEFAULT)
        cfg.update(config or {})
        c = L.UNetConfig()
        c.in_channels, c.out_channels = cfg["in_channels"], cfg["out_channels"]
        c.num_blocks = len(cfg["block_out_channels"])
        _fill(c.block_out_channels, cfg["block_out_channels"])
        c.layers_per_block, c.attention_heads = cfg["layers_per_block"], cfg["attention_heads"]
        c.norm_num_groups = cfg["norm_num_groups"]
        _fill(c.down_attn, cfg["down_attn"])
        _fill(c.up_attn, cfg["up_attn"])
        c.class_embed_dim = cfg["class_embed_dim"]
        acd = [int(d or 0) for d in cfg.get("attn_cross_dims", [0])]
        c.num_attn_per_layer = len(acd)
        _fill(c.attn_cross_dims, acd)
        self._n_ctx = sum(1 for d in acd if d > 0)
        super().__init__(L.lib().dmx_unet_create(C.byref(c)), cfg, device)

# ... 90 lines not shown
```

include/diffmusic_hip.h:

```cpp
#ifndef DIFFMUSIC_HIP_H
#define DIFFMUSIC_HIP_H
#include <stddef.h>
#include <stdint.h>

#ifdef __cplusplus
extern "C" {
#endif

#define DMX_ABI_VERSION 4
#define DMX_MAX_STAGES 8

typedef struct dmx_model dmx_model;

typedef struct dmx_hifigan_config {
  int model_in_dim;
  int upsample_initial_channel;
  int num_upsamples;
  int upsample_rates[DMX_MAX_STAGES];
  int upsample_kernel_sizes[DMX_MAX_STAGES];
  int num_kernels;
  int resblock_kernel_sizes[DMX_MAX_STAGES];
  int num_dilations;
  int resblock_dilation_sizes[DMX_MAX_STAGES * DMX_MAX_STAGES];
  float leaky_relu_slope;
} dmx_hifigan_config;

typedef struct dmx_vae_config {
  int latent_channels;
  int out_channels;
  int num_blocks;
  int block_out_channels[DMX_MAX_STAGES];
  int layers_per_block;
  int norm_num_groups;
  float eps;
} dmx_vae_config;

typedef struct dmx_unet_config {
  int in_channels, out_channels;
  int num_blocks;
  int block_out_channels[DMX_MAX_STAGES];
  int layers_per_block;
  int attention_heads;
  int norm_num_groups;
  int down_attn[DMX_MAX_STAGES];
  int up_attn[DMX_MAX_STAGES];
  int class_embed_dim;
  int num_attn_per_layer;
  int attn_cross_dims[4];
} dmx_unet_config;

int dmx_abi_version(void);
int dmx_act_dtype(void);
const char* dmx_last_error(void);

dmx_model* dmx_hifigan_create(const dmx_hifigan_config* cfg);
dmx_model* dmx_vae_decoder_create(const dmx_vae_config* cfg);
dmx_model* dmx_unet_create(const dmx_unet_config* cfg);
void dmx_model_destroy(dmx_model* m);
int dmx_model_num_params(const dmx_model* m);
const char* dmx_model_param_name(const dmx_model* m, int i);
size_t dmx_model_param_numel(const dmx_model* m, int i);
int dmx_model_param_ndim(const dmx_model* m, int i);
int dmx_model_param_dim(const dmx_model* m, int i, int d);
int dmx_model_load_param(dmx_model* m, const char* name, const float* data_host, size_t numel);
int dmx_model_finalize(dmx_model* m, void* stream);

int dmx_hifigan_out_len(const dmx_model* m, int frames);
size_t dmx_hifigan_workspace_bytes(dmx_model* m, int batch, int frames);
int dmx_hifigan_fwd(dmx_model* m, const uint16_t* mel, float* wav, int batch, int frames, void* ws, size_t ws_bytes,
                    void* stream);
int dmx_hifigan_bwd(dmx_model* m, const float* dwav, uint16_t* dmel, void* stream);
int dmx_hifigan_fwd_dead(dmx_model* m, const uint16_t* mel, float* wav, int batch, int frames, int s0, int s1, void* ws,
                         size_t ws_bytes, void* stream);
int dmx_hifigan_dead_plan(dmx_model* m, int* skipped, int* total, int* lo, int* hi, int n);
int dmx_conv_dead_rows(int k, int dil, int pad, int stride, int transposed, int t_in, int t_out, int a, int b, int* lo, int* hi);

size_t dmx_vae_workspace_bytes(dmx_model* m, int batch, int h, int w);
int dmx_vae_decode_fwd(dmx_model* m, const float* z, float z_scale, uint16_t* mel, float* mel_f32, int batch, int h, int w,
                       int keep_state, void* ws, size_t ws_bytes, void* stream);
int dmx_vae_decode_bwd(dmx_model* m, const uint16_t* dmel, float z_scale, float* dz, void* stream);

dmx_model* dmx_vae_encoder_create(const dmx_vae_config* cfg);
size_t dmx_vae_encoder_workspace_bytes(dmx_model* m, int batch, int frames, int bins);
int dmx_vae_encode_fwd(dmx_model* m, const float* mel, float log_floor, float* moments, int batch, int frames, int bins, void* ws,
                       size_t ws_bytes, void* stream);
int dmx_latent_init(const float* moments, float* mean, float* logvar, float* x, const float* eps, const float* noise, int batch,
                    int latent_channels, int hw, float sqrt_abar, float scaling_factor, float sqrt_1m_abar, void* stream);

size_t dmx_unet_workspace_bytes(dmx_model* m, int batch, int h, int w);
int dmx_unet_fwd(dmx_model* m, const float* x, const float* t, const float* class_labels, float* eps, int batch, int h,
                 int w, void* ws, size_t ws_bytes, void* stream);
int dmx_unet_fwd_ctx(dmx_model* m, const float* x, const float* t, const float* class_labels, const float* ctx0, int n0,
                     const float* ctx1, int n1, const float* bias1, float* eps, int batch, int h, int w, void* ws,
                     size_t ws_bytes, void* stream);
size_t dmx_unet_workspace_bytes_ctx(dmx_model* m, int batch, int h, int w, int n0, int n1);

typedef struct dmx_htsat_config {
  int spec_size;
  int num_mel_bins;
  int patch_size;
  int embed_dim;
  int window_size;
  int num_stages;
  int depths[4];
  int num_heads[4];
  float ln_eps;
  float bn_eps;
} dmx_htsat_config;
dmx_model* dmx_htsat_create(const dmx_htsat_config* cfg);
int dmx_htsat_feature_dims(dmx_model* m, int* tokens, int* channels);
size_t dmx_htsat_workspace_bytes(dmx_model* m, int batch, int frames);
int dmx_htsat_fwd(dmx_model* m, const float* mel, int batch, int frames, float* feat, int keep_state, void* ws, size_t ws_bytes, void* stream);
int dmx_htsat_bwd(dmx_model* m, const float* dfeat, const float* scale, float* dmel, void* stream);
size_t dmx_htsat_tape_raw(dmx_model* m, int stage, int block, int which, void* dst, size_t dst_elems, void* stream);
int dmx_gram_fwd(const float* F, float* G, int batch, int tokens, int channels, void* stream);
int dmx_gram_bwd(const float* F, const float* dG, float* dF, int batch, int tokens, int channels, void* stream);

typedef struct dmx_audio dmx_audio;
dmx_audio* dmx_audio_create(int n_fft, int hop, int n_mels, int window_hann, const float* fb_host);
void dmx_audio_destroy(dmx_audio* a);
int dmx_audio_num_frames(const dmx_audio* a, int L);
int dmx_audio_num_bins(const dmx_audio* a);
size_t dmx_audio_state_bytes(const dmx_audio* a, int batch, int L);
int dmx_audio_transform_fwd(dmx_audio* a, const float* wav, long long wav_stride, float* mel_out, void* state, int batch, int L,
                            int power2, int to_db, float lo, float hi, void* stream);
int dmx_audio_transform_bwd(dmx_audio* a, const float* dmel, float* dwav, long long dwav_stride, void* state, int batch, int L,
                            int power2, int to_db, float lo, float hi, int accumulate, void* stream);
int dmx_audio_is_fused(const dmx_audio* a, int L);
int dmx_audio_guidance_fwd(dmx_audio* a, const float* wav, long long wav_stride, const float* mask, const float* ref, long long ref_stride,
                           float* mel_out, void* state, int batch, int L, int power2, int to_db, float lo, float hi, void* stream);
int dmx_audio_guidance_bwd(dmx_audio* a, const float* wav, long long wav_stride, const float* mask, const float* ref, long long ref_stride,
                           float gscale, float* loss, float* dwav, long long dwav_stride, int Lfull, void* state, int batch, int L,
                           int power2, int to_db, float lo, float hi, void* stream);
int dmx_audio_guidance_fwd_ex(dmx_audio* a, const float* wav, long long wav_stride, const float* mask, const float* ref, long long ref_stride,
                              float* mel_out, void* state, int batch, int L, int power2, int to_db, float lo, float hi, const float* add,
                              long long add_stride, const float* addmag, float noise_scale, void* stream);
int dmx_audio_guidance_bwd_ex(dmx_audio* a, const float* wav, long long wav_stride, const float* mask, const float* ref, long long ref_stride,
                              float gscale, float* loss, float* dwav, long long dwav_stride, int Lfull, void* state, int batch, int L,
                              int power2, int to_db, float lo, float hi, const float* add, long long add_stride, const float* addmag,
                              float noise_scale, void* stream);
int dmx_audio_guidance_fwd_shaped(dmx_audio* a, const float* wav, long long wav_stride, const float* mask, const float* ref, long long ref_stride,
                                  float* mel_out, void* state, int batch, int L, int power2, int to_db, float lo, float hi, const float* add,
                                  long long add_stride, const float* addmag, float noise_scale, const float* thr, void* stream);
int dmx_audio_guidance_bwd_shaped(dmx_audio* a, const float* wav, long long wav_stride, const float* mask, const float* ref, long long ref_stride,
                                  float gscale, float* loss, float* dwav, long long dwav_stride, int Lfull, void* state, int batch, int L,
                                  int power2, int to_db, float lo, float hi, const float* add, long long add_stride, const float* addmag,
                                  float noise_scale, const float* thr, void* stream);
int dmx_clip_fwd(const float* x, long long x_stride, const float* thr, float* y, long long y_stride, int batch, int L, void* stream);
int dmx_clip_bwd(const float* dy, long long dy_stride, const float* wav, long long wav_stride, const float* thr, float* dwav,
                 long long dwav_stride, int batch, int L, int Lfull, void* stream);
int dmx_declip_project(const float* xhat, long long xhat_stride, const float* meas, long long meas_stride, const float* thr, float* out,
                       long long out_stride, int batch, int L, void* stream);
int dmx_drc_fwd(const float* x, long long x_stride, float* y, long long y_stride, float* state, unsigned char* tape, int batch, int L,
                float threshold_db, float slope, float knee_db, float a_att, float a_rel, float makeup_db, void* stream);
int dmx_drc_bwd(const float* dy, long long dy_stride, const float* x, long long x_stride, const float* state, const unsigned char* tape,
                float* work, float* dx, long long dx_stride, int batch, int L, int Lfull, float threshold_db, float slope, float knee_db,
                float a_att, float a_rel, float makeup_db, void* stream);
int dmx_drc_fwd_p(const float* x, long long x_stride, float* y, long long y_stride, float* state, unsigned char* tape, const float* theta,
                  int batch, int L, float knee_db, void* stream);
int dmx_drc_bwd_p(const float* dy, long long dy_stride, const float* x, long long x_stride, const float* state, const unsigned char* tape,
                  const float* theta, float* work, float* bq0, float* dx, long long dx_stride, int batch, int L, int Lfull, float knee_db,
                  void* stream);
int dmx_drc_pgrad(const float* state, const unsigned char* tape, const float* work, const float* bq0, const float* theta, float* part,
                  int batch, int L, float knee_db, void* stream);
int dmx_drc_update(const float* part, float* phi, float* m, float* v, float* theta, int batch, int L, int k, const double* lr, double beta1,
                   double beta2, double eps, float knee_db, const double* lo, const double* hi, void* stream);
int dmx_warp_fwd(const float* x, long long x_stride, const float* delay, long long delay_stride, float* y, int batch, int L, void* stream);
int dmx_warp_bwd(const float* dy, const float* delay, long long delay_stride, float* dx, int batch, int L, int full, void* stream);
int dmx_warp_wgrad(const float* dy, const float* x, long long x_stride, const float* delay, long long delay_stride, float* part, int batch,
                   int L, void* stream);
int dmx_warp_update(const float* part, float* coarse, float* m, float* v, float* fine, int batch, int L, int knot_stride, int k, double lr,
                    double beta1, double beta2, double eps, double max_delay, int anchor, void* stream);
int dmx_click_detect(const float* y, long long y_stride, float* a, float* e, float* sigma, unsigned char* flags, float* r, int batch, int L,
                     float threshold, float sigma_floor, void* stream);
int dmx_click_mask(const unsigned char* flags, float* mask, int* masked, int batch, int L, int guard, void* stream);
int dmx_mask_rows(const float* x, long long x_stride, const float* mask, long long mask_stride, float* y, int batch, int L, int Ly,
                  void* stream);
int dmx_declick_blend(const float* x, long long x_stride, const float* y, long long y_stride, const float* mask, long long mask_stride,
                      float* out, int batch, int L, int fade, void* stream);
int dmx_noise_add(const float* y, const float* z, float* out, long long n, float scale, void* stream);
int dmx_audio_stft_mag(dmx_audio* a, const float* wav, long long wav_stride, float* mag, void* state, int batch, int L, void* stream);
int dmx_audio_stft_mag_bwd(dmx_audio* a, const float* dmag, float* dwav, long long dwav_stride, void* state, int batch, int L,
                           int accumulate, void* stream);
int dmx_audio_tf_frames(int L);
int dmx_audio_tf_gain(dmx_audio* a, const float* x, long long x_stride, const float* gain, long long gain_clip_stride, float* out,
                      long long out_stride, int batch, int L, int full, void* stream);
int dmx_audio_tf_curve(dmx_audio* a, const float* x, long long x_stride, const float* curve, long long curve_clip_stride, float* out,
                       long long out_stride, int batch, int L, int full, void* stream);
int dmx_audio_tf_wgrad_segments(int L);
int dmx_audio_tf_wgrad(dmx_audio* a, const float* x, long long x_stride, const float* dy, long long dy_stride, float* partials, int batch, int L,
                       void* stream);
int dmx_audio_eq_update(const float* partials, int segments, float* g, float* m, float* v, int batch, int k, double lr, double beta1,
                        double beta2, double eps, int normalize, void* stream);
int dmx_audio_melscale(dmx_audio* a, const float* mag, float* mel_out, int batch, int frames, float lo, float hi, void* stream);
int dmx_mask_apply(const float* x, long long x_stride, const float* mask, float* y, long long y_stride, int batch, int L, int Ly,
                   void* stream);
int dmx_l2_loss(const float* ref, long long ref_stride, const float* pred, float* loss, float* dpred, int batch, long long n,
                float gscale, void* stream);
int dmx_track_stitch_fwd(const float* wav, long long wav_stride, float* track, const int* starts_host, int windows, int L, int R, int T,
                         void* stream);
int dmx_track_stitch_bwd(const float* dtrack, float* dwav, long long dwav_stride, const int* starts_host, int windows, int L, int R, int T,
                         int full, void* stream);
int dmx_stem_mix_fwd(const float* wav, long long wav_stride, float* mix, const float* gains_host, int stems, int groups, int L, void* stream);
int dmx_stem_mix_bwd(const float* dmix, float* dwav, long long dwav_stride, const float* gains_host, int stems, int groups, int L, int full,
                     void* stream);
int dmx_stem_project(const float* x, long long x_stride, const float* y, float* out, const float* gains_host, int stems, int L, void* stream);
int dmx_grad_normalize(float* x, float* inv_scale, int batch, long long n, float target, void* stream);

int dmx_fir_fwd(const float* in, long long in_stride, const float* h, float* out, long long out_stride, int batch, int Lin, int Lout,
                int taps, int orig, int new_, int off, void* stream);
int dmx_fir_bwd(const float* dout, long long dout_stride, const float* h, const float* h_rev, float* din, long long din_stride, int batch,
                int Lin, int Lout, int taps, int orig, int new_, int off, void* stream);
int dmx_fir_clip_fwd(const float* in, long long in_stride, const float* h, float* out, long long out_stride, int batch, int Lin, int Lout,
                     int taps, void* stream);
int dmx_fir_clip_bwd(const float* dout, long long dout_stride, const float* h, const float* h_rev, float* din, long long din_stride, int batch,
                     int Lin, int Lout, int taps, void* stream);
size_t dmx_fir_wgrad_workspace_floats(int batch, int Lout, int taps);
int dmx_fir_wgrad(const float* dy, long long dy_stride, const float* x, long long x_stride, float* partials, size_t partial_floats, int batch,
                  int L, int Lout, int taps, void* stream);
int dmx_ir_update(const float* partials, int segments, float* h, float* h_rev, float* m, float* v, int batch, int taps, double lr, double beta1,
                  double beta2, double eps, int k, void* stream);

#define DMX_SCHED_DDIM 0
#define DMX_SCHED_DPS 1
#define DMX_SCHED_MPGD 2
#define DMX_SCHED_DSG 3
#define DMX_SCHED_DIFFMUSIC 4
int dmx_sched_pred_x0(const float* x, const float* eps, float* x0, long long n, float alpha_t, void* stream);
int dmx_sched_pred_x0_ex(const float* x, const float* model_output, float* x0, long long n, float alpha_t, int prediction_type, float clip_range,
                         void* stream);
int dmx_sched_cfg_combine(const float* eps2, float* out, long long n, float scale, void* stream);
int dmx_sched_step(int mode, const float* x, const float* eps, const float* x0, const float* g0, const float* inv_scale,
                   const float* noise, float* prev, float* x0_out, float* grad_out, int batch, int n, float alpha_t, float alpha_prev,
                   float sigma, float rate, float eps_small, int global_norm, void* stream);
int dmx_sched_step_ex(int mode, const float* x, const float* eps, const float* x0, const float* g0, const float* inv_scale,
                      const float* noise, float* prev, float* x0_out, float* grad_out, int batch, int n, float alpha_t, float alpha_prev,
                      float sigma, float rate, float eps_small, int global_norm, int prediction_type, float clip_range, void* stream);

int dmx_randn_philox(float* out, int batch, long long n, const unsigned long long* seeds_host, unsigned long long offset, void* stream);

void dmx_prof_begin(void);
int dmx_prof_end(double* total_ms, double* total_flops);
int dmx_prof_dominant(double* ms, double* flops, double* bytes);

int dmx_gemm_raw(const void* desc, size_t desc_bytes, void* stream);
int dmx_flash_attn_raw(const void* q, const void* k, const void* v, void* o, const float* colbias, int B, int Nq, int Nk, int ldv,
                       int C, int heads, float scale, void* stream);
int dmx_flash_attn_ld_raw(const void* q, const void* k, const void* v, void* o, const float* colbias, int B, int Nq, int Nk, int ldq,
                          int ldk, int ldv, int C, int heads, float scale, int* qt_out, void* stream);
int dmx_softmax_raw(const float* S, void* P, const float* colbias, long long rows, int N, long long lds, long long ldp, int rows_per_bias,
                    void* stream);
int dmx_softmax_act_raw(const void* S, void* P, const float* colbias, long long rows, int N, long long ldp, int rows_per_bias, void* stream);
int dmx_transpose_raw(const void* in, void* out, int R, int C, long long ldi, long long ldo, int Z, int Zi, long long sIo, long long sIi,
                      long long sOo, long long sOi, void* stream);
int dmx_rowdot_raw(const void* a, const void* b, float* out, long long rows, int C, long long lda, long long ldb, void* stream);
int dmx_layernorm_raw(const void* x, void* y, const float* gamma, const float* beta, int rows, int C, float eps, void* stream);
int dmx_geglu_raw(const void* x, void* y, long long rows, int I, void* stream);
int dmx_gemm_splitk_workspace(void* ws, size_t bytes);
int dmx_conv_pair_raw(const void* desc_a, const void* desc_b, size_t desc_bytes, void* stream);
int dmx_conv_pair_dead_raw(const void* desc_a, const void* desc_b, size_t desc_bytes, const int* dead, int* skipped, int* total, void* stream);
int dmx_conv_pair_group_raw(int n, const void* descs_a, const void* descs_b, size_t desc_bytes, void* stream);
int dmx_conv_pair_group_dead_raw(int n, const void* descs_a, const void* descs_b, size_t desc_bytes, const int* dead, void* stream);
size_t dmx_groupnorm_scratch_floats(int B, int C, int G);
int dmx_groupnorm_raw(const void* x, void* y, const float* gamma, const float* beta, float* stats, float* scale, float* shift,
                      float* partial, int B, int P, int C, int G, float eps, int silu, void* stream);
size_t dmx_groupnorm_part_floats(int B, int P, int N);
int dmx_groupnorm_parts_raw(const void* x, void* y, const float* gamma, const float* beta, float* stats, float* scale, float* shift,
                            int B, int P, int C, int G, float eps, int silu, int nreg, float* const* part, const int* geom, void* stream);
int dmx_gemm_last_tile_rows_raw(void);
int dmx_conv2d_raw(const float* w_host, const float* b_host, const void* x, void* y, int B, int Hi, int Wi, int Ci, int Co, int k, int stride,
                   int pad_lo, int pad_hi, void* stream);
int dmx_groupnorm_bwd_raw(const void* x, const void* dy, const void* add, void* dx, const float* stats, const float* scale, const float* shift,
                          float* k0, float* k1, float* partial, int B, int P, int C, int G, int silu, int nreg, float* const* part,
                          const int* geom, void* stream);

#ifdef __cplusplus
}
#endif
#endif
```

Measured before the change: 27.13 steps/s (weak scaling: one step advances a batch of 8 clips on one GPU; value = K / wall x 1 GPU(s)).

## Sum HiFi-GAN resblock branches in registers within one fused conv-pair launch

Adds a branch-summing conv-pair kernel for the last dilation of each HiFi-GAN resblock stage. One workgroup runs the 2-3 kernel branches in sequence and keeps a running fp16-packed tile in registers instead of writing each branch's output and reading it back for accumulation. This removes per-branch launches and the intermediate sum buffer traffic. In exchange it adds register pressure, forces the smallest common row tile across branches, and narrows the dead-row handling. It is enabled by default and can be turned off with an environment variable.

```diff
diff --git a/diffmusic_amd/_lib.py b/diffmusic_amd/_lib.py
--- a/diffmusic_amd/_lib.py
+++ b/diffmusic_amd/_lib.py
@@ -81,6 +81,7 @@
     "dmx_hifigan_fwd_dead": (C.c_int, [C.c_void_p, C.c_void_p, C.c_void_p, C.c_int, C.c_int, C.c_int, C.c_int, C.c_void_p, C.c_size_t,
                                        C.c_void_p]),
     "dmx_hifigan_dead_plan": (C.c_int, [C.c_void_p, C.POINTER(C.c_int), C.POINTER(C.c_int), C.POINTER(C.c_int), C.POINTER(C.c_int), C.c_int]),
+    "dmx_hifigan_set_branch_sum": (C.c_int, [C.c_void_p, C.c_int]),
     "dmx_conv_dead_rows": (C.c_int, [C.c_int] * 9 + [C.POINTER(C.c_int), C.POINTER(C.c_int)]),
     "dmx_vae_workspace_bytes": (C.c_size_t, [C.c_void_p, C.c_int, C.c_int, C.c_int]),
     "dmx_vae_decode_fwd": (C.c_int, [C.c_void_p, C.c_void_p, C.c_float, C.c_void_p, C.c_void_p, C.c_int, C.c_int, C.c_int,
@@ -120,6 +121,7 @@
     "dmx_geglu_raw": (C.c_int, [C.c_void_p, C.c_void_p, C.c_longlong, C.c_int, C.c_void_p]),
     "dmx_gemm_splitk_workspace": (C.c_int, [C.c_void_p, C.c_size_t]),
     "dmx_conv_pair_raw": (C.c_int, [C.c_void_p, C.c_void_p, C.c_size_t, C.c_void_p]),
+    "dmx_conv_pair_sum_raw": (C.c_int, [C.c_int, C.c_void_p, C.c_void_p, C.c_size_t, C.POINTER(C.c_int), C.c_void_p]),
     "dmx_conv_pair_group_raw": (C.c_int, [C.c_int, C.c_void_p, C.c_void_p, C.c_size_t, C.c_void_p]),
     "dmx_conv_pair_dead_raw": (C.c_int, [C.c_void_p, C.c_void_p, C.c_size_t, C.POINTER(C.c_int), C.POINTER(C.c_int), C.POINTER(C.c_int), C.c_void_p]),
     "dmx_conv_pair_group_dead_raw": (C.c_int, [C.c_int, C.c_void_p, C.c_void_p, C.c_size_t, C.POINTER(C.c_int), C.c_void_p]),
@@ -223,7 +225,8 @@
                "dmx_stem_mix_fwd", "dmx_stem_mix_bwd", "dmx_stem_project", "dmx_audio_tf_gain", "dmx_audio_tf_frames",
                "dmx_audio_tf_curve", "dmx_audio_tf_wgrad_segments", "dmx_audio_tf_wgrad", "dmx_audio_eq_update", "dmx_drc_fwd", "dmx_drc_bwd",
                "dmx_warp_fwd", "dmx_warp_bwd", "dmx_warp_wgrad", "dmx_warp_update", "dmx_drc_fwd_p", "dmx_drc_bwd_p", "dmx_drc_pgrad",
-               "dmx_drc_update", "dmx_click_detect", "dmx_click_mask", "dmx_mask_rows", "dmx_declick_blend")
+               "dmx_drc_update", "dmx_click_detect", "dmx_click_mask", "dmx_mask_rows", "dmx_declick_blend",
+               "dmx_hifigan_set_branch_sum")
 
 _lib = None
 
diff --git a/diffmusic_amd/csrc/capi.hip b/diffmusic_amd/csrc/capi.hip
--- a/diffmusic_amd/csrc/capi.hip
+++ b/diffmusic_amd/csrc/capi.hip
@@ -73,6 +73,11 @@
   if (!m || !m->impl || m->impl->kind != DMX_MODEL_HIFIGAN) { dmx_set_error("wrong model handle"); return -1; }
   return dmx_hifigan_dead_plan_impl(m->impl, skipped, total, lo, hi, n);
 }
+int dmx_hifigan_set_branch_sum(dmx_model* m, int on) {
+  if (!m || !m->impl || m->impl->kind != DMX_MODEL_HIFIGAN) { dmx_set_error("wrong model handle"); return DMX_ERR_STATE; }
+  if (on >= 0) dmx_hifigan_set_branch_sum_impl(m->impl, on);
+  return dmx_hifigan_get_branch_sum_impl(m->impl);
+}
 int dmx_conv_dead_rows(int k, int dil, int pad, int stride, int transposed, int t_in, int t_out, int a, int b, int* lo, int* hi) {
   if (!lo || !hi) return DMX_ERR_STATE;
   return dmx_conv_dead_rows_impl(k, dil, pad, stride, transposed, t_in, t_out, a, b, lo, hi);
@@ -209,6 +214,20 @@
 }
 
 static PairDead pair_dead_of(const int* d) { PairDead pd; pd.skip0 = d[0]; pd.skip1 = d[1]; pd.zero0 = d[2]; pd.zero1 = d[3]; return pd; }
+
+int dmx_conv_pair_sum_raw(int n, const void* descs_a, const void* descs_b, size_t desc_bytes, const int* dead, void* stream) {
+  if (desc_bytes != sizeof(GemmDesc)) { dmx_set_error("GemmDesc size mismatch: %zu vs %zu", desc_bytes, sizeof(GemmDesc)); return DMX_ERR_SHAPE; }
+  if (n < 2 || n > 3 || !descs_a || !descs_b) { dmx_set_error("conv pair sum: 2 or 3 branches"); return DMX_ERR_SHAPE; }
+  const GemmDesc* a = reinterpret_cast<const GemmDesc*>(descs_a);
+  const GemmDesc* b = reinterpret_cast<const GemmDesc*>(descs_b);
+  const GemmDesc* pa[3]; const GemmDesc* pb[3];
+  PairDead pd[3];
+  for (int j = 0; j < n; ++j) { pa[j] = a + j; pb[j] = b + j; if (dead) pd[j] = pair_dead_of(dead + 4 * j); }
+  if (!dmx_conv_pair_sum_eligible(n, pa, pb)) { dmx_set_error("branches not handled by the branch-summing pair launch"); return DMX_ERR_SHAPE; }
+  const int rc = dmx_conv_pair_sum_launch(n, pa, pb, ST(stream), dead ? pd : nullptr);
+  if (rc == DMX_ERR_SHAPE) dmx_set_error("dead rows not handled by the branch-summing pair launch (zero rows need the residual to be stage a's input)");
+  return rc;
+}
 
 int dmx_conv_pair_dead_raw(const void* desc_a, const void* desc_b, size_t desc_bytes, const int* dead, int* skipped, int* total, void* stream) {
   if (skipped) *skipped = 0;
diff --git a/diffmusic_amd/csrc/conv_pair.h b/diffmusic_amd/csrc/conv_pair.h
--- a/diffmusic_amd/csrc/conv_pair.h
+++ b/diffmusic_amd/csrc/conv_pair.h
@@ -8,6 +8,8 @@
 bool dmx_conv_pair_eligible(const GemmDesc* a, const GemmDesc& b);
 int dmx_conv_pair_launch(const GemmDesc* a, const GemmDesc& b, hipStream_t st, const PairDead* dead = nullptr);
 int dmx_conv_pair_group_launch(int n, const GemmDesc* const* a, const GemmDesc* const* b, hipStream_t st, const PairDead* dead = nullptr);
+bool dmx_conv_pair_sum_eligible(int n, const GemmDesc* const* a, const GemmDesc* const* b);
+int dmx_conv_pair_sum_launch(int n, const GemmDesc* const* a, const GemmDesc* const* b, hipStream_t st, const PairDead* dead = nullptr);
 void dmx_conv_pair_slabs(const GemmDesc* a, const GemmDesc& b, const PairDead* dead, int* skipped, int* total);
 
 int dmx_prof_open(hipStream_t st);
diff --git a/diffmusic_amd/csrc/conv_pair.hip b/diffmusic_amd/csrc/conv_pair.hip
--- a/diffmusic_amd/csrc/conv_pair.hip
+++ b/diffmusic_amd/csrc/conv_pair.hip
@@ -17,6 +17,7 @@
   int a_tape_bits_only;
   int skip_q0, skip_n;
   int z0, z1;
+  int own_q0, own_q1;
 };
 
 #ifdef DMX_PAIR_STAMPS
@@ -97,8 +98,9 @@
                : "memory");
 }
 
-template <int C>
-__device__ __forceinline__ void pair_body(const PairParams& P, char* smem, int bid, const int nwg) {
+template <int C, bool SUM>
+__device__ __forceinline__ bool pair_body_impl(const PairParams& P, char* smem, int bid, const int nwg, uint2 (&run)[4 * PairCfg<C>::FN],
+                                               const int sum_mode) {
   using K = PairCfg<C>;
   constexpr int PITCH = K::PITCH, CPR = K::CPR, FN = K::FN, NS = K::NS, PER = K::PER, TILE = K::TILE, NT = K::NT, NW = K::NW, WN = K::WN;
   char* ring = smem;
@@ -106,7 +108,13 @@
   unsigned char* s_bits = reinterpret_cast<unsigned char*>(slab + K::SLAB_BYTES);
   float* s_bias = reinterpret_cast<float*>(slab + K::SLAB_BYTES + K::BITS_BYTES);
 
-  const int tid = threadIdx.x, lane = tid & 63, lr = lane & 15, lq = lane >> 4;
+  int tid_ = threadIdx.x;
+  if constexpr (SUM) asm volatile("" : "+v"(tid_));
+  int tid = tid_;
+  int lane = tid & 63, lr = lane & 15, lq = lane >> 4;
+  auto fresh_tid = [&]() {
+    if constexpr (SUM) { asm volatile("" : "+v"(tid)); lane = tid & 63; lr = lane & 15; lq = lane >> 4; }
+  };
   const int wave = __builtin_amdgcn_readfirstlane(tid >> 6);
   const int rg = wave / WN, cg = wave - rg * WN;
 #ifdef DMX_PAIR_STAMPS
@@ -122,6 +130,9 @@
   const int b = bid / P.nb;
   int tq = bid - b * P.nb;
   if (tq >= P.skip_q0) tq += P.skip_n;
+  if constexpr (SUM) {
+    if (tq >= P.own_q0 && tq < P.own_q1) return false;
+  }
   const int t0 = tq * P.BMo;
   const bool single = P.single != 0;
   const int kA = single ? 0 : P.a.ntaps, kB = P.b.ntaps;
@@ -203,6 +214,7 @@
   asm volatile("s_waitcnt vmcnt(0)" ::: "memory");
   __syncthreads();
   DMX_STAMP(1);
+  fresh_tid();
 
   f32x4 acc[4][FN];
   auto zero_acc = [&]() {
@@ -328,6 +340,7 @@
     init_acc(P.a);
     run_stage(false, stepsA, 0);
     DMX_STAMP(2);
+    fresh_tid();
     const int fa = P.a.flags;
     float4 abias[FN];
     {
@@ -339,7 +352,7 @@
 #pragma unroll
       for (int n = 0; n < FN; ++n) abias[n] = (fa & EPI_BIAS) ? make_float4(ab[n][0], ab[n][1], ab[n][2], ab[n][3]) : make_float4(0.f, 0.f, 0.f, 0.f);
     }
-    if (P.r_from_slab) {
+    if (!SUM && P.r_from_slab) {
       u32x2_t rp[4 * FN];
 #pragma unroll
       for (int i = 0; i < 4; ++i)
@@ -428,13 +441,18 @@
   run_stage(true, stepsB, stepsA);
   __syncthreads();
   DMX_STAMP(4);
+  fresh_tid();
   {
     constexpr int EPI_WAVE_BYTES = 64 * (FN * 32 + 16) + 64 * 12;
     static_assert(EPI_WAVE_BYTES * NW <= K::SLAB_BYTES, "epilogue staging does not fit the slab");
     const int mbase = b * T + t0;
     const int tend = t0 + P.BMo < T ? t0 + P.BMo : T;
-    gemm_epilogue_lds_impl<4, FN, 1>(P.b, acc, mbase + rg * 64, cg * 64, lane, 0, T, slab + wave * EPI_WAVE_BYTES, b * T + tend, rpre,
-                                        !single && P.r_from_slab != 0);
+    if constexpr (SUM)
+      gemm_epilogue_lds_core<4, FN, 7>(P.b, acc, mbase + rg * 64, cg * 64, lane, 0, T, slab + wave * EPI_WAVE_BYTES, b * T + tend, rpre,
+                                          false, run, sum_mode, b * T + P.z0, b * T + P.z1);
+    else
+      gemm_epilogue_lds_impl<4, FN, 1>(P.b, acc, mbase + rg * 64, cg * 64, lane, 0, T, slab + wave * EPI_WAVE_BYTES, b * T + tend, rpre,
+                                          !single && P.r_from_slab != 0);
   }
   if (tape_bits_valid) {
 #pragma unroll
@@ -449,6 +467,13 @@
   if (threadIdx.x == 0 && stamp_id < 4096)
     for (int i = 0; i < 8; ++i) g_pair_stamps[stamp_id * 8 + i] = stamp_v[i];
 #endif
+  return true;
+}
+
+template <int C>
+__device__ __forceinline__ void pair_body(const PairParams& P, char* smem, int bid, const int nwg) {
+  uint2 none[4 * PairCfg<C>::FN] = {};
+  (void)pair_body_impl<C, false>(P, smem, bid, nwg, none, 0);
 }
 
 template <int C>
@@ -465,6 +490,23 @@
   const int j = blockIdx.y, n = G.n[j];
   if ((int)blockIdx.x >= n) return;
   pair_body<C>(G.p[j], smem, blockIdx.x, n);
+}
+
+struct PairSum { PairParams p[DMX_PAIR_GROUP]; int n; };
+template <int C>
+__global__ __launch_bounds__(PairCfg<C>::NT, PairCfg<C>::MIN_WAVES) void conv_pair_sum_kernel(const PairSum G) {
+  extern __shared__ __attribute__((aligned(1024))) char smem[];
+  uint2 run[4 * PairCfg<C>::FN];
+#pragma unroll
+  for (int i = 0; i < 4 * PairCfg<C>::FN; ++i) run[i] = make_uint2(0, 0);
+  int have = 0;
+  bool used = false;
+#pragma unroll 1
+  for (int j = 0; j < G.n; ++j) {
+    if (used) __syncthreads();
+    const bool ran = pair_body_impl<C, true>(G.p[j], smem, blockIdx.x, gridDim.x, run, have | (j + 1 < G.n ? 2 : 0));
+    if (ran) { have = 1; used = true; }
+  }
 }
 
 struct Halo { int lo, hi; bool ok; int d; };
@@ -530,7 +572,7 @@
   if (hi > lo && hi - lo < nb) { q0 = lo; q1 = hi; }
 }
 
-long long pair_params(const GemmDesc* a, const GemmDesc& b, PairParams& P, double& fl, double& by, const PairDead* dead = nullptr) {
+long long pair_params(const GemmDesc* a, const GemmDesc& b, PairParams& P, double& fl, double& by, const PairDead* dead = nullptr, int bmo = 0) {
   memset(&P, 0, sizeof(P));
   P.b = b;
   P.single = a ? 0 : 1;
@@ -541,6 +583,7 @@
   if (a) { const Halo ha = halo_of(*a); P.loA = ha.lo; P.hiA = ha.hi; P.off0A = a->tdx[0] + ha.lo; P.dA = ha.d; }
   P.T = b.Wq;
   P.BMo = a ? PAIR_ROWS - hb.lo - hb.hi : PAIR_ROWS;
+  if (bmo > 0 && bmo < P.BMo) P.BMo = bmo;
   P.nb = cdiv(P.T, P.BMo);
   const int nb_all = P.nb;
   {
@@ -662,6 +705,58 @@
   return hipGetLastError() == hipSuccess ? DMX_OK : DMX_ERR_LAUNCH;
 }
 
+bool dmx_conv_pair_sum_eligible(int n, const GemmDesc* const* a, const GemmDesc* const* b) {
+  if (n < 2 || n > DMX_PAIR_GROUP) return false;
+  for (int j = 0; j < n; ++j) {
+    if (!a[j] || !b[j] || !dmx_conv_pair_eligible(a[j], *b[j])) return false;
+    if (b[j]->N != 32 && b[j]->N != 64) return false;
+    if (b[j]->N != b[0]->N || b[j]->M != b[0]->M || b[j]->Wq != b[0]->Wq || b[j]->C != b[0]->C) return false;
+    if (((b[j]->flags & EPI_ACCUM) != 0) != (j > 0)) return false;
+    if (b[j]->flags & EPI_F32OUT) return false;
+    if (j < n - 1 && (b[j]->flags & (EPI_LRELU2 | EPI_BITS2 | EPI_NO_C))) return false;
+  }
+  return true;
+}
+
+int dmx_conv_pair_sum_launch(int n, const GemmDesc* const* a, const GemmDesc* const* b, hipStream_t st, const PairDead* dead) {
+  if (!dmx_conv_pair_sum_eligible(n, a, b)) return DMX_ERR_SHAPE;
+  int bmo = PAIR_ROWS;
+  for (int j = 0; j < n; ++j) { const Halo hb = halo_of(*b[j]); if (PAIR_ROWS - hb.lo - hb.hi < bmo) bmo = PAIR_ROWS - hb.lo - hb.hi; }
+  PairSum G;
+  memset(&G, 0, sizeof(G));
+  G.n = n;
+  const int T = b[0]->Wq, nb_all = cdiv(T, bmo);
+  double fl = 0.0, by = 0.0;
+  int Ksum = 0, iq0 = 0, iq1 = nb_all;
+  for (int j = 0; j < n; ++j) {
+    double f1, b1;
+    (void)pair_params(a[j], *b[j], G.p[j], f1, b1, dead ? dead + j : nullptr, bmo);
+    if (!pair_zero_ok(G.p[j])) return DMX_ERR_SHAPE;
+    PairParams& P = G.p[j];
+    P.own_q0 = P.skip_q0; P.own_q1 = P.skip_q0 + P.skip_n;
+    if (P.own_q0 > iq0) iq0 = P.own_q0;
+    if (P.own_q1 < iq1) iq1 = P.own_q1;
+    b1 -= 2.0 * b[j]->M * (double)b[j]->N * ((j < n - 1 ? 1.0 : 0.0) + ((b[j]->flags & EPI_ACCUM) ? 1.0 : 0.0)) * (double)P.nb / nb_all;
+    fl += f1; by += b1; Ksum += a[j]->K + b[j]->K;
+  }
+  if (iq1 <= iq0) iq0 = iq1 = 0;
+  for (int j = 0; j < n; ++j) { G.p[j].skip_q0 = iq0; G.p[j].skip_n = iq1 - iq0; G.p[j].nb = nb_all - (iq1 - iq0); }
+  const long long grid = (long long)(b[0]->M / T) * (nb_all - (iq1 - iq0));
+  if (grid < 1 || grid > 0x7fffffffLL) return DMX_ERR_SHAPE;
+  const int C = b[0]->N;
+  const int rec = dmx_prof_open(st);
+  auto launch = [&](auto tag) {
+    constexpr int CC = decltype(tag)::value;
+    static bool attr = false;
+    if (!attr) { (void)hipFuncSetAttribute((const void*)conv_pair_sum_kernel<CC>, hipFuncAttributeMaxDynamicSharedMemorySize, PairCfg<CC>::LDS_BYTES); attr = true; }
+    hipLaunchKernelGGL(conv_pair_sum_kernel<CC>, dim3((unsigned)grid), dim3(PairCfg<CC>::NT), PairCfg<CC>::LDS_BYTES, st, G);
+  };
+  if (C == 32) launch(std::integral_constant<int, 32>{});
+  else launch(std::integral_constant<int, 64>{});
+  dmx_prof_close(rec, st, fl, by, b[0]->M, C, Ksum, b[0]->ntaps, b[n - 1]->flags, 23);
+  return hipGetLastError() == hipSuccess ? DMX_OK : DMX_ERR_LAUNCH;
+}
+
 #ifdef DMX_PAIR_STAMPS
 extern "C" int dmx_pair_stamps_read(unsigned long long* host) {
   return hipMemcpyFromSymbol(host, HIP_SYMBOL(g_pair_stamps), sizeof(unsigned long long) * 4096 * 8) == hipSuccess ? 0 : -1;
diff --git a/diffmusic_amd/csrc/gemm_epilogue.h b/diffmusic_amd/csrc/gemm_epilogue.h
--- a/diffmusic_amd/csrc/gemm_epilogue.h
+++ b/diffmusic_amd/csrc/gemm_epilogue.h
@@ -99,10 +99,12 @@
 struct EpiChunk { static constexpr int IB = (FM % DMX_EPI_IB == 0) ? DMX_EPI_IB : (FM % 4 == 0) ? 4 : (FM % 3 == 0) ? 3 : (FM % 2 == 0) ? 2 : 1; static constexpr int CH = IB * 16; };
 
 template <int FM, int FN, int EM>
-__device__ __forceinline__ void gemm_epilogue_lds_impl(const GemmDesc& p, f32x4 (&acc)[FM][FN], int m0, int n0, int lane,
+__device__ __forceinline__ void gemm_epilogue_lds_core(const GemmDesc& p, f32x4 (&acc)[FM][FN], int m0, int n0, int lane,
                                                        long long coff, int HqWq, char* wl, int mlimit,
-                                                       const uint2 (&rpre)[FM * FN], const bool use_rpre) {
-  constexpr bool BITS = EM == 1;
+                                                       const uint2 (&rpre)[FM * FN], const bool use_rpre,
+                                                       uint2 (&run)[FM * FN], const int sum_mode, const int zr0, const int zr1) {
+  constexpr bool SUM = EM == 7;
+  constexpr bool BITS = EM == 1 || SUM;
   constexpr bool SOFT = EM == 2;
   constexpr bool GEGLU = EM == 3;
   constexpr bool ROWS = EM == 4;
@@ -162,12 +164,14 @@
       for (int it = 0; it < NIT; ++it) orows[it] = tab[it * RPI + rr];
       DMX_LDS_SYNC();
     }
+    int zlo = 0, zhi = 0;
     auto stage_in = [&](const act_t* G, int ld, auto&& f) {
       {
         uint4 v[NIT];
 #pragma unroll
         for (int it = 0; it < NIT; ++it) {
-          const bool ok = orows[it] >= 0 && col_ok;
+          bool ok = orows[it] >= 0 && col_ok;
+          if constexpr (SUM) ok = ok && !(orows[it] >= zlo && orows[it] < zhi);
           const long long off = ok ? (long long)orows[it] * ld + ncol : 0ll;
           v[it] = *reinterpret_cast<const uint4*>(G + coff + off);
           if (!ok) v[it] = make_uint4(0, 0, 0, 0);
@@ -394,7 +398,7 @@
           for (int e = 0; e < 4; ++e) a[e] *= 0.5f * g[e] * erfcf(g[e] * -0.70710678118654752f);
         }
     }
-    if ((flags & EPI_RESID) && use_rpre) {
+    if (!SUM && (flags & EPI_RESID) && use_rpre) {
       const float is = (flags & EPI_RESID_INV) ? p.resid_inv_slope : 1.f;
 #pragma unroll
       for (int ii = 0; ii < IB; ++ii)
@@ -407,9 +411,11 @@
         }
     } else if (flags & EPI_RESID) {
       const float is = (flags & EPI_RESID_INV) ? p.resid_inv_slope : 1.f;
+      zlo = zr0; zhi = zr1;
       stage_in(p.R, p.ldr, [&](f32x4& a, float x0, float x1, float x2, float x3) {
         a[0] += fminf(x0, x0 * is); a[1] += fminf(x1, x1 * is); a[2] += fminf(x2, x2 * is); a[3] += fminf(x3, x3 * is);
       });
+      zlo = zhi = 0;
     }
     if (p.alpha != 1.f) {
       const float al = p.alpha;
@@ -418,8 +424,21 @@
 #pragma unroll
         for (int j = 0; j < FN; ++j) { f32x4& a = acc[h * IB + ii][j]; a[0] *= al; a[1] *= al; a[2] *= al; a[3] *= al; }
     }
-    if (flags & EPI_ACCUM)
-      stage_in(reinterpret_cast<const act_t*>(p.C), p.ldc, [&](f32x4& a, float x0, float x1, float x2, float x3) { a[0] += x0; a[1] += x1; a[2] += x2; a[3] += x3; });
+    if constexpr (SUM) {
+      if (sum_mode & 1) {
+#pragma unroll
+        for (int ii = 0; ii < IB; ++ii)
+#pragma unroll
+          for (int j = 0; j < FN; ++j) {
+            const uint2 q = run[(h * IB + ii) * FN + j];
+            f32x4& a = acc[h * IB + ii][j];
+            a[0] += alo(q.x); a[1] += ahi(q.x); a[2] += alo(q.y); a[3] += ahi(q.y);
+          }
+      }
+    } else {
+      if (flags & EPI_ACCUM)
+        stage_in(reinterpret_cast<const act_t*>(p.C), p.ldc, [&](f32x4& a, float x0, float x1, float x2, float x3) { a[0] += x0; a[1] += x1; a[2] += x2; a[3] += x3; });
+    }
     if (flags & EPI_TANH) {
 #pragma unroll
       for (int ii = 0; ii < IB; ++ii)
@@ -454,7 +473,20 @@
       }
     }
     const bool bits2 = (flags & EPI_BITS2) != 0;
-    if (!(flags & EPI_NO_C)) {
+    bool kept = false;
+    if constexpr (SUM) {
+      if (sum_mode & 2) {
+#pragma unroll
+        for (int ii = 0; ii < IB; ++ii)
+#pragma unroll
+          for (int j = 0; j < FN; ++j) {
+            const f32x4& a = acc[h * IB + ii][j];
+            run[(h * IB + ii) * FN + j] = make_uint2(pack2a(a[0], a[1]), pack2a(a[2], a[3]));
+          }
+        kept = true;
+      }
+    }
+    if (!kept && !(flags & EPI_NO_C)) {
       stage_out(reinterpret_cast<act_t*>(p.C), p.ldc, [&](const f32x4& a, float (&o)[4]) { o[0] = a[0]; o[1] = a[1]; o[2] = a[2]; o[3] = a[3]; });
       if constexpr (BITS) { if (bits2 && !(flags & EPI_LRELU2)) emit_bits(); }
       if constexpr (GNS) { if (flags & EPI_GNSTATS) emit_gn(); }
@@ -476,7 +508,7 @@
       }
       DMX_LDS_SYNC();
     }
-    if (flags & EPI_LRELU2) {
+    if (!kept && (flags & EPI_LRELU2)) {
       const float sl = p.act_slope;
       stage_out(p.C2, p.ldc2, [&](const f32x4& a, float (&o)[4]) {
         o[0] = fmaxf(a[0], a[0] * sl); o[1] = fmaxf(a[1], a[1] * sl); o[2] = fmaxf(a[2], a[2] * sl); o[3] = fmaxf(a[3], a[3] * sl);
@@ -489,6 +521,15 @@
 }
 
 template <int FM, int FN, int EM>
+__device__ __forceinline__ void gemm_epilogue_lds_impl(const GemmDesc& p, f32x4 (&acc)[FM][FN], int m0, int n0, int lane,
+                                                       long long coff, int HqWq, char* wl, int mlimit,
+                                                       const uint2 (&rpre)[FM * FN], const bool use_rpre) {
+  static_assert(EM != 7, "the running-tile epilogue is called through gemm_epilogue_lds_core");
+  uint2 none[FM * FN] = {};
+  gemm_epilogue_lds_core<FM, FN, EM>(p, acc, m0, n0, lane, coff, HqWq, wl, mlimit, rpre, use_rpre, none, 0, 0, 0);
+}
+
+template <int FM, int FN, int EM>
 __device__ __forceinline__ void gemm_epilogue_lds(const GemmDesc& p, f32x4 (&acc)[FM][FN], int m0, int n0, int lane,
                                                   long long coff, int HqWq, char* wl, int mlimit = 0x7fffffff) {
   const uint2 none[FM * FN] = {};
diff --git a/diffmusic_amd/csrc/hifigan.hip b/diffmusic_amd/csrc/hifigan.hip
--- a/diffmusic_amd/csrc/hifigan.hip
+++ b/diffmusic_amd/csrc/hifigan.hip
@@ -54,6 +54,7 @@
   dmx_hifigan_config cfg;
   DeadPlan plan;
   bool use_dead = false;
+  bool branch_sum = getenv("DMX_NO_PAIR_SUM") == nullptr;
   static constexpr size_t kSplitKBytes = 32u << 20;
   float* splitk_ws = nullptr;
   ConvLayer conv_pre, conv_post;
@@ -152,6 +153,7 @@
     }
     dmx_conv_pair_slabs(&da, db, &pd, &skipped, &total);
   }
+  bool stage_sums(int C) const { return branch_sum && !multi_wanted() && nk >= 2 && nk <= 3 && (C == 32 || C == 64); }
   bool stage_all_fused(int s, int To) const {
     bool all = nk <= 3;
     for (int k = 0; k < nk; ++k) for (int d = 0; d < nd; ++d) all = all && step_is_fused(idx(s, k, d), To);
@@ -273,7 +275,10 @@
           }
         }
       const size_t mk = arena.mark();
-      act_t* sum = arena.bf(n);
+      bool all_fused = nk <= 3;
+      for (int k = 0; k < nk; ++k) for (int d = 0; d < nd; ++d) all_fused = all_fused && fused[idx(s, k, d)] != 0;
+      const bool sums = all_fused && stage_sums(C);
+      act_t* sum = sums ? nullptr : arena.bf(n);
       {
         Epi e; e.flags = EPI_LRELU2 | EPI_NO_C; e.act_slope = slope; e.C2 = xs_a[s];
         if (xs_b) { e.flags |= EPI_BITS2; e.B2 = xs_b; }
@@ -281,8 +286,6 @@
       }
       const float next_slope = (s == ns - 1) ? 0.01f : slope;
       const bool mt = multi();
-      bool all_fused = nk <= 3;
-      for (int k = 0; k < nk; ++k) for (int d = 0; d < nd; ++d) all_fused = all_fused && fused[idx(s, k, d)] != 0;
       if (all_fused && !mt) {
         for (int d = 0; d < nd; ++d) {
           GemmDesc da[DMX_MAX_STAGES], db[DMX_MAX_STAGES];
@@ -316,6 +319,7 @@
               return DMX_ERR_STATE;
             }
           if (d < nd - 1) RUN(dmx_conv_pair_group_launch(nk, pa, pb, st, dead ? pd : nullptr));
+          else if (sums) RUN(dmx_conv_pair_sum_launch(nk, pa, pb, st, dead ? pd : nullptr));
           else for (int k = 0; k < nk; ++k) RUN(conv_pair_run(da[k], db[k], st, dead ? &pd[k] : nullptr));
         }
         arena.release(mk);
@@ -440,6 +444,7 @@
           }
           if (!dry) {
             if (d > 0) RUN(dmx_conv_pair_group_launch(nk, pa, pb, st, dead ? pd : nullptr));
+            else if (stage_sums(C)) RUN(dmx_conv_pair_sum_launch(nk, pa, pb, st, dead ? pd : nullptr));
             else for (int k = 0; k < nk; ++k) RUN(conv_pair_run(da[k], db[k], st, dead ? &pd[k] : nullptr));
           }
           for (int k = 0; k < nk; ++k) gcs[k] = dsts[k];
@@ -514,6 +519,8 @@
   }
   return h->ns;
 }
+void dmx_hifigan_set_branch_sum_impl(Model* m, int on) { static_cast<HifiGan*>(m)->branch_sum = on != 0 && getenv("DMX_NO_PAIR_SUM") == nullptr; }
+int dmx_hifigan_get_branch_sum_impl(Model* m) { return static_cast<HifiGan*>(m)->branch_sum ? 1 : 0; }
 int dmx_hifigan_bwd_impl(Model* m, const float* dwav, act_t* dmel, hipStream_t st) {
   return static_cast<HifiGan*>(m)->backward(dwav, dmel, st);
 }
diff --git a/diffmusic_amd/csrc/models.h b/diffmusic_amd/csrc/models.h
--- a/diffmusic_amd/csrc/models.h
+++ b/diffmusic_amd/csrc/models.h
@@ -24,6 +24,8 @@
 int dmx_hifigan_bwd_impl(Model* m, const float* dwav, act_t* dmel, hipStream_t st);
 int dmx_hifigan_fwd_dead_impl(Model* m, const act_t* mel, float* wav, int B, int T, int s0, int s1, void* ws, size_t wsb, hipStream_t st);
 int dmx_hifigan_dead_plan_impl(Model* m, int* skipped, int* total, int* lo, int* hi, int n);
+void dmx_hifigan_set_branch_sum_impl(Model* m, int on);
+int dmx_hifigan_get_branch_sum_impl(Model* m);
 int dmx_conv_dead_rows_impl(int k, int dil, int pad, int stride, int transposed, int t_in, int t_out, int a, int b, int* lo, int* hi);
 size_t dmx_hifigan_ws_impl(Model* m, int B, int T);
 
diff --git a/diffmusic_amd/engine.py b/diffmusic_amd/engine.py
--- a/diffmusic_amd/engine.py
+++ b/diffmusic_amd/engine.py
@@ -102,6 +102,14 @@
         c.leaky_relu_slope = cfg["leaky_relu_slope"]
         super().__init__(L.lib().dmx_hifigan_create(C.byref(c)), cfg, device)
         self.dead_span_enabled = os.environ.get("DMX_NO_DEAD_SPAN", "0") in ("", "0")
+
+    @property
+    def branch_sum_enabled(self):
+        return L.lib().dmx_hifigan_set_branch_sum(self._h, -1) > 0
+
+    @branch_sum_enabled.setter
+    def branch_sum_enabled(self, on):
+        L.check(min(L.lib().dmx_hifigan_set_branch_sum(self._h, 1 if on else 0), 0), "hifigan_set_branch_sum")
 
     def _stride_of(self, name):
         return self.cfg["upsample_rates"][int(name.split(".")[1])]
diff --git a/include/diffmusic_hip.h b/include/diffmusic_hip.h
--- a/include/diffmusic_hip.h
+++ b/include/diffmusic_hip.h
@@ -73,6 +73,7 @@
 int dmx_hifigan_fwd_dead(dmx_model* m, const uint16_t* mel, float* wav, int batch, int frames, int s0, int s1, void* ws,
                          size_t ws_bytes, void* stream);
 int dmx_hifigan_dead_plan(dmx_model* m, int* skipped, int* total, int* lo, int* hi, int n);
+int dmx_hifigan_set_branch_sum(dmx_model* m, int on);
 int dmx_conv_dead_rows(int k, int dil, int pad, int stride, int transposed, int t_in, int t_out, int a, int b, int* lo, int* hi);
 
 size_t dmx_vae_workspace_bytes(dmx_model* m, int batch, int h, int w);
@@ -258,6 +259,7 @@
 int dmx_geglu_raw(const void* x, void* y, long long rows, int I, void* stream);
 int dmx_gemm_splitk_workspace(void* ws, size_t bytes);
 int dmx_conv_pair_raw(const void* desc_a, const void* desc_b, size_t desc_bytes, void* stream);
+int dmx_conv_pair_sum_raw(int n, const void* descs_a, const void* descs_b, size_t desc_bytes, const int* dead, void* stream);
 int dmx_conv_pair_dead_raw(const void* desc_a, const void* desc_b, size_t desc_bytes, const int* dead, int* skipped, int* total, void* stream);
 int dmx_conv_pair_group_raw(int n, const void* descs_a, const void* descs_b, size_t desc_bytes, void* stream);
 int dmx_conv_pair_group_dead_raw(int n, const void* descs_a, const void* descs_b, size_t desc_bytes, const int* dead, void* stream);
```

After: 27.12 steps/s (weak scaling: one step advances a batch of 8 clips on one GPU; value = K / wall x 1 GPU(s)). Within noise of the previous version (-0.1%).
